# bgconley/cadence-rag

Hardware: AMD Instinct MI355X
Metric: queries/sec @ recall@10=1.0 (exact cosine top-10, 1024-d fp32 corpus) (higher is better)
Workload: dtype f32; 1 GPU; BASELINE configs[1]: brute-force cosine top-10, 100000x1024 fp32 corpus on one GPU, 64 queries/step resident in HBM; rows_per_gpu=100000, rows_total=100000, dim=1024, k=10, parallelism=1 GPU, rounds=1, arithmetic=fp16-MFMA prefilter (proven bound) + exact fp32 rescoring, api=crag_index_search_async (in stream order), hbm_bytes_per_corpus_row=6156

## Files before the change

### cadence_rag_amd/_native.py

```python
from __future__ import annotations

import ctypes
import os
import subprocess
from pathlib import Path
from typing import Optional

_CSRC = Path(__file__).resolve().parent / "csrc"
LIB_PATH = Path(os.environ["CRAG_DENSE_LIB"]) if os.environ.get("CRAG_DENSE_LIB") else _CSRC / "libcrag_dense.so"

CRAG_MAX_K = 128
CRAG_DIM = 1024
CRAG_DEDUPE_MAX_WIDTH = 256
CRAG_SUBSET_MAX_WIDTH = 4096
CRAG_GROUP_MAX_PER = 8
CRAG_FILTER_MAX_QUERIES = 64
CRAG_ATTR_MAX_QUERIES = 64
CRAG_ATTR_MAX_CLAUSES = 8
CRAG_ATTR_MAX_KEYS = 512
CRAG_FACET_MAX_QUERIES = 64
CRAG_FACET_MAX_NAMESPACES = 16
CRAG_FACET_MAX_TOP = 64
CRAG_E2BIG = -5
CRAG_DECODE_MAX_SEQS = 8
CRAG_DECODE_MAX_ROWS = 8
CRAG_DECODE_SPLIT = 128
CRAG_LM_HEAD_MAX_BANNED = 64
CRAG_EXTEND_BLOCK = 32
CRAG_EXTEND_TILE = 32
CRAG_EXTEND_SPLIT = 512
CRAG_EXTEND_SPLIT_ROWS = 512
CRAG_GRAMMAR_MAX_STATES = 4096
CRAG_GRAMMAR_MAX_CLASSES = 64
CRAG_GRAMMAR_DEAD = 0xFFFF
CRAG_SAMPLE_MIN_TEMPERATURE = 0.01
CRAG_SAMPLE_MAX_TEMPERATURE = 100.0

_c = ctypes
_P = _c.c_void_p
SIGNATURES = {
    "crag_last_error": (_c.c_char_p, []),
    "crag_version": (_c.c_char_p, []),
    "crag_device_count": (_c.c_int, []),
    "crag_index_create": (_c.c_int, [_c.c_int, _c.c_int, _c.c_int64, _c.POINTER(_P)]),
    "crag_index_destroy": (_c.c_int, [_P]),
    "crag_index_add": (_c.c_int, [_P, _P, _P, _c.c_int64]),
    "crag_index_update": (_c.c_int, [_P, _c.c_int64, _P, _c.c_int64]),
    "crag_index_remove": (_c.c_int, [_P, _P, _c.c_int64, _c.POINTER(_c.c_int64)]),
    "crag_index_compact": (_c.c_int, [_P, _P, _c.POINTER(_c.c_int64)]),
    "crag_index_insert": (_c.c_int, [_P, _P, _P, _c.c_int64]),
    "crag_index_size": (_c.c_int64, [_P]),
    "crag_index_capacity": (_c.c_int64, [_P]),
    "crag_index_dim": (_c.c_int, [_P]),
    "crag_index_get_rows": (_c.c_int, [_P, _c.c_int64, _c.c_int64, _P, _P]),
    "crag_index_count_eligible": (_c.c_int, [_P, _P, _c.POINTER(_c.c_int64)]),
    "crag_index_search": (_c.c_int, [_P, _P, _c.c_int, _c.c_int, _P, _c.c_int64, _P, _P, _P]),
    "crag_index_search_async": (_c.c_int, [_P, _P, _c.c_int, _c.c_int, _P, _c.c_int64, _P, _P, _P, _P]),
    "crag_merge_topk": (_c.c_int, [_c.c_int, _P, _P, _P, _c.c_int, _c.c_int, _c.c_int, _P, _P, _P, _P]),
    "crag_result_record_bytes": (_c.c_int64, [_c.c_int, _c.c_int]),
    "crag_merge_topk_packed": (_c.c_int, [_c.c_int, _P, _c.c_int, _c.c_int, _c.c_int, _P, _P, _P, _P]),
    "crag_rrf_fuse": (_c.c_int, [_c.c_int, _P, _P, _P, _c.c_int, _c.c_int, _c.c_int, _P, _P, _P, _P, _P]),
    "crag_tech_lane": (_c.c_int, [_P, _P, _P, _P, _c.c_int64, _P, _P, _c.c_int, _c.c_int, _P, _c.c_int64, _P, _P, _P, _P]),
    "crag_upload_slot_create": (_P, []),
    "crag_upload_slot_destroy": (None, [_P]),
    "crag_tech_lane_host": (_c.c_int, [_P, _P, _P, _P, _c.c_int64, _P, _P, _c.c_int, _c.c_int, _P, _c.c_int64, _P, _P, _P,
                                       _P, _P]),
    "crag_bm25_scratch_bytes": (_c.c_int64, [_c.c_int64, _c.c_int, _c.c_int]),
    "crag_bm25_lane_host": (_c.c_int, [_P, _P, _P, _P, _P, _c.c_int64, _c.c_int64, _c.c_float, _P, _P, _P, _c.c_int, _c.c_int,
                                       _P, _c.c_int64, _P, _P, _c.c_int64, _P, _P, _P, _P]),
    "crag_filter_masks_host": (_c.c_int, [_P, _P, _c.c_int64, _c.c_int64, _P, _P, _P, _c.c_int, _P, _P, _c.c_int64, _P]),
    "crag_attr_masks_host": (_c.c_int, [_P, _P, _c.c_int64, _c.c_int64, _P, _P, _c.c_int, _P, _c.c_int, _P, _c.c_int64, _P, _P,
                                        _c.c_int64, _P]),
    "crag_facet_workspace_bytes": (_c.c_int64, [_c.c_int64, _c.c_int, _c.c_int64, _c.c_int]),
    "crag_facet_counts_host": (_c.c_int, [_P, _P, _P, _c.c_int64, _c.c_int64, _c.c_int64, _P, _c.c_int64, _P, _P, _c.c_int,
                                          _c.c_int, _c.c_int, _P, _c.c_int64, _P, _P, _P, _P, _P]),
    "crag_index_profile_enable": (_c.c_int, [_P, _c.c_int]),
    "crag_index_profile_read": (_c.c_int, [_P, _c.POINTER(_c.c_int64), _c.POINTER(_c.c_double),
                                           _c.POINTER(_c.c_double)]),
    "crag_index_profile_read_ex": (_c.c_int, [_P, _c.POINTER(_c.c_int64), _c.POINTER(_c.c_double),
                                              _c.POINTER(_c.c_double), _c.POINTER(_c.c_double)]),
    "crag_index_last_scan_kernel": (_c.c_char_p, [_P]),
    "crag_index_scan_waits": (_c.c_char_p, [_P]),
    "crag_index_prefilter_row_bytes": (_c.c_int64, [_P]),
    "crag_index_search_pipelined": (_c.c_int, [_P, _P, _c.c_int, _c.c_int, _P, _c.c_int64, _P, _P, _P, _P, _c.c_int]),
    "crag_index_join": (_c.c_int, [_P, _P]),
    "crag_index_dedupe_async": (_c.c_int, [_P, _P, _P, _c.c_int, _c.c_int, _c.c_float, _P, _P, _P, _P, _P]),
    "crag_index_search_ids_scratch_bytes": (_c.c_int64, [_c.c_int, _c.c_int]),
    "crag_index_search_ids_async": (_c.c_int, [_P, _P, _c.c_int, _P, _P, _c.c_int, _c.c_int64, _c.c_int, _P, _P, _P, _P, _P,
                                               _c.c_int64, _P]),
    "crag_index_search_grouped_scratch_bytes": (_c.c_int64, [_c.c_int, _c.c_int64, _c.c_int]),
    "crag_index_search_grouped_async": (_c.c_int, [_P, _P, _c.c_int, _c.c_int, _P, _c.c_int64, _c.c_int, _P, _c.c_int64,
                                                   _P, _P, _P, _P, _P, _c.c_int64, _P]),
    "crag_index_phase_trace": (_c.c_int, [_P, _c.POINTER(_c.c_uint64)]),
    "crag_index_prefilter_stats": (_c.c_int, [_P, _c.POINTER(_c.c_int64), _c.POINTER(_c.c_int64),
                                              _c.POINTER(_c.c_int64)]),
    "crag_index_scan_geometry": (_c.c_int, [_P, _c.c_int, _c.POINTER(_c.c_int), _c.POINTER(_c.c_int),
                                            _c.POINTER(_c.c_int), _c.POINTER(_c.c_int64)]),
    "crag_enc_embed_gather": (_c.c_int, [_P, _P, _P, _c.c_int64, _c.c_int, _c.c_int64, _P]),
    "crag_enc_rmsnorm": (_c.c_int, [_P, _P, _P, _P, _P, _c.c_int64, _c.c_int, _c.c_float, _P]),
    "crag_enc_qk_norm_rope": (_c.c_int, [_P, _P, _P, _P, _P, _c.c_int64, _c.c_int, _c.c_int, _c.c_float, _P]),
    "crag_enc_v_transpose": (_c.c_int, [_P, _P, _P, _c.c_int64, _c.c_int, _c.c_int, _P]),
    "crag_enc_attention": (_c.c_int, [_P, _P, _P, _P, _P, _P, _P, _c.c_int, _c.c_int64, _c.c_int, _c.c_int,
                                      _c.c_float, _P]),
    "crag_enc_swiglu": (_c.c_int, [_P, _P, _c.c_int64, _c.c_int, _P]),
    "crag_enc_skinny_gemm": (_c.c_int, [_P, _P, _P, _c.c_int, _c.c_int, _c.c_int, _c.c_int, _c.c_int, _P]),
    "crag_enc_qk_rope_vt": (_c.c_int, [_P, _P, _P, _P, _P, _c.c_int64, _c.c_int, _c.c_int, _c.c_float, _P, _P, _c.c_int64, _P]),
    "crag_enc_pool_normalize": (_c.c_int, [_P, _P, _P, _P, _c.c_int, _c.c_int, _c.c_int, _c.c_int, _c.c_float, _P]),
    "crag_enc_pool_normalize_add": (_c.c_int, [_P, _P, _P, _P, _P, _c.c_int, _c.c_int, _c.c_int, _c.c_int, _c.c_float, _P]),
    "crag_enc_pool_normalize_rows": (_c.c_int, [_P, _P, _P, _P, _P, _c.c_int, _c.c_int, _c.c_int, _c.c_float, _P]),
    "crag_enc_small_gemm": (_c.c_int, [_P, _P, _P, _P, _P, _P, _c.c_int, _c.c_int, _c.c_int, _c.c_int, _c.c_int, _c.c_int,
                                       _c.c_float, _P]),
    "crag_enc_wide_partial_bytes": (_c.c_int64, [_c.c_int, _c.c_int, _c.c_int]),
    "crag_enc_wide_gemm": (_c.c_int, [_P, _P, _P, _c.c_int, _c.c_int, _c.c_int, _c.c_int, _P]),
    "crag_enc_wide_gemm_direct": (_c.c_int, [_P, _P, _P, _c.c_int, _c.c_int, _c.c_int, _c.c_int, _c.c_int, _P]),
    "crag_enc_wide_reduce": (_c.c_int, [_P, _P, _c.c_int, _c.c_int, _c.c_int, _c.c_int, _c.c_int, _P]),
    "crag_enc_wide_gemm_rows": (_c.c_int, [_P, _P, _P, _c.c_int, _c.c_int, _c.c_int, _c.c_int, _P]),
    "crag_enc_rmsnorm_partials": (_c.c_int, [_P, _c.c_int, _c.c_int, _P, _P, _P, _P, _c.c_int, _c.c_int, _c.c_float, _P]),
    "crag_enc_small_attention": (_c.c_int, [_P, _P, _P, _P, _c.c_int, _P, _P, _c.c_int, _c.c_int, _c.c_int, _c.c_float,
                                            _c.c_float, _P]),
    "crag_enc_small_attention_seqs": (_c.c_int, [_P, _P, _P, _P, _c.c_int, _P, _P, _c.c_int, _c.c_int, _P, _c.c_int,
                                                 _c.c_int, _c.c_float, _c.c_float, _P]),
    "crag_enc_small_attention_seqs_parts": (_c.c_int, [_P, _c.c_int, _c.c_int, _P, _P, _P, _c.c_int, _P, _P, _c.c_int,
                                                       _c.c_int, _P, _c.c_int, _c.c_int, _c.c_float, _c.c_float, _P]),
    "crag_enc_attention_prefixed": (_c.c_int, [_P, _P, _P, _P, _P, _P, _P, _P, _c.c_int, _c.c_int64, _c.c_int, _c.c_int,
                                               _c.c_float, _P]),
    "crag_enc_rerank_head": (_c.c_int, [_P, _P, _P, _P, _P, _P, _c.c_int, _c.c_int, _c.c_float, _P]),
    "crag_enc_decode_workspace_bytes": (_c.c_int64, [_c.c_int, _c.c_int, _c.c_int]),
    "crag_enc_decode_attention": (_c.c_int, [_P, _P, _P, _P, _c.c_int, _P, _P, _c.c_int, _c.c_int, _P, _P, _c.c_int, _c.c_int,
                                             _c.c_int, _c.c_float, _c.c_float, _P, _c.c_int64, _P, _P]),
    "crag_enc_decode_attention_shared": (_c.c_int, [_P, _P, _P, _P, _c.c_int, _P, _P, _c.c_int, _c.c_int, _P, _P, _P, _P,
                                                    _c.c_int, _c.c_int, _c.c_int, _c.c_float, _c.c_float, _P, _c.c_int64,
                                                    _P, _P]),
    "crag_enc_decode_attention_rows": (_c.c_int, [_P, _P, _P, _P, _c.c_int, _P, _P, _c.c_int, _c.c_int, _P, _P, _P, _P, _P,
                                                  _c.c_int, _c.c_int, _c.c_int, _c.c_float, _c.c_float, _P, _c.c_int64,
                                                  _P, _P]),
    "crag_enc_lm_head": (_c.c_int, [_P, _P, _P, _P, _P, _P, _P, _c.c_int, _c.c_int, _c.c_int, _c.c_int64, _c.c_float, _P]),
    "crag_enc_extend_workspace_bytes": (_c.c_int64, [_c.c_int, _c.c_int, _c.c_int, _c.c_int]),
    "crag_enc_extend_attention": (_c.c_int, [_P, _P, _P, _P, _c.c_int, _P, _P, _c.c_int, _c.c_int, _P, _P, _P, _c.c_int,
                                             _c.c_int, _c.c_int, _c.c_float, _c.c_float, _P, _c.c_int64, _P, _P]),
    "crag_enc_grammar_argmax": (_c.c_int, [_P, _c.c_int64, _P, _P, _P, _P, _P, _P, _c.c_int, _c.c_int, _P, _P, _P, _c.c_int,
                                           _P]),
    "crag_enc_sample": (_c.c_int, [_P, _c.c_int64, _P, _P, _P, _P, _P, _P, _c.c_uint64, _c.c_uint32, _P, _P, _P, _c.c_int, _P]),
    "crag_enc_grammar_advance": (_c.c_int, [_P, _P, _P, _c.c_int64, _P, _P, _c.c_int, _c.c_int, _P, _P, _c.c_int, _P]),
    "crag_enc_logprobs": (_c.c_int, [_P, _c.c_int64, _P, _P, _P, _P, _P, _P, _P, _P, _c.c_int, _c.c_int, _P]),
}


class NativeLibraryError(RuntimeError):
    """libcrag_dense.so is missing, failed to load, or a call into it failed."""


_lib: Optional[ctypes.CDLL] = None


def build_native(force: bool = False) -> Path:
    cmd = ["make", "-C", str(_CSRC)] + (["-B"] if force else [])
    proc = subprocess.run(cmd, capture_output=True, text=True)
    if proc.returncode != 0:
        raise NativeLibraryError(f"building libcrag_dense.so failed:\n{proc.stdout}\n{proc.stderr}")
    return LIB_PATH


def load() -> ctypes.CDLL:
    global _lib
    if _lib is not None:
        return _lib
    if not LIB_PATH.exists():
        raise NativeLibraryError(
            f"{LIB_PATH} not found: the dense lane has no CPU fallback. Build it with "
            f"`python -c 'import __graft_entry__ as g; g.build()'` or `make -C {_CSRC}`.")
    try:
        lib = ctypes.CDLL(str(LIB_PATH))
    except OSError as exc:
        raise NativeLibraryError(f"failed to load {LIB_PATH}: {exc}") from exc
    for name, (restype, argtypes) in SIGNATURES.items():
        try:
            fn = getattr(lib, name)
        except AttributeError as exc:
            raise NativeLibraryError(f"{LIB_PATH} does not export {name}") from exc
        fn.restype = restype
        fn.argtypes = argtypes
    _lib = lib
    return lib


def last_error() -> str:
    msg = load().crag_last_error()
    return msg.decode("utf-8", "replace") if msg else ""


def check(rc: int, what: str) -> None:
    if rc != 0:
        raise NativeLibraryError(f"{what} failed (code {rc}): {last_error()}")
```

### cadence_rag_amd/csrc/crag_api.hip

```cpp

#include <stdlib.h>

#include <new>

#include "crag_index.h"

namespace {

thread_local char g_err[512] = "";

int init_index(crag_index *ix) {
    const size_t cbytes = (size_t)ix->cap_rows * crag::DIM * sizeof(float);
    hipError_t e;
    if ((e = hipMalloc((void **)&ix->corpus, cbytes)) != hipSuccess ||
        (e = hipMalloc((void **)&ix->inv_norm, (size_t)ix->cap_rows * sizeof(float))) != hipSuccess ||
        (e = hipMalloc((void **)&ix->ids, (size_t)ix->cap_rows * sizeof(int64_t))) != hipSuccess)
        return fail(CRAG_ENOMEM, "hipMalloc for %lld rows failed: %s", (long long)ix->cap_rows, hipGetErrorString(e));
    if ((e = hipMemset(ix->inv_norm, 0, (size_t)ix->cap_rows * sizeof(float))) != hipSuccess ||
        (e = hipMemset(ix->corpus, 0, cbytes)) != hipSuccess)
        return fail(CRAG_EHIP, "hipMemset failed: %s", hipGetErrorString(e));
    for (auto &w : ix->ws)
        if ((e = hipEventCreateWithFlags(&w.done, hipEventDisableTiming)) != hipSuccess)
            return fail(CRAG_EHIP, "hipEventCreate failed: %s", hipGetErrorString(e));
    ix->sw.no_wide = getenv("CRAG_NO_WIDE") != nullptr;
    ix->env_no_reverse = getenv("CRAG_NO_REVERSE") != nullptr;
    ix->env_unpipelined = getenv("CRAG_UNPIPELINED") != nullptr;
    ix->sw.no_prefilter = getenv("CRAG_NO_PREFILTER") != nullptr;
    ix->sw.no_rsplit = getenv("CRAG_NO_RSPLIT") != nullptr;
    if (const char *v = getenv("CRAG_PF_NT")) ix->sw.pf_nt = atoi(v) ? 1 : 0;
    if (const char *v = getenv("CRAG_PF_WAITS")) {
        if (!strcmp(v, "tile")) ix->sw.pf_waits = crag::PF_WAITS_TILE;
        else if (!strcmp(v, "fragment")) ix->sw.pf_waits = crag::PF_WAITS_FRAGMENT;
    }
    if (const char *v = getenv("CRAG_PF_LAGS")) {
        int d = 0, r = 0;
        if (sscanf(v, "%d,%d", &d, &r) == 2 && d >= 1 && r > d && r <= 4) {
            ix->sw.pf_derive_lag = d;
            ix->sw.pf_read_lag = r;
        }
    }
    if (const char *v = getenv("CRAG_TEST_FAIL_AFTER_SCAN")) ix->env_fail_after_scan = atoll(v);
    if (const char *v = getenv("CRAG_PIPE_STREAMS")) {
        const int n = atoi(v);
        if (n >= 1 && n <= crag_index::MAX_PIPE) ix->n_pipe = n;
    }
    if (const char *v = getenv("CRAG_EDIT_CHUNK_ROWS")) {
        const long long c = atoll(v);
        if (c >= 32 && c % 32 == 0 && c <= ((long long)1 << 24)) ix->edit_chunk_rows = c;
    }
    if (const char *v = getenv("CRAG_PF_NT_ABOVE_MB")) ix->sw.nt_above_bytes = (int64_t)atoll(v) << 20;
    if (!ix->sw.no_prefilter && getenv("CRAG_NO_FP16_MIRROR") == nullptr) {
        const size_t mbytes = (size_t)ix->cap_rows * crag::DIM * sizeof(_Float16);
        if ((e = hipMalloc((void **)&ix->corpus16, mbytes)) != hipSuccess ||
            (e = hipMemset(ix->corpus16, 0, mbytes)) != hipSuccess)
            return fail(CRAG_ENOMEM, "hipMalloc for the fp16 mirror of %lld rows failed: %s", (long long)ix->cap_rows,
                        hipGetErrorString(e));
    }
    if ((e = hipMalloc((void **)&ix->irregular_dev, sizeof(uint32_t))) != hipSuccess ||
        (e = hipMalloc((void **)&ix->pf_stats, crag::PF_STAT_SLOTS * 3 * sizeof(unsigned long long))) != hipSuccess ||
        (e = hipMemset(ix->irregular_dev, 0, sizeof(uint32_t))) != hipSuccess ||
        (e = hipMemset(ix->pf_stats, 0, crag::PF_STAT_SLOTS * 3 * sizeof(unsigned long long))) != hipSuccess)
        return fail(CRAG_ENOMEM, "hipMalloc for the index state failed: %s", hipGetErrorString(e));
    if (getenv("CRAG_PHASE_TRACE") != nullptr) {
        if ((e = hipMalloc((void **)&ix->phase_trace, 128 * sizeof(unsigned long long))) != hipSuccess ||
            (e = hipMemset(ix->phase_trace, 0, 128 * sizeof(unsigned long long))) != hipSuccess)
            return fail(CRAG_ENOMEM, "hipMalloc for the phase trace failed: %s", hipGetErrorString(e));
    }
    return CRAG_OK;
}

int check_merge_args(bool any_null, int n_lists, int nq, int k) {
    if (any_null) return fail(CRAG_EINVAL, "NULL pointer argument");
    if (n_lists <= 0 || nq < 0 || k <= 0 || k > CRAG_MAX_K)
        return fail(CRAG_EINVAL, "bad sizes n_lists=%d nq=%d k=%d", n_lists, nq, k);
    if ((int64_t)n_lists * k > 4096) return fail(CRAG_EINVAL, "n_lists*k must be <= 4096");
    return CRAG_OK;
}

int merge_lists(int device, crag::XMergeParams &p, int n_lists, int nq, int k, int64_t *d_out_ids, float *d_out_scores,
                int32_t *d_out_counts, void *stream) {
    DeviceGuard guard(device);
    if (!guard.ok) return fail(CRAG_EHIP, "hipSetDevice(%d) failed", device);
    p.out_ids = d_out_ids;
    p.out_scores = d_out_scores;
    p.out_counts = d_out_counts;
    p.n_lists = n_lists;
    p.nq = nq;
    p.k = k;
    HIP_TRY(crag::launch_merge_results(p, (hipStream_t)stream));
    return CRAG_OK;
}

}

extern "C" {

const char *crag_last_error(void) { return g_err; }

void crag_set_error_(const char *msg) { snprintf(g_err, sizeof(g_err), "%s", msg ? msg : ""); }

const char *crag_version(void) { return "cadence-rag_amd dense lane 0.1 (gfx950)"; }

int crag_device_count(void) {
    int n = 0;
    if (hipGetDeviceCount(&n) != hipSuccess) {
        (void)hipGetLastError();
        return 0;
    }
    return n;
}

int crag_index_create(int device, int dim, int64_t capacity, crag_index **out) {
    if (!out) return fail(CRAG_EINVAL, "out is NULL");
    *out = nullptr;
    if (dim <= 0 || dim > CRAG_DIM) return fail(CRAG_EINVAL, "dim must be in [1, %d] (got %d)", CRAG_DIM, dim);
    if (capacity <= 0) return fail(CRAG_EINVAL, "capacity must be > 0 (got %lld)", (long long)capacity);
    int ndev = crag_device_count();
    if (ndev <= 0) return fail(CRAG_ENODEV, "no HIP device visible");
    if (device < 0 || device >= ndev) return fail(CRAG_EINVAL, "device %d out of range [0, %d)", device, ndev);
    DeviceGuard guard(device);
    if (!guard.ok) return fail(CRAG_EHIP, "hipSetDevice(%d) failed", device);
    hipDeviceProp_t prop;
    HIP_TRY(hipGetDeviceProperties(&prop, device));
    if (strncmp(prop.gcnArchName, "gfx950", 6) != 0)
        return fail(CRAG_ENODEV, "device %d is %s; this library is built for gfx950 only", device,
                    prop.gcnArchName);
    crag_index *ix = new (std::nothrow) crag_index();
    if (!ix) return fail(CRAG_ENOMEM, "out of host memory");
    ix->device = device;
    ix->dim = dim;
    ix->capacity = capacity;
    ix->cap_rows = ((capacity + 31) / 32) * 32;
    ix->n_cu = prop.multiProcessorCount;
    int rc = init_index(ix);
    if (rc) {
        crag_index_destroy(ix);
        return rc;
    }
    *out = ix;
    return CRAG_OK;
}

int crag_index_destroy(crag_index *ix) {
    if (!ix) return CRAG_OK;
    DeviceGuard guard(ix->device);
    (void)hipDeviceSynchronize();
    for (auto &t : ix->ev_pool)
        for (hipEvent_t e : {t.e0, t.e1a, t.e1, t.e2, t.e3}) (void)hipEventDestroy(e);
    for (int i = 0; i < crag_index::MAX_PIPE; ++i) {
        if (ix->pipe_fork[i]) (void)hipEventDestroy(ix->pipe_fork[i]);
        if (ix->pipe_done[i]) (void)hipEventDestroy(ix->pipe_done[i]);
        if (ix->pipe[i]) (void)hipStreamDestroy(ix->pipe[i]);
    }
    for (void *p : {(void *)ix->irregular_dev, (void *)ix->phase_trace, (void *)ix->pf_stats, (void *)ix->corpus,
                    (void *)ix->corpus16, (void *)ix->inv_norm, (void *)ix->ids})
        if (p) (void)hipFree(p);
    for (auto &w : ix->ws) {
        for (auto &b : w.buf) b.release();
        if (w.done) (void)hipEventDestroy(w.done);
    }
    for (DevBuf *b : {&ix->stage_q, &ix->stage_rows, &ix->stage_ids, &ix->stage_mask, &ix->stage_out, &ix->scratch,
                      &ix->edit_bounce, &ix->edit_srcpos, &ix->edit_mask, &ix->edit_prefix, &ix->edit_newpos})
        b->release();
    delete ix;
    return CRAG_OK;
}

int64_t crag_index_size(const crag_index *ix) { return ix ? ix->size : -1; }
int64_t crag_index_capacity(const crag_index *ix) { return ix ? ix->capacity : -1; }
int crag_index_dim(const crag_index *ix) { return ix ? ix->dim : -1; }

int crag_merge_topk(int device, const int64_t *d_ids, const float *d_scores, const int32_t *d_counts,
                    int n_lists, int nq, int k, int64_t *d_out_ids, float *d_out_scores,
                    int32_t *d_out_counts, void *stream) {
    int rc = check_merge_args(!d_ids || !d_scores || !d_counts || !d_out_ids || !d_out_scores || !d_out_counts, n_lists,
                              nq, k);
    if (rc || nq == 0) return rc;
    crag::XMergeParams p;
    p.ids = d_ids;
    p.scores = d_scores;
    p.counts = d_counts;
    p.stride_ids = (int64_t)nq * k;
    p.stride_scores = (int64_t)nq * k;
    p.stride_counts = nq;
    return merge_lists(device, p, n_lists, nq, k, d_out_ids, d_out_scores, d_out_counts, stream);
}

int64_t crag_result_record_bytes(int nq, int k) {
    if (nq < 0 || k <= 0) return -1;
    const int64_t b = (int64_t)nq * k * 8 + (int64_t)nq * k * 4 + (int64_t)nq * 4;
    return (b + 7) & ~(int64_t)7;
}

int crag_merge_topk_packed(int device, const void *d_records, int n_lists, int nq, int k, int64_t *d_out_ids,
                           float *d_out_scores, int32_t *d_out_counts, void *stream) {
    int rc = check_merge_args(!d_records || !d_out_ids || !d_out_scores || !d_out_counts, n_lists, nq, k);
    if (rc || nq == 0) return rc;
    const int64_t rec = crag_result_record_bytes(nq, k);
    const char *base = (const char *)d_records;
    crag::XMergeParams p;
    p.ids = (const int64_t *)base;
    p.scores = (const float *)(base + (int64_t)nq * k * 8);
    p.counts = (const int32_t *)(base + (int64_t)nq * k * 12);
    p.stride_ids = rec / 8;
    p.stride_scores = rec / 4;
    p.stride_counts = rec / 4;
    return merge_lists(device, p, n_lists, nq, k, d_out_ids, d_out_scores, d_out_counts, stream);
}

int crag_index_profile_enable(crag_index *ix, int enabled) {
    if (!ix) return fail(CRAG_EINVAL, "index is NULL");
    std::lock_guard<std::mutex> lk(ix->mu);
    ix->profiling = enabled > 0 ? enabled : 0;
    ix->prof_calls = 0;
    ix->ev_used = 0;
    return CRAG_OK;
}

int crag_index_profile_read_ex(crag_index *ix, int64_t *n_launches, double *scan_ms_total,
                               double *merge_ms_total, double *event_pair_ms_total) {
    if (!ix) return fail(CRAG_EINVAL, "index is NULL");
    std::lock_guard<std::mutex> lk(ix->mu);
    DeviceGuard guard(ix->device);
    double scan = 0.0, merge = 0.0, pair = 0.0;
    for (size_t i = 0; i < ix->ev_used; ++i) {
        float a = 0.f, b = 0.f, c = 0.f, d = 0.f;
        HIP_TRY(hipEventSynchronize(ix->ev_pool[i].e3));
        HIP_TRY(hipEventElapsedTime(&a, ix->ev_pool[i].e0, ix->ev_pool[i].e1a));
        HIP_TRY(hipEventElapsedTime(&d, ix->ev_pool[i].e1a, ix->ev_pool[i].e1));
        HIP_TRY(hipEventElapsedTime(&b, ix->ev_pool[i].e1, ix->ev_pool[i].e2));
        HIP_TRY(hipEventElapsedTime(&c, ix->ev_pool[i].e2, ix->ev_pool[i].e3));
        scan += b;
        merge += a + c;
        pair += d;
    }
    if (n_launches) *n_launches = (int64_t)ix->ev_used;
    if (scan_ms_total) *scan_ms_total = scan;
    if (merge_ms_total) *merge_ms_total = merge;
    if (event_pair_ms_total) *event_pair_ms_total = pair;
    ix->ev_used = 0;
    return CRAG_OK;
}

int crag_index_profile_read(crag_index *ix, int64_t *n_launches, double *scan_ms_total,
                            double *merge_ms_total) {
    return crag_index_profile_read_ex(ix, n_launches, scan_ms_total, merge_ms_total, nullptr);
}

int crag_index_prefilter_stats(crag_index *ix, int64_t *searches, int64_t *candidates, int64_t *rescored_rows) {
    if (!ix) return fail(CRAG_EINVAL, "index is NULL");
    std::lock_guard<std::mutex> lk(ix->mu);
    DeviceGuard guard(ix->device);
    unsigned long long v[3] = {0, 0, 0};
    std::vector<unsigned long long> rec((size_t)crag::PF_STAT_SLOTS * 3);
    HIP_TRY(hipDeviceSynchronize());
    HIP_TRY(hipMemcpy(rec.data(), ix->pf_stats, rec.size() * sizeof(unsigned long long), hipMemcpyDeviceToHost));
    HIP_TRY(hipMemset(ix->pf_stats, 0, rec.size() * sizeof(unsigned long long)));
    for (size_t i = 0; i < rec.size(); ++i) v[i % 3] += rec[i];
    if (candidates) *candidates = (int64_t)v[0];
    if (rescored_rows) *rescored_rows = (int64_t)v[1];
    if (searches) *searches = (int64_t)v[2];
    return CRAG_OK;
}

int crag_index_phase_trace(crag_index *ix, uint64_t *out128) {
    if (!ix || !out128) return fail(CRAG_EINVAL, "index / out is NULL");
    if (!ix->phase_trace) return fail(CRAG_EINVAL, "the index was not created with CRAG_PHASE_TRACE=1");
    std::lock_guard<std::mutex> lk(ix->mu);
    DeviceGuard guard(ix->device);
    HIP_TRY(hipDeviceSynchronize());
    HIP_TRY(hipMemcpy(out128, ix->phase_trace, 128 * sizeof(unsigned long long), hipMemcpyDeviceToHost));
    return CRAG_OK;
}

const char *crag_index_last_scan_kernel(const crag_index *ix) { return ix ? ix->last_scan_kernel : ""; }
const char *crag_index_scan_waits(const crag_index *ix) { return ix ? ix->last_scan_waits : ""; }

int64_t crag_index_prefilter_row_bytes(const crag_index *ix) {
    if (!ix || ix->sw.no_prefilter) return 0;
    return (int64_t)crag::DIM * (ix->corpus16 ? 2 : 4);
}

int crag_index_scan_geometry(const crag_index *ix, int nq, int *workgroups, int *threads,
                             int *query_blocks, int64_t *algorithmic_bytes_per_launch) {
    if (!ix) return fail(CRAG_EINVAL, "index is NULL");
    const int qb = (nq + 31) / 32;
    if (workgroups) *workgroups = plan_search(ix->size, ix->n_cu, nq, 1, false, false, ix->sw).G;
    if (threads) *threads = crag::SCAN_THREADS;
    if (query_blocks) *query_blocks = qb;
    if (algorithmic_bytes_per_launch)
        *algorithmic_bytes_per_launch = ix->size * (int64_t)ix->dim * 4 + (int64_t)nq * ix->dim * 4;
    return CRAG_OK;
}

}
```

### cadence_rag_amd/csrc/crag_api_search.hip

```cpp

#include "crag_index.h"

namespace {

struct SearchArgs {
    const float *queries;
    int nq, k;
    const uint8_t *mask;
    int64_t mask_stride;
    int64_t *out_ids;
    float *out_scores;
    int32_t *out_counts;
};

int acquire_workspace(crag_index *ix, hipStream_t st, Workspace **out) {
    Workspace *ws = nullptr;
    for (auto &w : ix->ws)
        if (w.in_use && w.stream == st) ws = &w;
    if (!ws)
        for (auto &w : ix->ws)
            if (!w.in_use) {
                w.in_use = true;
                w.stream = st;
                ws = &w;
                if (&w == &ix->ws[crag_index::MAX_WS - 1]) ix->record_done = true;
                break;
            }
    if (!ws) {
        for (auto &w : ix->ws)
            if (!ws || w.last_use < ws->last_use) ws = &w;
        if (ws->done_recorded && !ws->dirty) {
            HIP_TRY(hipStreamWaitEvent(st, ws->done, 0));
        } else {
            HIP_TRY(hipDeviceSynchronize());
        }
        ix->record_done = true;
        ws->stream = st;
    }
    ws->last_use = ++ix->use_clock;
    *out = ws;
    return CRAG_OK;
}

int reserve_workspace(const crag_index *ix, Workspace *ws, const SearchPlan &pl, int k, hipStream_t st) {
    DevBuf *b = ws->buf;
    const size_t nq_pad = (size_t)pl.nq_pad;
    int rc;
    if ((rc = b[Workspace::PARTIAL].ensure((size_t)pl.q_blocks * pl.G * 32 * (size_t)k * sizeof(uint2)))) return rc;
    if ((rc = b[Workspace::GBOUND].ensure_zeroed((size_t)pl.q_blocks * 32 * crag::GB_CELLS * sizeof(uint32_t), st))) return rc;
    if ((rc = b[Workspace::A32].ensure(nq_pad * crag::DIM * sizeof(float)))) return rc;
    if ((rc = b[Workspace::QINV].ensure(nq_pad * sizeof(float)))) return rc;
    if (!pl.prefilter) return CRAG_OK;
    if ((rc = b[Workspace::A16].ensure(nq_pad * crag::DIM * 2))) return rc;
    if ((rc = b[Workspace::PF_GBOUND].ensure_zeroed((ix->n_cu + nq_pad) * crag::PF_BOUND_CELLS * sizeof(uint32_t), st))) return rc;
    if ((rc = b[Workspace::PF_CAND].ensure(nq_pad * pl.cap * sizeof(uint2)))) return rc;
    if (pl.rsplit > 1) {
        const size_t slots = nq_pad * 8;
        if ((rc = b[Workspace::PF_XKEYS].ensure(slots * CRAG_MAX_K * sizeof(uint64_t)))) return rc;
        if ((rc = b[Workspace::PF_XIDS].ensure(slots * CRAG_MAX_K * sizeof(int64_t)))) return rc;
        if ((rc = b[Workspace::PF_XCOUNT].ensure(slots * sizeof(uint2)))) return rc;
        if ((rc = b[Workspace::PF_XTICKET].ensure_zeroed(nq_pad * sizeof(uint32_t), st))) return rc;
    }
    if ((rc = b[Workspace::PF_COUNT].ensure_zeroed(nq_pad * sizeof(uint32_t), st))) return rc;
    if ((rc = b[Workspace::PF_FLAGS].ensure_zeroed(4 * sizeof(uint32_t), st))) return rc;
    if (ws->dirty) {
        for (int i = Workspace::KEPT_ZERO_FIRST; i < Workspace::KEPT_ZERO_END; ++i)
            if (b[i].p) HIP_TRY(hipMemsetAsync(b[i].p, 0, b[i].bytes, st));
        ws->dirty = false;
    }
    return CRAG_OK;
}

int profile_begin(crag_index *ix, hipStream_t st, EvSet **out) {
    *out = nullptr;
    if (!(ix->profiling > 0 && (ix->prof_calls++ % ix->profiling) == ix->profiling / 2)) return CRAG_OK;
    if (ix->ev_used == ix->ev_pool.size()) {
        EvSet t;
        for (hipEvent_t *e : {&t.e0, &t.e1a, &t.e1, &t.e2, &t.e3}) HIP_TRY(hipEventCreate(e));
        ix->ev_pool.push_back(t);
    }
    *out = &ix->ev_pool[ix->ev_used++];
    HIP_TRY(hipEventRecord((*out)->e0, st));
    return CRAG_OK;
}

crag::PrepParams prep_params(const crag_index *ix, const Workspace *ws, const SearchPlan &pl, const SearchArgs &a) {
    return crag::PrepParams{a.queries, a.nq, ix->dim, ws->at<float>(Workspace::QINV), ws->at<float>(Workspace::A32),
                            pl.prefilter ? ws->at<_Float16>(Workspace::A16) : nullptr};
}

crag::ScanParams scan_params(const crag_index *ix, const Workspace *ws, const SearchPlan &pl, const SearchArgs &a,
                             int reverse) {
    crag::ScanParams sp;
    sp.wide = pl.wide;
    sp.corpus = ix->corpus;
    sp.inv_norm = ix->inv_norm;
    sp.queries = a.queries;
    sp.a32 = ws->at<const float>(Workspace::A32);
    sp.qinv = ws->at<const float>(Workspace::QINV);
    sp.gate = nullptr;
    sp.dim = ix->dim;
    sp.mask = (const uint32_t *)a.mask;
    sp.mask_stride_w = a.mask_stride / 4;
    sp.partial = ws->at<uint2>(Workspace::PARTIAL);
    sp.gbound = ws->at<uint32_t>(Workspace::GBOUND);
    sp.n_rows = ix->size;
    sp.cap_rows = ix->cap_rows;
    sp.nq = a.nq;
    sp.k = a.k;
    sp.G = pl.G;
    sp.nb = pl.nb;
    sp.pub_rank = pl.pub_rank;
    sp.reverse = reverse;
    sp.unpipelined = (ix->env_unpipelined && !pl.prefilter) ? 1 : 0;
    sp.piece_shift = crag::crag_piece_shift(ix->corpus16 != nullptr);
    return sp;
}

crag::MergeParams merge_params(const crag_index *ix, const Workspace *ws, const SearchPlan &pl, const SearchArgs &a) {
    crag::MergeParams mp;
    mp.partial = ws->at<const uint2>(Workspace::PARTIAL);
    mp.ids = ix->ids;
    mp.gbound = ws->at<uint32_t>(Workspace::GBOUND);
    mp.id_base = 0;
    mp.out_ids = a.out_ids;
    mp.out_scores = a.out_scores;
    mp.out_counts = a.out_counts;
    mp.k = a.k;
    mp.G = pl.G;
    return mp;
}

crag::PfParams pf_params(const crag_index *ix, const Workspace *ws, const SearchPlan &pl, const SearchArgs &a,
                         int reverse) {
    crag::PfParams fp;
    fp.corpus = ix->corpus;
    fp.corpus16 = ix->corpus16;
    fp.inv_norm = ix->inv_norm;
    fp.a16 = ws->at<const _Float16>(Workspace::A16);
    fp.qinv = ws->at<const float>(Workspace::QINV);
    fp.mask = (const uint32_t *)a.mask;
    fp.mask_stride_w = a.mask_stride / 4;
    fp.gbound_idle = ws->at<const uint32_t>(Workspace::PF_GBOUND);
    fp.gbound = ws->at<uint32_t>(Workspace::PF_GBOUND) + (size_t)ix->n_cu * crag::PF_BOUND_CELLS;
    fp.cand = ws->at<uint2>(Workspace::PF_CAND);
    fp.count = ws->at<uint32_t>(Workspace::PF_COUNT);
    fp.flags = ws->at<uint32_t>(Workspace::PF_FLAGS);
    fp.seq = ws->seq;
    fp.n_rows = ix->size;
    fp.nq = a.nq;
    fp.k = a.k;
    fp.G = pl.G;
    fp.reverse = reverse;
    fp.sets = pl.sets;
    fp.pub0 = pl.pub0;
    fp.cap = pl.cap;
    fp.derive_lag = pl.derive_lag;
    fp.read_lag = pl.read_lag;
    fp.nt = pl.nt;
    return fp;
}

crag::FinParams fin_params(const crag_index *ix, const Workspace *ws, const SearchPlan &pl, const SearchArgs &a,
                           const crag::PfParams &fp, crag::ScanParams sp, const crag::MergeParams &mp) {
    crag::FinParams fin;
    fin.corpus = ix->corpus;
    fin.inv_norm = ix->inv_norm;
    fin.a32 = ws->at<const float>(Workspace::A32);
    fin.qinv = ws->at<const float>(Workspace::QINV);
    fin.cand = ws->at<const uint2>(Workspace::PF_CAND);
    fin.count = ws->at<uint32_t>(Workspace::PF_COUNT);
    fin.gbound = fp.gbound;
    fin.flags = ws->at<const uint32_t>(Workspace::PF_FLAGS);
    fin.seq = fp.seq;
    fin.ids = ix->ids;
    fin.out_ids = a.out_ids;
    fin.out_scores = a.out_scores;
    fin.out_counts = a.out_counts;
    fin.stats = ix->pf_stats + (size_t)(ws - ix->ws) * (crag::PF_STAT_SLOTS / crag_index::MAX_WS) * 3;
    fin.k = a.k;
    fin.cap = pl.cap;
    fin.merge = mp;
    fin.nq = a.nq;
    fin.rsplit = pl.rsplit;
    const bool shared = pl.rsplit > 1;
    fin.xkeys = shared ? ws->at<uint64_t>(Workspace::PF_XKEYS) : nullptr;
    fin.xids = shared ? ws->at<int64_t>(Workspace::PF_XIDS) : nullptr;
    fin.xcount = shared ? ws->at<uint2>(Workspace::PF_XCOUNT) : nullptr;
    fin.xticket = shared ? ws->at<uint32_t>(Workspace::PF_XTICKET) : nullptr;
    sp.wide = 0;
    sp.gate = nullptr;
    sp.unpipelined = 1;
    fin.scan = sp;
    fin.fb_blocks = pl.fb_blocks;
    fin.fb_done = ws->at<uint32_t>(Workspace::PF_FLAGS) + 1;
    fin.trace = ix->phase_trace;
    return fin;
}

int search_device(crag_index *ix, const SearchArgs &a, hipStream_t st) {
    if (a.nq <= 0) return CRAG_OK;
    const SearchPlan pl = plan_search(ix->size, ix->n_cu, a.nq, a.k, ix->corpus16 != nullptr, ix->irregular, ix->sw);
    int rc;
    Workspace *ws = nullptr;
    if ((rc = acquire_workspace(ix, st, &ws))) return rc;
    if ((rc = reserve_workspace(ix, ws, pl, a.k, st))) return rc;
    if (pl.window_too_large)
        return fail(CRAG_EINVAL, "index too large for one device scan window (%lld rows)", (long long)ix->size);
    EvSet *ev = nullptr;
    if ((rc = profile_begin(ix, st, &ev))) return rc;

    HIP_TRY(crag::launch_prep_queries(prep_params(ix, ws, pl, a), pl.nq_pad, st));
    const int reverse = ix->env_no_reverse ? 0 : ix->pass_parity;
    ix->pass_parity ^= 1;
    const crag::ScanParams sp = scan_params(ix, ws, pl, a, reverse);
    const crag::MergeParams mp = merge_params(ix, ws, pl, a);
    if (ev) {
        HIP_TRY(hipEventRecord(ev->e1a, st));
        HIP_TRY(hipEventRecord(ev->e1, st));
    }
    if (pl.prefilter) {
        if (++ws->seq == 0u) ws->seq = 1u;
        const crag::PfParams fp = pf_params(ix, ws, pl, a, reverse);
        const int nqb = pl.wide ? 2 : 1;
        ws->dirty = true;
        const int waits = pf_waits_for(ix->size * (int64_t)crag::DIM * 2, ix->corpus16 != nullptr, pl.nt, ix->sw.pf_waits);
        HIP_TRY(crag::launch_prefilter(fp, nqb, pl.nq_pad / (32 * nqb), waits == crag::PF_WAITS_FRAGMENT, st,
                                       &ix->last_scan_kernel));
        ix->last_scan_waits = waits == crag::PF_WAITS_FRAGMENT ? "fragment" : "tile";
        if (ix->env_fail_after_scan > 0 && ++ix->pf_searches == ix->env_fail_after_scan)
            return fail(CRAG_EHIP, "injected failure behind the scan launch (CRAG_TEST_FAIL_AFTER_SCAN)");
        if (ev) HIP_TRY(hipEventRecord(ev->e2, st));
        HIP_TRY(crag::launch_finalize(fin_params(ix, ws, pl, a, fp, sp, mp), st));
        ws->dirty = false;
    } else {
        HIP_TRY(crag::launch_scan(sp, pl.q_blocks, st, &ix->last_scan_kernel));
        ix->last_scan_waits = "tile";
        if (ev) HIP_TRY(hipEventRecord(ev->e2, st));
        HIP_TRY(crag::launch_merge_partials(mp, a.nq, st));
    }
    if (ev) HIP_TRY(hipEventRecord(ev->e3, st));
    ws->done_recorded = ix->record_done;
    if (ix->record_done) HIP_TRY(hipEventRecord(ws->done, st));
    return CRAG_OK;
}

int check_search_args(const crag_index *ix, const SearchArgs &a) {
    if (!ix) return fail(CRAG_EINVAL, "index is NULL");
    if (a.nq < 0) return fail(CRAG_EINVAL, "nq must be >= 0 (got %d)", a.nq);
    if (a.k <= 0 || a.k > CRAG_MAX_K) return fail(CRAG_EINVAL, "k must be in [1, %d] (got %d)", CRAG_MAX_K, a.k);
    if (a.nq > 0 && (!a.queries || !a.out_ids || !a.out_scores || !a.out_counts))
        return fail(CRAG_EINVAL, "queries / out_ids / out_scores / out_counts must not be NULL");
    if (a.mask) {
        const int64_t need = ((ix->size + 31) / 32) * 4;
        if (a.mask_stride != 0 && (a.mask_stride % 4 != 0 || a.mask_stride < need))
            return fail(CRAG_EINVAL, "mask_stride must be 0 or a multiple of 4 >= %lld (got %lld)",
                        (long long)need, (long long)a.mask_stride);
        if (((uintptr_t)a.mask) & 3) return fail(CRAG_EINVAL, "row_mask must be 4-byte aligned");
    }
    return CRAG_OK;
}

}

extern "C" {

int crag_search_plan_(int64_t size, int n_cu, int nq, int k, int has_mirror, int irregular, int no_wide,
                      int no_prefilter, int no_rsplit, int pf_derive_lag, int pf_read_lag, int pf_nt,
                      int64_t nt_above_bytes, SearchPlan *out) {
    const SearchSwitches sw = {no_wide, no_prefilter, no_rsplit, pf_derive_lag, pf_read_lag, pf_nt, nt_above_bytes};
    if (out) *out = plan_search(size, n_cu, nq, k, has_mirror != 0, irregular != 0, sw);
    return (int)sizeof(SearchPlan);
}

int crag_pf_waits_(int64_t mirror_bytes, int has_mirror, int nt, int pf_waits_switch) {
    return pf_waits_for(mirror_bytes, has_mirror != 0, nt, pf_waits_switch);
}

int64_t crag_pf_frag_waits_max_bytes_(void) { return crag::PF_FRAG_WAITS_MAX_BYTES; }

int crag_index_search_async(crag_index *ix, const float *d_queries, int nq, int k,
                            const uint8_t *d_row_mask, int64_t mask_stride, int64_t *d_out_ids,
                            float *d_out_scores, int32_t *d_out_counts, void *stream) {
    const SearchArgs a = {d_queries, nq, k, d_row_mask, mask_stride, d_out_ids, d_out_scores, d_out_counts};
    int rc = check_search_args(ix, a);
    if (rc) return rc;
    std::lock_guard<std::mutex> lk(ix->mu);
    DeviceGuard guard(ix->device);
    return search_device(ix, a, (hipStream_t)stream);
}

int crag_index_search_pipelined(crag_index *ix, const float *d_queries, int nq, int k,
                                const uint8_t *d_row_mask, int64_t mask_stride, int64_t *d_out_ids,
                                float *d_out_scores, int32_t *d_out_counts, void *stream, int flags) {
    const SearchArgs a = {d_queries, nq, k, d_row_mask, mask_stride, d_out_ids, d_out_scores, d_out_counts};
    int rc = check_search_args(ix, a);
    if (rc) return rc;
    std::lock_guard<std::mutex> lk(ix->mu);
    DeviceGuard guard(ix->device);
    for (int i = 0; i < ix->n_pipe; ++i) {
        if (!ix->pipe[i]) HIP_TRY(hipStreamCreateWithFlags(&ix->pipe[i], hipStreamNonBlocking));
        if (!ix->pipe_fork[i]) HIP_TRY(hipEventCreateWithFlags(&ix->pipe_fork[i], hipEventDisableTiming));
        if (!ix->pipe_done[i]) HIP_TRY(hipEventCreateWithFlags(&ix->pipe_done[i], hipEventDisableTiming));
    }
    if (k > 24 || ix->n_pipe <= 1) return search_device(ix, a, (hipStream_t)stream);
    const int i = (int)(ix->pipe_next++ % (unsigned)ix->n_pipe);
    if (!(flags & CRAG_PIPE_INPUTS_READY)) {
        HIP_TRY(hipEventRecord(ix->pipe_fork[i], (hipStream_t)stream));
        HIP_TRY(hipStreamWaitEvent(ix->pipe[i], ix->pipe_fork[i], 0));
    }
    rc = search_device(ix, a, ix->pipe[i]);
    if (rc) return rc;
    ix->pipe_pending[i] = true;
    return CRAG_OK;
}

int crag_index_join(crag_index *ix, void *stream) {
    if (!ix) return fail(CRAG_EINVAL, "index is NULL");
    std::lock_guard<std::mutex> lk(ix->mu);
    DeviceGuard guard(ix->device);
    for (int i = 0; i < ix->n_pipe; ++i)
        if (ix->pipe_pending[i]) {
            HIP_TRY(hipEventRecord(ix->pipe_done[i], ix->pipe[i]));
            HIP_TRY(hipStreamWaitEvent((hipStream_t)stream, ix->pipe_done[i], 0));
            ix->pipe_pending[i] = false;
        }
    return CRAG_OK;
}

int crag_index_search(crag_index *ix, const float *queries, int nq, int k, const uint8_t *row_mask,
                      int64_t mask_stride, int64_t *out_ids, float *out_scores, int32_t *out_counts) {
    int rc = check_search_args(ix, {queries, nq, k, row_mask, mask_stride, out_ids, out_scores, out_counts});
    if (rc) return rc;
    if (nq == 0) return CRAG_OK;
    std::lock_guard<std::mutex> lk(ix->mu);
    DeviceGuard guard(ix->device);

    const float *dq = nullptr;
    if ((rc = stage_in(ix->stage_q, queries, (size_t)nq * ix->dim * sizeof(float), &dq))) return rc;
    const uint8_t *dm = nullptr;
    int64_t dstride = 0;
    if ((rc = stage_row_masks(ix, row_mask, mask_stride, nq, &dm, &dstride))) return rc;
    const bool ids_dev = is_device_ptr(out_ids), sc_dev = is_device_ptr(out_scores),
               ct_dev = is_device_ptr(out_counts);
    const size_t b_ids = (size_t)nq * k * sizeof(int64_t), b_sc = (size_t)nq * k * sizeof(float),
                 b_ct = (size_t)nq * sizeof(int32_t);
    if ((rc = ix->stage_out.ensure(b_ids + b_sc + b_ct + 64))) return rc;
    char *so = (char *)ix->stage_out.p;
    int64_t *d_ids = ids_dev ? out_ids : (int64_t *)so;
    float *d_sc = sc_dev ? out_scores : (float *)(so + b_ids);
    int32_t *d_ct = ct_dev ? out_counts : (int32_t *)(so + b_ids + b_sc);

    rc = search_device(ix, {dq, nq, k, dm, dstride, d_ids, d_sc, d_ct}, 0);
    if (rc) return rc;
    HIP_TRY(hipStreamSynchronize(0));
    if (!ids_dev) HIP_TRY(hipMemcpy(out_ids, d_ids, b_ids, hipMemcpyDeviceToHost));
    if (!sc_dev) HIP_TRY(hipMemcpy(out_scores, d_sc, b_sc, hipMemcpyDeviceToHost));
    if (!ct_dev) HIP_TRY(hipMemcpy(out_counts, d_ct, b_ct, hipMemcpyDeviceToHost));
    return CRAG_OK;
}

int crag_index_dedupe_async(crag_index *ix, const int64_t *d_ids, const int32_t *d_counts, int nq, int width,
                            float threshold, int64_t *d_out_ids, int32_t *d_out_counts, int32_t *d_out_dup_of,
                            float *d_out_sim, void *stream) {
    if (!ix) return fail(CRAG_EINVAL, "index is NULL");
    if (nq < 0) return fail(CRAG_EINVAL, "nq must be >= 0 (got %d)", nq);
    if (width < 1 || width > CRAG_DEDUPE_MAX_WIDTH)
        return fail(CRAG_EINVAL, "width must be in [1, %d] (got %d)", CRAG_DEDUPE_MAX_WIDTH, width);
    if (!(threshold > -1.f && threshold <= 1.f))
        return fail(CRAG_EINVAL, "threshold must be finite, in (-1, 1] (got %g)", (double)threshold);
    if (!d_ids || !d_counts || !d_out_ids || !d_out_counts)
        return fail(CRAG_EINVAL, "ids / counts / out_ids / out_counts must not be NULL");
    if (nq == 0) return CRAG_OK;
    std::lock_guard<std::mutex> lk(ix->mu);
    DeviceGuard guard(ix->device);
    crag::DedupeParams p;
    p.corpus = ix->corpus;
    p.inv_norm = ix->inv_norm;
    p.stored = ix->ids;
    p.size = ix->size;
    p.piece_shift = crag::crag_piece_shift(ix->corpus16 != nullptr);
    p.ids = d_ids;
    p.counts = d_counts;
    p.width = width;
    p.threshold = threshold;
    p.out_ids = d_out_ids;
    p.out_counts = d_out_counts;
    p.out_dup_of = d_out_dup_of;
    p.out_sim = d_out_sim;
    HIP_TRY(crag::launch_dedupe(p, nq, (hipStream_t)stream));
    return CRAG_OK;
}

int64_t crag_index_search_ids_scratch_bytes(int nq, int width) { return crag::subset_scratch_bytes(nq, width); }

int crag_index_search_ids_async(crag_index *ix, const float *d_queries, int nq, const int64_t *d_ids,
                                const int32_t *d_counts, int width, int64_t list_stride, int k, int64_t *d_out_ids,
                                float *d_out_scores, int32_t *d_out_counts, float *d_out_slot_scores, void *d_scratch,
                                int64_t scratch_bytes, void *stream) {
    if (!ix) return fail(CRAG_EINVAL, "search_ids: index is NULL");
    if (nq < 0 || nq > 65535) return fail(CRAG_EINVAL, "search_ids: nq must be in [0, 65535] (got %d)", nq);
    if (width < 1) return fail(CRAG_EINVAL, "search_ids: width must be >= 1 (got %d)", width);
    if (k < 1 || k > CRAG_MAX_K) return fail(CRAG_EINVAL, "search_ids: k must be in [1, %d] (got %d)", CRAG_MAX_K, k);
    if (list_stride != 0 && list_stride != width)
        return fail(CRAG_EINVAL, "search_ids: list_stride must be 0 (one shared list) or width (got %lld)",
                    (long long)list_stride);
    if (!d_queries || !d_ids || !d_counts || !d_out_ids || !d_out_scores || !d_out_counts || !d_scratch)
        return fail(CRAG_EINVAL, "search_ids: queries / ids / counts / outputs / scratch must not be NULL");
    if (width > CRAG_SUBSET_MAX_WIDTH)
        return fail(CRAG_E2BIG, "search_ids: width %d exceeds CRAG_SUBSET_MAX_WIDTH (%d): use the row_mask route", width,
                    CRAG_SUBSET_MAX_WIDTH);
    if (scratch_bytes < crag::subset_scratch_bytes(nq, width) || ((uintptr_t)d_scratch & 7))
        return fail(CRAG_EINVAL, "search_ids: scratch too small or not 8-byte aligned (crag_index_search_ids_scratch_bytes)");
    if (nq == 0) return CRAG_OK;
    std::lock_guard<std::mutex> lk(ix->mu);
    DeviceGuard guard(ix->device);
    crag::SubsetParams p;
    p.corpus = ix->corpus;
    p.inv_norm = ix->inv_norm;
    p.stored = ix->ids;
    p.size = ix->size;
    p.piece_shift = crag::crag_piece_shift(ix->corpus16 != nullptr);
    p.queries = d_queries;
    p.nq = nq;
    p.dim = ix->dim;
    p.k = k;
    p.ids = d_ids;
    p.counts = d_counts;
    p.width = width;
    p.list_stride = list_stride;
    p.keys = (uint64_t *)d_scratch;
    p.out_ids = d_out_ids;
    p.out_scores = d_out_scores;
    p.out_counts = d_out_counts;
    p.out_slot_scores = d_out_slot_scores;
    HIP_TRY(crag::launch_subset(p, (hipStream_t)stream));
    return CRAG_OK;
}

int64_t crag_index_search_grouped_scratch_bytes(int nq, int64_t n_groups, int per_group) {
    return crag::group_scratch_bytes(nq, n_groups, per_group);
}

int crag_index_search_grouped_async(crag_index *ix, const float *d_queries, int nq, int k, const int32_t *d_row_group,
                                    int64_t n_groups, int per_group, const uint8_t *d_row_mask, int64_t mask_stride,
                                    int64_t *d_out_ids, float *d_out_scores, int32_t *d_out_groups, int32_t *d_out_counts,
                                    void *d_scratch, int64_t scratch_bytes, void *stream) {
    if (!ix) return fail(CRAG_EINVAL, "search_grouped: index is NULL");
    if (nq < 0 || nq > 65535) return fail(CRAG_EINVAL, "search_grouped: nq must be in [0, 65535] (got %d)", nq);
    if (k < 1 || k > CRAG_MAX_K) return fail(CRAG_EINVAL, "search_grouped: k must be in [1, %d] (got %d)", CRAG_MAX_K, k);
    if (per_group < 1 || per_group > CRAG_GROUP_MAX_PER)
        return fail(CRAG_EINVAL, "search_grouped: per_group must be in [1, %d] (got %d)", CRAG_GROUP_MAX_PER, per_group);
    if (n_groups < 1 || n_groups >= ((int64_t)1 << 31))
        return fail(CRAG_EINVAL, "search_grouped: n_groups must be in [1, 2^31) (got %lld)", (long long)n_groups);
    if (!d_queries || !d_row_group || !d_out_ids || !d_out_scores || !d_out_counts || !d_scratch)
        return fail(CRAG_EINVAL, "search_grouped: queries / row_group / out_ids / out_scores / out_counts / scratch must not be NULL");
    if (d_row_mask) {
        const int64_t need = ((ix->size + 31) / 32) * 4;
        if (mask_stride != 0 && (mask_stride % 4 != 0 || mask_stride < need))
            return fail(CRAG_EINVAL, "search_grouped: mask_stride must be 0 or a multiple of 4 >= %lld (got %lld)",
                        (long long)need, (long long)mask_stride);
        if (((uintptr_t)d_row_mask) & 3) return fail(CRAG_EINVAL, "search_grouped: row_mask must be 4-byte aligned");
    }
    if (scratch_bytes < crag::group_scratch_bytes(nq, n_groups, per_group) || ((uintptr_t)d_scratch & 7))
        return fail(CRAG_EINVAL,
                    "search_grouped: scratch too small or not 8-byte aligned (crag_index_search_grouped_scratch_bytes)");
    if (nq == 0) return CRAG_OK;
    std::lock_guard<std::mutex> lk(ix->mu);
    DeviceGuard guard(ix->device);
    crag::GroupParams p;
    p.corpus = ix->corpus;
    p.inv_norm = ix->inv_norm;
    p.stored = ix->ids;
    p.size = ix->size;
    p.piece_shift = crag::crag_piece_shift(ix->corpus16 != nullptr);
    p.queries = d_queries;
    p.nq = nq;
    p.dim = ix->dim;
    p.k = k;
    p.row_group = d_row_group;
    p.n_groups = n_groups;
    p.per_group = per_group;
    p.mask = (const uint32_t *)d_row_mask;
    p.mask_stride_w = mask_stride / 4;
    p.table = (uint64_t *)d_scratch;
    p.qinv = (float *)(p.table + (size_t)nq * (size_t)n_groups * (size_t)per_group);
    p.out_ids = d_out_ids;
    p.out_scores = d_out_scores;
    p.out_groups = d_out_groups;
    p.out_counts = d_out_counts;
    HIP_TRY(crag::launch_grouped(p, (hipStream_t)stream));
    return CRAG_OK;
}

}
```

### cadence_rag_amd/csrc/crag_exact.h

```cpp
#pragma once
#include <hip/hip_runtime.h>
#include <stdint.h>

#include "crag_kernels.h"
#include "crag_layout.h"

namespace crag {

__device__ __forceinline__ uint32_t f2ord(float f) {
    uint32_t u = __float_as_uint(f);
    return (u & 0x80000000u) ? ~u : (u | 0x80000000u);
}
__device__ __forceinline__ float ord2f(uint32_t u) {
    u = (u & 0x80000000u) ? (u & 0x7fffffffu) : ~u;
    return __uint_as_float(u);
}
__device__ __forceinline__ uint64_t mk64(uint32_t hi, uint32_t lo) {
    return ((uint64_t)hi << 32) | lo;
}

__device__ __forceinline__ void sort_keys_desc(uint64_t *keys, int P) {
    const int tid = threadIdx.x;
    for (int k2 = 2; k2 <= P; k2 <<= 1)
        for (int j = k2 >> 1; j > 0; j >>= 1) {
            for (int t = tid; t < (P >> 1); t += SCAN_THREADS) {
                const int i = ((t & ~(j - 1)) << 1) | (t & (j - 1)), l = i | j;
                const uint64_t a = keys[i], b = keys[l];
                const bool desc = (i & k2) == 0;
                if (desc ? a < b : a > b) {
                    keys[i] = b;
                    keys[l] = a;
                }
            }
            __syncthreads();
        }
}

__device__ __forceinline__ f32x4 load_query_quad(const float *queries, int dim, int q, int nq, int t) {
    f32x4 v = {0.f, 0.f, 0.f, 0.f};
    if (q < nq && t < 256) {
        const float *src = queries + (size_t)q * dim;
        if ((dim & 3) == 0) {
            if (4 * t < dim) v = *reinterpret_cast<const f32x4 *>(src + 4 * t);
        } else {
#pragma unroll
            for (int c = 0; c < 4; ++c)
                if (4 * t + c < dim) v[c] = src[4 * t + c];
        }
    }
    return v;
}

__device__ __forceinline__ float canonical_qinv(const f32x4 v, bool real_query, double *sh) {
    double ss = ((double)v[0] * v[0] + (double)v[1] * v[1]) + ((double)v[2] * v[2] + (double)v[3] * v[3]);
    for (int o = 32; o > 0; o >>= 1) ss += __shfl_xor(ss, o);
    const int wv = threadIdx.x >> 6;
    if ((threadIdx.x & 63) == 0 && wv < 4) sh[wv] = ss;
    __syncthreads();
    const double tot = sh[0] + sh[1] + sh[2] + sh[3];
    __syncthreads();
    const bool ok = real_query && (tot > 0.0) && (tot < 1.0e300) && (tot == tot);
    float qinv = ok ? (float)(1.0 / sqrt(tot)) : 0.f;
    if (!(qinv < 3.0e38f)) qinv = 0.f;
    return qinv;
}

__device__ __forceinline__ void make_key(float dot, float scale, int64_t row, uint32_t &khi, uint32_t &klo) {
    float sc = dot * scale;
    sc = __builtin_amdgcn_fmed3f(sc, -1.f, 1.f);
    const bool ok = (scale > 0.f) && (sc == sc);
    khi = ok ? f2ord(sc) : 0u;
    klo = ok ? ~(uint32_t)row : 0u;
}

template <int PS>
__device__ __forceinline__ float exact_slice_dot(const f32x4 *qslice ,
                                                 const f32x4 *ctile , int jrow) {
    f32x4 c0[16], c1[16];
#pragma unroll
    for (int s = 0; s < 16; ++s) {
        c0[s] = ctile[(((2 * s) >> PS) * 32 + jrow) * (1 << PS) + ((2 * s) & ((1 << PS) - 1))];
        c1[s] = ctile[(((2 * s) >> PS) * 32 + jrow) * (1 << PS) + ((2 * s) & ((1 << PS) - 1)) + 1];
    }
    float acc = 0.f;
#pragma unroll
    for (int s = 0; s < 16; ++s) {
        const f32x4 q0 = qslice[2 * s], q1 = qslice[2 * s + 1];
#pragma unroll
        for (int cc = 0; cc < 4; ++cc) {
            acc = __builtin_fmaf(q0[cc], c0[s][cc], acc);
            acc = __builtin_fmaf(q1[cc], c1[s][cc], acc);
        }
    }
    return acc;
}

template <int PS>
__device__ __forceinline__ void exact_slice_fetch(const f32x4 *ctile , int jrow, f32x4 (&c0)[16],
                                                  f32x4 (&c1)[16]) {
#pragma unroll
    for (int s = 0; s < 16; ++s) {
        c0[s] = ctile[(((2 * s) >> PS) * 32 + jrow) * (1 << PS) + ((2 * s) & ((1 << PS) - 1))];
        c1[s] = ctile[(((2 * s) >> PS) * 32 + jrow) * (1 << PS) + ((2 * s) & ((1 << PS) - 1)) + 1];
    }
}

__device__ __forceinline__ void slice_query_read(const f32x4 *qslice, int h, f32x4 (&q)[8]) {
#pragma unroll
    for (int i = 0; i < 8; ++i) q[i] = qslice[8 * h + i];
}
__device__ __forceinline__ float slice_query_fma(float acc, int h, const f32x4 (&q)[8], const f32x4 (&c0)[16],
                                                 const f32x4 (&c1)[16]) {
#pragma unroll
    for (int s4 = 0; s4 < 4; ++s4) {
        const f32x4 q0 = q[2 * s4], q1 = q[2 * s4 + 1];
#pragma unroll
        for (int cc = 0; cc < 4; ++cc) {
            acc = __builtin_fmaf(q0[cc], c0[4 * h + s4][cc], acc);
            acc = __builtin_fmaf(q1[cc], c1[4 * h + s4][cc], acc);
        }
    }
    return acc;
}
__device__ __forceinline__ float exact_slice_fma(const f32x4 *qslice , const f32x4 (&c0)[16],
                                                 const f32x4 (&c1)[16]) {
    f32x4 qa[8], qb[8];
    slice_query_read(qslice, 0, qa);
    slice_query_read(qslice, 1, qb);
    __builtin_amdgcn_sched_barrier(0);
    float acc = slice_query_fma(0.f, 0, qa, c0, c1);
    __builtin_amdgcn_sched_barrier(0);
    slice_query_read(qslice, 2, qa);
    __builtin_amdgcn_sched_barrier(0);
    acc = slice_query_fma(acc, 1, qb, c0, c1);
    __builtin_amdgcn_sched_barrier(0);
    slice_query_read(qslice, 3, qb);
    __builtin_amdgcn_sched_barrier(0);
    acc = slice_query_fma(acc, 2, qa, c0, c1);
    acc = slice_query_fma(acc, 3, qb, c0, c1);
    return acc;
}

}
```

### cadence_rag_amd/csrc/crag_index.h

```cpp
#pragma once
#include <mutex>
#include <vector>

#include "crag_host.h"
#include "crag_kernels.h"
#include "crag_search_plan.h"

#pragma GCC visibility push(hidden)

int stage_row_masks(struct crag_index *ix, const uint8_t *row_mask, int64_t mask_stride, int nq, const uint8_t **d_mask,
                    int64_t *d_stride);

struct EvSet {
    hipEvent_t e0, e1a, e1, e2, e3;
};

struct Workspace {
    enum Buf {
        PARTIAL, GBOUND,
        A32, A16, QINV, PF_CAND, PF_XKEYS, PF_XIDS, PF_XCOUNT,
        PF_GBOUND, PF_COUNT, PF_FLAGS, PF_XTICKET,
        N_BUF,
        KEPT_ZERO_FIRST = PF_GBOUND, KEPT_ZERO_END = N_BUF
    };
    DevBuf buf[N_BUF];
    template <class T> T *at(Buf b) const { return (T *)buf[b].p; }
    hipStream_t stream = nullptr;
    bool in_use = false;
    hipEvent_t done = nullptr;
    uint32_t seq = 0;
    bool done_recorded = false;
    bool dirty = false;
    uint64_t last_use = 0;
};

#pragma GCC visibility pop

struct crag_index {
    int device = 0;
    int dim = 0;
    int64_t capacity = 0;
    int64_t cap_rows = 0;
    int64_t size = 0;
    int n_cu = 0;
    float *corpus = nullptr;
    _Float16 *corpus16 = nullptr;
    float *inv_norm = nullptr;
    int64_t *ids = nullptr;
    static constexpr int MAX_WS = 8;
    Workspace ws[MAX_WS];
    static constexpr int MAX_PIPE = 4;
    int n_pipe = 3;
    hipStream_t pipe[MAX_PIPE] = {nullptr, nullptr, nullptr, nullptr};
    hipEvent_t pipe_fork[MAX_PIPE] = {nullptr, nullptr, nullptr, nullptr}, pipe_done[MAX_PIPE] = {nullptr, nullptr, nullptr, nullptr};
    bool pipe_pending[MAX_PIPE] = {false, false, false, false};
    unsigned pipe_next = 0;
    uint64_t use_clock = 0;
    bool record_done = false;
    int64_t last_id = INT64_MIN;
    SearchSwitches sw;
    bool env_no_reverse = false, env_unpipelined = false;
    bool irregular = false;
    uint32_t *irregular_dev = nullptr;
    unsigned long long *pf_stats = nullptr;
    unsigned long long *phase_trace = nullptr;
    const char *last_scan_kernel = "";
    const char *last_scan_waits = "";
    DevBuf stage_q, stage_rows, stage_ids, stage_mask, stage_out, scratch;
    int64_t edit_chunk_rows = 16384;
    DevBuf edit_bounce, edit_srcpos, edit_mask, edit_prefix, edit_newpos;
    std::mutex mu;
    int pass_parity = 0;
    int64_t env_fail_after_scan = 0;
    int64_t pf_searches = 0;
    int profiling = 0;
    int64_t prof_calls = 0;
    std::vector<EvSet> ev_pool;
    size_t ev_used = 0;
};

static_assert(crag_index::MAX_WS == crag::PF_STAT_WS, "one block of statistics records per workspace");
```

### cadence_rag_amd/csrc/crag_kernels.h

```cpp
#pragma once
#include <hip/hip_runtime.h>
#include <stdint.h>

#include "crag_arch.h"

namespace crag {

constexpr int TILE_ROWS = 32;
constexpr int DIM = 1024;
constexpr int TILE_FLOATS = TILE_ROWS * DIM;
constexpr int SCAN_WAVES = 8;
constexpr int SCAN_THREADS = SCAN_WAVES * 64;
constexpr int KSLICE = DIM / SCAN_WAVES;
constexpr int GB_CELLS = 32;

struct ScanParams {
    const float *corpus;
    const float *inv_norm;
    const float *queries;
    const float *a32;
    const float *qinv;
    const uint32_t *gate;
    int wide;
    const uint32_t *mask;
    int64_t mask_stride_w;
    uint2 *partial;
    uint32_t *gbound;
    int64_t n_rows;
    int64_t cap_rows;
    int nq;
    int dim;
    int k;
    int G;
    int nb;
    int pub_rank;
    int reverse;
    int unpipelined;
    int piece_shift;
};

struct MergeParams {
    const uint2 *partial;
    const int64_t *ids;
    uint32_t *gbound;
    int64_t id_base;
    int64_t *out_ids;
    float *out_scores;
    int32_t *out_counts;
    int k;
    int G;
};

constexpr int PF_BOUND_CELLS = 160;
constexpr int PF_STAT_WS = 8;
constexpr int PF_STAT_SLOTS = 2048;
constexpr int PF_MIN_ROWS_PER_GROUP = 128;
enum PfWaits { PF_WAITS_TILE = 0, PF_WAITS_FRAGMENT = 1 };
constexpr int64_t PF_FRAG_WAITS_MAX_BYTES = 256ll << 20;

struct PrepParams {
    const float *queries;
    int nq, dim;
    float *qinv;
    float *a32;
    _Float16 *a16;
};

struct PfParams {
    const float *corpus;
    const _Float16 *corpus16;
    const float *inv_norm;
    const _Float16 *a16;
    const float *qinv;
    const uint32_t *mask;
    int64_t mask_stride_w;
    uint32_t *gbound;
    const uint32_t *gbound_idle;
    uint2 *cand;
    uint32_t *count;
    uint32_t *flags;
    uint32_t seq;
    int64_t n_rows;
    int nq, k, G, reverse;
    int sets;
    int pub0;
    int nt;
    int derive_lag, read_lag;
    int cap;
};

struct FinParams {
    const float *corpus;
    const float *inv_norm;
    const float *a32;
    const float *qinv;
    const uint2 *cand;
    uint32_t *count;
    uint32_t *gbound;
    const uint32_t *flags;
    uint32_t seq;
    const int64_t *ids;
    int64_t *out_ids;
    float *out_scores;
    int32_t *out_counts;
    unsigned long long *stats;
    int k, cap;
    int nq;
    int rsplit;
    uint64_t *xkeys;
    int64_t *xids;
    uint2 *xcount;
    uint32_t *xticket;
    int fb_blocks;
    uint32_t *fb_done;
    unsigned long long *trace;

    ScanParams scan;
    MergeParams merge;
};

struct XMergeParams {
    const int64_t *ids;
    const float *scores;
    const int32_t *counts;
    int64_t *out_ids;
    float *out_scores;
    int32_t *out_counts;
    int64_t stride_ids, stride_scores, stride_counts;
    int n_lists;
    int nq;
    int k;
};

hipError_t launch_scan(const ScanParams &p, int q_blocks, hipStream_t st, const char **kernel_name);
hipError_t launch_prep_queries(const PrepParams &p, int nq_pad, hipStream_t st);
hipError_t launch_prefilter(const PfParams &p, int nqb, int passes, int frag_waits, hipStream_t st,
                            const char **kernel_name);
hipError_t launch_finalize(const FinParams &p, hipStream_t st);
hipError_t launch_merge_partials(const MergeParams &p, int nq, hipStream_t st);
hipError_t launch_merge_results(const XMergeParams &p, hipStream_t st);
hipError_t launch_store_rows(const float *rows, int dim, int64_t pos, int64_t n, float *corpus,
                             float *inv_norm, uint32_t *irregular, _Float16 *mirror, hipStream_t st);
hipError_t launch_load_rows(const float *corpus, int dim, int64_t pos, int64_t n, float *rows, int piece_shift,
                            hipStream_t st);
inline int crag_piece_shift(bool has_mirror) { return has_mirror ? 5 : 2; }
hipError_t launch_count_eligible(const float *inv_norm, int64_t n, const uint32_t *mask,
                                 unsigned long long *out, hipStream_t st);
hipError_t launch_check_ids(const int64_t *ids, int64_t n, int64_t prev, unsigned long long *out_bad,
                            hipStream_t st);
hipError_t launch_fill_ids(int64_t *ids, int64_t pos, int64_t n, int64_t first, hipStream_t st);

struct RowStore {
    float *corpus;
    _Float16 *mirror;
    float *inv_norm;
    int64_t *ids;
};
hipError_t launch_lookup_ids(const int64_t *stored, int64_t size, const int64_t *ids, int64_t n, int64_t *pos,
                             int add_index, uint32_t *drop, unsigned long long *found, hipStream_t st);
hipError_t launch_remove_srcpos(const uint32_t *keep, const uint32_t *prefix, int64_t n_words, int64_t d0, int64_t m,
                                int64_t *srcpos, hipStream_t st);
hipError_t launch_insert_srcpos(const int64_t *newpos, int64_t n_new, int64_t d0, int64_t m, int64_t *srcpos,
                                hipStream_t st);
hipError_t launch_move_rows(const RowStore &index, const RowStore &bounce, const int64_t *srcpos, int64_t d0, int64_t m,
                            hipStream_t st);
hipError_t launch_store_rows_at(const float *rows, int dim, const int64_t *dstpos, const int64_t *new_ids, int64_t n,
                                const RowStore &index, uint32_t *irregular, hipStream_t st);
hipError_t launch_clear_rows(const RowStore &index, int64_t pos, int64_t n, hipStream_t st);
hipError_t launch_irregular_flag(const float *inv_norm, int64_t n, uint32_t *flag, hipStream_t st);

constexpr int BM25_RANGE = 16384;
constexpr int BM25_MAX_Q = 64;

struct Bm25Params {
    const int64_t *post_ptr;
    const int32_t *post_pos;
    const uint16_t *post_tf;
    const int32_t *doc_len;
    const int64_t *ids;
    const int32_t *q_ptr;
    const int32_t *q_term;
    const float *q_w;
    const uint32_t *mask;
    int64_t mask_stride_w;
    uint64_t *part_keys;
    int32_t *part_cnt;
    int64_t n;
    int n_ranges, nq, k;
    float avgdl;
    int64_t *out_ids;
    float *out_scores;
    int32_t *out_counts;
};
int64_t bm25_scratch_bytes(int64_t n_rows, int nq, int k);
hipError_t launch_bm25(const Bm25Params &p, hipStream_t st);


struct DedupeParams {
    const float *corpus;
    const float *inv_norm;
    const int64_t *stored;
    int64_t size;
    int piece_shift;
    const int64_t *ids;
    const int32_t *counts;
    int width;
    float threshold;
    int64_t *out_ids;
    int32_t *out_counts;
    int32_t *out_dup_of;
    float *out_sim;
};
hipError_t launch_dedupe(const DedupeParams &p, int nq, hipStream_t st);

struct SubsetParams {
    const float *corpus;
    const float *inv_norm;
    const int64_t *stored;
    int64_t size;
    int piece_shift;
    const float *queries;
    int nq, dim, k;
    const int64_t *ids;
    const int32_t *counts;
    int width;
    int64_t list_stride;
    uint64_t *keys;
    int64_t *out_ids;
    float *out_scores;
    int32_t *out_counts;
    float *out_slot_scores;
};
int64_t subset_scratch_bytes(int nq, int width);
hipError_t launch_subset(const SubsetParams &p, hipStream_t st);

struct GroupParams {
    const float *corpus;
    const float *inv_norm;
    const int64_t *stored;
    int64_t size;
    int piece_shift;
    const float *queries;
    int nq, dim, k;
    const int32_t *row_group;
    int64_t n_groups;
    int per_group;
    const uint32_t *mask;
    int64_t mask_stride_w;
    uint64_t *table;
    float *qinv;
    int64_t *out_ids;
    float *out_scores;
    int32_t *out_groups;
    int32_t *out_counts;
};
int64_t group_scratch_bytes(int nq, int64_t n_groups, int per_group);
hipError_t launch_grouped(const GroupParams &p, hipStream_t st);

}
```

### cadence_rag_amd/csrc/crag_search.hip

```cpp

#include <hip/hip_runtime.h>
#include <stdint.h>

#include <type_traits>

#include "crag_exact.h"
#include "crag_kernels.h"
#include "crag_layout.h"

namespace crag {

typedef float f32x16 __attribute__((ext_vector_type(16)));


template <int X>
__device__ __forceinline__ uint32_t swz_xor(uint32_t v) {
    return (uint32_t)__builtin_amdgcn_ds_swizzle((int)v, (X << 10) | 0x1f);
}

template <int X>
__device__ __forceinline__ void cmpx(uint32_t &hi, uint32_t &lo, bool want_max) {
    const uint32_t phi = swz_xor<X>(hi), plo = swz_xor<X>(lo);
    const bool keep = (mk64(hi, lo) > mk64(phi, plo)) == want_max;
    hi = keep ? hi : phi;
// ... 1059 lines not shown
        for (int o = 32; o > 0; o >>= 1) {
            const unsigned long long other = __shfl_xor(m, o);
            m = other > m ? other : m;
        }
        if ((tid & 63) == 0) wave_max[tid >> 6] = m;
    }
    __syncthreads();
    if (tid == 0) {
        unsigned long long m = wave_max[0];
        for (int i = 1; i < MERGE_THREADS / 64; ++i) m = wave_max[i] > m ? wave_max[i] : m;
        s_tau = m;
    }
    __syncthreads();
    if (use_heads) {
        const int n_pad = (n_lists + 7) & ~7;
        const ulonglong2 *h2 = reinterpret_cast<const ulonglong2 *>(heads);
        for (int l = tid; l < n_lists; l += MERGE_THREADS) {
            const uint64_t mine = heads[l];
            if (mine == 0ull) continue;
            int rank = 0;
            for (int i = 0; i < n_pad / 2; i += 4) {
                const ulonglong2 a0 = h2[i], a1 = h2[i + 1], a2 = h2[i + 2], a3 = h2[i + 3];
                rank += (a0.x > mine) + (a0.y > mine) + (a1.x > mine) + (a1.y > mine) + (a2.x > mine) +
                        (a2.y > mine) + (a3.x > mine) + (a3.y > mine);
            }
            if (rank == k - 1) atomicMax(&s_tau, (unsigned long long)mine);
        }
        __syncthreads();
    }
    const uint64_t tau = s_tau;

    for (int l = tid; l < n_lists; l += MERGE_THREADS) {
        const uint2 *lp = base + (size_t)l * lstride;
        for (int pos = 0; pos < k; ++pos) {
            uint64_t kk;
            if (l == tid && pos < LEAD) {
                kk = lead[0];
#pragma unroll
                for (int i = 1; i < LEAD; ++i)
                    if (pos == i) kk = lead[i];
            } else {
                kk = key_of(lp[pos]);
            }
            if (kk == 0ull || kk < tau) break;
            const int idx = atomicAdd(&s_cnt, 1);
            if (idx < MERGE_CAP) cand[idx] = kk;
        }
    }
    __syncthreads();
    int C = s_cnt;
    const bool in_lds = C <= MERGE_CAP;
    const uint64_t *src = cand;

    if (C > MERGE_RANK_MAX) {
        uint64_t prefix = 0ull, pmask = 0ull;
        int need = k;
        for (int pass = 0; pass < 8; ++pass) {
            const int shift = 56 - 8 * pass;
            hist[tid] = 0;
            __syncthreads();
            if (in_lds) {
                for (int e = tid; e < C; e += MERGE_THREADS) {
                    const uint64_t kk = cand[e];
                    if ((kk & pmask) == prefix) atomicAdd(&hist[(int)((kk >> shift) & 255ull)], 1);
                }
            } else {
                for (int e = tid; e < total; e += MERGE_THREADS) {
                    const int l = e / k, pos = e - l * k;
                    const uint64_t kk = key_of(base[(size_t)l * lstride + pos]);
                    if (kk >= tau && kk != 0ull && (kk & pmask) == prefix)
                        atomicAdd(&hist[(int)((kk >> shift) & 255ull)], 1);
                }
            }
            __syncthreads();
            {
                const int above = suffix_above(hist, wave_tot, tid);
                const int here = hist[tid];
                if (above < need && above + here >= need) {
                    s_digit = tid;
                    s_need = need - above;
                }
            }
            __syncthreads();
            prefix |= (uint64_t)s_digit << shift;
            pmask |= 255ull << shift;
            need = s_need;
            __syncthreads();
        }
        const uint64_t kth = prefix;
        if (tid == 0) s_cnt = 0;
        __syncthreads();
        if (in_lds) {
            for (int e = tid; e < C; e += MERGE_THREADS) {
                const uint64_t kk = cand[e];
                if (kk >= kth) {
                    const int idx = atomicAdd(&s_cnt, 1);
                    if (idx < CRAG_MAX_K_) win[idx] = kk;
                }
            }
        } else {
            for (int e = tid; e < total; e += MERGE_THREADS) {
                const int l = e / k, pos = e - l * k;
                const uint64_t kk = key_of(base[(size_t)l * lstride + pos]);
                if (kk != 0ull && kk >= kth) {
                    const int idx = atomicAdd(&s_cnt, 1);
                    if (idx < CRAG_MAX_K_) win[idx] = kk;
                }
            }
        }
        __syncthreads();
        C = s_cnt < CRAG_MAX_K_ ? s_cnt : CRAG_MAX_K_;
        src = win;
    }

    const int count = C < k ? C : k;
    for (int e = tid; e < C; e += MERGE_THREADS) {
        const uint64_t mine = src[e];
        int rank = 0;
        for (int i = 0; i < C; ++i) rank += (src[i] > mine) ? 1 : 0;
        if (rank < k) {
            const uint32_t row = ~(uint32_t)(mine & 0xffffffffull);
            p.out_scores[(size_t)q * k + rank] = ord2f((uint32_t)(mine >> 32));
            p.out_ids[(size_t)q * k + rank] = p.ids ? p.ids[row] : (int64_t)row + p.id_base;
        }
    }
    for (int r = count + tid; r < k; r += MERGE_THREADS) {
        p.out_scores[(size_t)q * k + r] = __uint_as_float(0x7fc00000u);
        p.out_ids[(size_t)q * k + r] = -1;
    }
    if (tid == 0) p.out_counts[q] = count;
    if (p.gbound && tid < GB_CELLS) p.gbound[(size_t)q * GB_CELLS + tid] = 0u;
}

__global__ __launch_bounds__(MERGE_THREADS) void merge_partials_kernel(MergeParams p) { merge_partials_body(p, blockIdx.x); }

constexpr int XMERGE_CAP = 4096;

__global__ __launch_bounds__(MERGE_THREADS) void merge_results_kernel(XMergeParams p) {
    __shared__ uint32_t s_sc[XMERGE_CAP];
    __shared__ int64_t s_id[XMERGE_CAP];
    __shared__ int s_cnt;
    const int q = blockIdx.x, tid = threadIdx.x, k = p.k;
    if (tid == 0) s_cnt = 0;
    __syncthreads();
    for (int e = tid; e < p.n_lists * k; e += MERGE_THREADS) {
        const int l = e / k, pos = e - l * k;
        const size_t src = (size_t)q * k + pos;
        const int cnt = p.counts[(size_t)l * p.stride_counts + q];
        const float sc = p.scores[(size_t)l * p.stride_scores + src];
        const int64_t id = p.ids[(size_t)l * p.stride_ids + src];
        if (pos < cnt) {
            const int idx = atomicAdd(&s_cnt, 1);
            s_sc[idx] = f2ord(sc);
            s_id[idx] = id;
        }
    }
    __syncthreads();
    const int C = s_cnt;
    const int count = C < k ? C : k;
    for (int e = tid; e < C; e += MERGE_THREADS) {
        const uint32_t ms = s_sc[e];
        const int64_t mi = s_id[e];
        int rank = 0;
        for (int i = 0; i < C; ++i) {
            const uint32_t os = s_sc[i];
            rank += (os > ms || (os == ms && s_id[i] < mi)) ? 1 : 0;
        }
        if (rank < k) {
            p.out_scores[(size_t)q * k + rank] = ord2f(ms);
            p.out_ids[(size_t)q * k + rank] = mi;
        }
    }
    for (int r = count + tid; r < k; r += MERGE_THREADS) {
        p.out_scores[(size_t)q * k + r] = __uint_as_float(0x7fc00000u);
        p.out_ids[(size_t)q * k + r] = -1;
    }
    if (tid == 0) p.out_counts[q] = count;
}

template <int PS>
__global__ __launch_bounds__(256) void store_rows_kernel(const float *rows, int dim, int64_t pos,
                                                         float *corpus, float *inv_norm, uint32_t *irregular,
                                                         _Float16 *mirror) {
    const int64_t i = blockIdx.x;
    store_row<PS>(rows + (size_t)i * dim, dim, pos + i, corpus, inv_norm, irregular, mirror);
}

template <int PS>
__global__ __launch_bounds__(256) void load_rows_kernel(const float *corpus, int dim, int64_t pos,
                                                        float *rows) {
    const int64_t i = blockIdx.x;
    const int kq = threadIdx.x;
    const int64_t row = pos + i;
    const float *src = corpus + (size_t)(row >> 5) * TILE_FLOATS + ((size_t)(kq >> PS) * 32 + (row & 31)) * (4 << PS) + (kq & ((1 << PS) - 1)) * 4;
    const f32x4 v = *reinterpret_cast<const f32x4 *>(src);
    float *dst = rows + (size_t)i * dim;
#pragma unroll
    for (int c = 0; c < 4; ++c)
        if (4 * kq + c < dim) dst[4 * kq + c] = v[c];
}

__global__ __launch_bounds__(256) void count_eligible_kernel(const float *inv_norm, int64_t n,
                                                             const uint32_t *mask,
                                                             unsigned long long *out) {
    unsigned long long c = 0;
    for (int64_t i = (int64_t)blockIdx.x * blockDim.x + threadIdx.x; i < n;
         i += (int64_t)gridDim.x * blockDim.x) {
        bool ok = inv_norm[i] > 0.f;
        if (ok && mask) ok = (mask[i >> 5] >> (i & 31)) & 1u;
        c += ok ? 1 : 0;
    }
    for (int o = 32; o > 0; o >>= 1) c += __shfl_xor(c, o);
    if ((threadIdx.x & 63) == 0 && c) atomicAdd(out, c);
}

__global__ void fill_ids_kernel(int64_t *ids, int64_t pos, int64_t n, int64_t first) {
    const int64_t i = (int64_t)blockIdx.x * blockDim.x + threadIdx.x;
    if (i < n) ids[pos + i] = first + i;
}

constexpr float PF_DELTA = 1.25e-3f;
constexpr int PF_FLUSH_ABOVE = 768;
constexpr int PF_STAGE = PF_FLUSH_ABOVE + 2048;
constexpr int PF_PER = (PF_STAGE + SCAN_THREADS - 1) / SCAN_THREADS;
constexpr int PF_TAU_CELL = 128;
constexpr int PF_STASH_MIRROR = 4;
constexpr int PF_STASH_ROWS = 2;

typedef _Float16 f16x8 __attribute__((ext_vector_type(8)));
typedef _Float16 f16x2 __attribute__((ext_vector_type(2)));
typedef float f32x2 __attribute__((ext_vector_type(2)));

__global__ __launch_bounds__(256) void prep_queries_kernel(PrepParams p) {
    __shared__ double sh[4];
    const int q = blockIdx.x, t = threadIdx.x;
    const f32x4 v = load_query_quad(p.queries, p.dim, q, p.nq, t);
    const float qinv = canonical_qinv(v, q < p.nq, sh);
    if (t == 0) p.qinv[q] = qinv;
    const int qb = q >> 5, i = q & 31, w = t >> 5, d = (4 * t) & 127;
    {
        const int sidx = d >> 3, h = (d >> 2) & 1;
        reinterpret_cast<f32x4 *>(p.a32)[((size_t)(qb * SCAN_WAVES + w) * 16 + sidx) * 64 + h * 32 + i] = v;
    }
    if (p.a16) {
        const int t8 = d >> 4, g = (d >> 3) & 1, h = (d >> 2) & 1;
        f32x2 lo = {v[0] * qinv, v[1] * qinv}, hi = {v[2] * qinv, v[3] * qinv};
        const f16x2 l2 = __builtin_convertvector(lo, f16x2), h2 = __builtin_convertvector(hi, f16x2);
        _Float16 *dst = p.a16 + ((((size_t)(qb * SCAN_WAVES + w) * 8 + t8) * 64 + h * 32 + i) * 8 + 4 * g);
        typedef _Float16 f16x4 __attribute__((ext_vector_type(4)));
        *reinterpret_cast<f16x4 *>(dst) = f16x4{l2[0], l2[1], h2[0], h2[1]};
    }
}

template <int X>
__device__ __forceinline__ uint32_t dpp_xor(uint32_t v, int lane) {
    if constexpr (X == 1) return (uint32_t)__builtin_amdgcn_mov_dpp((int)v, 0xB1, 0xF, 0xF, true);
    else if constexpr (X == 2) return (uint32_t)__builtin_amdgcn_mov_dpp((int)v, 0x4E, 0xF, 0xF, true);
    else if constexpr (X == 3) return (uint32_t)__builtin_amdgcn_mov_dpp((int)v, 0x1B, 0xF, 0xF, true);
    else if constexpr (X == 7) return (uint32_t)__builtin_amdgcn_mov_dpp((int)v, 0x141, 0xF, 0xF, true);
    else if constexpr (X == 15) return (uint32_t)__builtin_amdgcn_mov_dpp((int)v, 0x140, 0xF, 0xF, true);
    else if constexpr (X == 8) return (uint32_t)__builtin_amdgcn_mov_dpp((int)v, 0x128, 0xF, 0xF, true);
    else if constexpr (X == 4) {
        const uint32_t up = (uint32_t)__builtin_amdgcn_mov_dpp((int)v, 0x12C, 0xF, 0xF, true);
        const uint32_t dn = (uint32_t)__builtin_amdgcn_mov_dpp((int)v, 0x124, 0xF, 0xF, true);
        return (lane & 4) ? dn : up;
    } else return swz_xor<X>(v);
}

__device__ __forceinline__ uint32_t sort32_desc_u32(uint32_t v, int lane) {
#define CRAG_CX(X_, BIT_)                                              \
    {                                                                  \
        const uint32_t o_ = dpp_xor<X_>(v, lane);                      \
        const bool mx_ = !(lane & BIT_);                               \
        v = mx_ ? (o_ > v ? o_ : v) : (o_ < v ? o_ : v);               \
    }
    CRAG_CX(1, 1) CRAG_CX(3, 2) CRAG_CX(1, 1) CRAG_CX(7, 4) CRAG_CX(2, 2) CRAG_CX(1, 1) CRAG_CX(15, 8) CRAG_CX(4, 4)
    CRAG_CX(2, 2) CRAG_CX(1, 1) CRAG_CX(31, 16) CRAG_CX(8, 8) CRAG_CX(4, 4) CRAG_CX(2, 2) CRAG_CX(1, 1)
#undef CRAG_CX
    return v;
}

template <class F>
__device__ __forceinline__ uint32_t wave_reduce_u32(uint32_t v, int lane, F f) {
    v = f(v, dpp_xor<1>(v, lane));
    v = f(v, dpp_xor<2>(v, lane));
    v = f(v, dpp_xor<4>(v, lane));
    v = f(v, dpp_xor<8>(v, lane));
    const auto r16 = __builtin_amdgcn_permlane16_swap(v, v, false, false);
    v = f(r16[0], r16[1]);
    const auto r32 = __builtin_amdgcn_permlane32_swap(v, v, false, false);
    return f(r32[0], r32[1]);
}

template <int NQB>
struct PfLds {
    typedef float slab_t __attribute__((ext_vector_type(2 * NQB)));
    slab_t slab[2][SCAN_WAVES][SCAN_WAVES][64];
    uint2 stage[PF_STAGE];
    float qthr[32 * NQB];
    uint32_t qcount[32 * NQB], qbase[32 * NQB], qfill[32 * NQB];
    uint32_t n_stage;
    uint32_t need[NQB];
    uint32_t want_flush[2][SCAN_WAVES];
};

template <int NQB>
struct PfOwner {
    int ql0;
    int qg0;
    uint32_t okmask;
};

template <int NQB>
__device__ __forceinline__ void pf_stage(PfLds<NQB> &L, const PfOwner<NQB> &o, const float (&sc)[2 * NQB],
                                         const bool (&pass)[2 * NQB], uint32_t row_in_window, uint32_t *flags, uint32_t seq) {
#pragma unroll
    for (int e = 0; e < 2 * NQB; ++e) {
        if (pass[e]) {
            const uint32_t slot = atomicAdd(&L.n_stage, 1u);
            if (slot < (uint32_t)PF_STAGE) {
                L.stage[slot] = make_uint2(f2ord(sc[e]), (row_in_window << 6) | (uint32_t)(o.ql0 + e));
            } else {
                *flags = seq;
            }
        }
    }
}

template <int NQB, bool LAST>
__device__ __forceinline__ void pf_sift(const PfParams &p, PfLds<NQB> &L, int64_t window_row0) {
    __syncthreads();
    const uint32_t n = L.n_stage < (uint32_t)PF_STAGE ? L.n_stage : (uint32_t)PF_STAGE;
    const int tid = threadIdx.x;
    if (LAST && n == 0u) return;
    uint2 ent[PF_PER];
    bool keep[PF_PER];
#pragma unroll
    for (int i = 0; i < PF_PER; ++i) {
        const uint32_t idx = (uint32_t)tid + (uint32_t)i * SCAN_THREADS;
        keep[i] = false;
        if (idx < n) {
            ent[i] = L.stage[idx];
            keep[i] = ord2f(ent[i].x) >= L.qthr[ent[i].y & 63u];
        }
    }
    if (tid < 32 * NQB) {
        L.qcount[tid] = 0u;
        L.qfill[tid] = 0u;
    }
    __syncthreads();
    if (tid == 0) L.n_stage = 0u;
    __syncthreads();
#pragma unroll
    for (int i = 0; i < PF_PER; ++i)
        if (keep[i]) {
            atomicAdd(&L.qcount[ent[i].y & 63u], 1u);
            if (!LAST) L.stage[atomicAdd(&L.n_stage, 1u)] = ent[i];
        }
    __syncthreads();
    if constexpr (!LAST) {
        const uint32_t kept = L.n_stage;
        __syncthreads();
        if (kept <= (uint32_t)(PF_FLUSH_ABOVE / 2)) return;
    }
    if (tid < 32 * NQB) {
        const uint32_t cnt = L.qcount[tid];
        const int qg = (int)blockIdx.y * (32 * NQB) + tid;
        L.qbase[tid] = cnt ? atomicAdd(&p.count[qg], cnt) : 0u;
    }
    __syncthreads();
#pragma unroll
    for (int i = 0; i < PF_PER; ++i)
        if (keep[i]) {
            const uint32_t ql = ent[i].y & 63u;
            const uint32_t pos = L.qbase[ql] + atomicAdd(&L.qfill[ql], 1u);
            const int qg = (int)blockIdx.y * (32 * NQB) + (int)ql;
            if (pos < (uint32_t)p.cap) {
                p.cand[(size_t)qg * p.cap + pos] = make_uint2(ent[i].x, (uint32_t)(window_row0 + (int64_t)(ent[i].y >> 6)));
            } else {
                p.flags[0] = p.seq;
            }
        }
    if (LAST) return;
    __syncthreads();
    if (tid == 0) L.n_stage = 0u;
    __syncthreads();
}


__device__ __forceinline__ int pf_next_pub(int after, int n_tiles, int read_lag) {
    const int last = n_tiles >= 12 ? n_tiles - 4 : -1;
    const int np = after < 0 ? 0 : (after == 0 ? read_lag + 1 : after * 4 + 3);
    if (after < last && np + (np >> 2) >= last) return last;
    return (np < n_tiles) ? np : (1 << 30);
}

template <int NQB, int SETS, bool MIRROR, bool NT, bool FRAG>
__global__ __launch_bounds__(SCAN_THREADS) void prefilter_kernel(PfParams p) {
    static_assert(!FRAG || (MIRROR && !NT), "the per-fragment wait schedule exists for the cached mirror only");
    constexpr int RPO = 2 * NQB;
    constexpr int AUX = NT ? 2 : 0;
    __shared__ PfLds<NQB> L;
    ScanCtx c;
    c.lane = threadIdx.x & 63;
    c.w = __builtin_amdgcn_readfirstlane((int)(threadIdx.x >> 6));
    c.g = blockIdx.x;
    c.qb = blockIdx.y;
    c.j = c.lane & 31;
    c.h = c.lane >> 5;
    c.reverse = p.reverse != 0;
    constexpr int PS = PS_SMALL;
    c.lane_off = (uint32_t)(c.w * (KSLICE * 32 * 4) + c.j * (16 << PS) + c.h * 16);
    {
        const uint32_t nt = (uint32_t)((p.n_rows + 31) >> 5), G = (uint32_t)p.G, g = (uint32_t)c.g;
        const uint32_t qt = nt / G, rt = nt - qt * G;
        const uint32_t t0 = qt * g + (rt * g) / G, t1 = qt * (g + 1) + (rt * (g + 1)) / G;
        c.t_begin = t0;
        c.n_tiles = (int)(t1 - t0);
        c.r_begin = (int64_t)t0 * 32;
        c.r_end = (int64_t)t1 * 32 < p.n_rows ? (int64_t)t1 * 32 : p.n_rows;
    }
    const int lane = c.lane, w = c.w, j = c.j, h = c.h;

    constexpr int NB = MIRROR ? 8 : 16;
    constexpr uint32_t TILE_BYTES = MIRROR ? TILE_FLOATS * 2 : TILE_FLOATS * 4;
    const char *wg_base = MIRROR ? reinterpret_cast<const char *>(p.corpus16) + (size_t)c.t_begin * TILE_BYTES
                                 : reinterpret_cast<const char *>(p.corpus) + (size_t)c.t_begin * TILE_BYTES;
    const __amdgpu_buffer_rsrc_t rsrc = __builtin_amdgcn_make_buffer_rsrc(
        const_cast<char *>(wg_base), 0, (int)((uint32_t)c.n_tiles * TILE_BYTES), 0x00020000);
    const uint32_t lane_off = MIRROR ? (uint32_t)(w * (8 * 1024) + lane * 16) : c.lane_off;
    auto voff = [&](int step) -> uint32_t {
        const int t = tile_of(c, step);
        const int64_t r = (c.t_begin + t) * 32 + j;
        const bool valid = (step < c.n_tiles) && (r >= c.r_begin) && (r < c.r_end);
        return valid ? (uint32_t)t * TILE_BYTES + lane_off : 0x80000000u;
    };
    u32x4 b[NB];
    if constexpr (!FRAG) {
        const uint32_t v0 = voff(0);
#pragma unroll
        for (int s = 0; s < NB; ++s) b[s] = __builtin_amdgcn_raw_buffer_load_b128(rsrc, v0 + (MIRROR ? (uint32_t)s * 1024u : b_soff<PS>(s)), 0, AUX);
    }
    f16x8 a[NQB][8];
    PfOwner<NQB> o;
    {
        const int R = w * RPO, qb = R >> 4, r = R & 15;
        o.ql0 = qb * 32 + (r & 3) + 8 * (r >> 2) + 4 * h;
        o.qg0 = (int)blockIdx.y * (32 * NQB) + o.ql0;
        o.okmask = 0u;
    }
    {
        typedef float qv_t __attribute__((ext_vector_type(RPO)));
        qv_t qi;
        if constexpr (FRAG) qi = *reinterpret_cast<const qv_t *>(p.qinv + o.qg0);
#pragma unroll
        for (int qb = 0; qb < NQB; ++qb) {
            const f16x8 *af = reinterpret_cast<const f16x8 *>(p.a16) +
                              ((size_t)(((int)blockIdx.y * NQB + qb) * SCAN_WAVES + w) * 8) * 64 + lane;
#pragma unroll
            for (int t8 = 0; t8 < 8; ++t8) a[qb][t8] = af[t8 * 64];
        }
        if constexpr (FRAG) {
            __builtin_amdgcn_sched_barrier(0);
            const uint32_t v0 = voff(0);
#pragma unroll
            for (int s = 0; s < NB; ++s) b[s] = __builtin_amdgcn_raw_buffer_load_b128(rsrc, v0 + (uint32_t)s * 1024u, 0, AUX);
            __builtin_amdgcn_sched_barrier(0);
        } else {
            qi = *reinterpret_cast<const qv_t *>(p.qinv + o.qg0);
        }
#pragma unroll
        for (int e = 0; e < RPO; ++e)
            if (o.qg0 + e < p.nq && qi[e] > 0.f) o.okmask |= 1u << e;
    }
    if (threadIdx.x < 32 * NQB) L.qthr[threadIdx.x] = -__builtin_inff();
    if (threadIdx.x < NQB) L.need[threadIdx.x] = 0u;
    if (threadIdx.x == 0) L.n_stage = 0u;
    constexpr int PF_STASH = MIRROR ? PF_STASH_MIRROR : PF_STASH_ROWS;
    float stash[PF_STASH][RPO];
#pragma unroll
    for (int t = 0; t < PF_STASH; ++t)
#pragma unroll
        for (int e = 0; e < RPO; ++e) stash[t][e] = __uint_as_float(0x7fc00000u);
    float thr[RPO];
    uint32_t tau[RPO];
    uint32_t lmax[RPO][SETS];
    uint32_t dirty = 0u;
#pragma unroll
    for (int e = 0; e < RPO; ++e) {
        thr[e] = -__builtin_inff();
        tau[e] = 0u;
#pragma unroll
        for (int s = 0; s < SETS; ++s) lmax[e][s] = 0u;
    }
    float inv_cur = 1.f;
    if (!MIRROR && c.n_tiles > 0) inv_cur = p.inv_norm[(c.t_begin + tile_of(c, 0)) * 32 + j];
    if constexpr (!FRAG) __builtin_amdgcn_s_waitcnt(0x0F70);
    __syncthreads();

    const int k_base = p.k / SETS, k_rem = p.k % SETS;
    const f32x16 zero16 = f32x16{0, 0, 0, 0, 0, 0, 0, 0, 0, 0, 0, 0, 0, 0, 0, 0};
    uint32_t *const gb_row = p.gbound + (size_t)o.qg0 * PF_BOUND_CELLS + j;
    const uint32_t *const idle_row = p.gbound_idle + (size_t)c.g * PF_BOUND_CELLS + j;

    auto load_taus = [&](uint32_t (&tq)[RPO]) {
#pragma unroll
        for (int e = 0; e < RPO; ++e) {
            const bool live = (o.okmask >> e) & 1u;
            tq[e] = __hip_atomic_load(live ? gb_row - j + e * PF_BOUND_CELLS + PF_TAU_CELL : idle_row - j + PF_TAU_CELL,
                                      __ATOMIC_RELAXED, __HIP_MEMORY_SCOPE_AGENT);
        }
    };
    auto take_taus = [&](const uint32_t (&tq)[RPO]) {
#pragma unroll
        for (int e = 0; e < RPO; ++e)
            if (tq[e] > tau[e]) {
                tau[e] = tq[e];
                thr[e] = ord2f(tq[e]) - 2.f * PF_DELTA;
                if (j == 0) L.qthr[o.ql0 + e] = thr[e];
            }
    };
    auto any_without_bound = [&]() -> bool {
        bool none = false;
#pragma unroll
        for (int e = 0; e < RPO; ++e) none = none || (((o.okmask >> e) & 1u) && tau[e] == 0u);
        return __builtin_amdgcn_ballot_w64(none) != 0ull;
    };
    constexpr int DS = SETS >= 2 ? SETS / 2 : 1;
    auto load_cells = [&](int dq, uint32_t (&cell)[DS]) {
        const uint32_t *rec = p.gbound + (size_t)((int)blockIdx.y * (32 * NQB) + dq) * PF_BOUND_CELLS;
#pragma unroll
        for (int i = 0; i < DS; ++i)
            cell[i] = __hip_atomic_load(rec + (SETS >= 2 ? 2 * i + h : 0) * 32 + j, __ATOMIC_RELAXED, __HIP_MEMORY_SCOPE_AGENT);
    };
    auto derive_cells = [&](int dq, const uint32_t (&cell)[DS]) {
        uint32_t t = 0xffffffffu;
#pragma unroll
        for (int i = 0; i < DS; ++i) {
            const uint32_t sorted = sort32_desc_u32(cell[i], lane);
            const int sset = SETS >= 2 ? 2 * i + h : 0;
            const int ks = k_base + (sset < k_rem ? 1 : 0);
            const uint32_t kth = (uint32_t)__shfl((int)sorted, (lane & 32) | (ks - 1));
            t = kth < t ? kth : t;
        }
        if constexpr (SETS >= 2) {
            const uint32_t other = (uint32_t)__shfl((int)t, lane ^ 32);
            t = other < t ? other : t;
        }
        if (lane == 0 && t != 0u)
            (void)__hip_atomic_fetch_max(p.gbound + (size_t)((int)blockIdx.y * (32 * NQB) + dq) * PF_BOUND_CELLS + PF_TAU_CELL, t,
                                         __ATOMIC_RELAXED, __HIP_MEMORY_SCOPE_AGENT);
    };
    auto derive_own = [&]() {
#pragma unroll
        for (int e = 0; e < RPO; ++e) {
            const bool live = (o.okmask >> e) & 1u;
            uint32_t t = 0xffffffffu;
#pragma unroll
            for (int s = 0; s < SETS; ++s) {
                const uint32_t v = __hip_atomic_load(live ? gb_row + e * PF_BOUND_CELLS + s * 32 : idle_row + s * 32,
                                                     __ATOMIC_RELAXED, __HIP_MEMORY_SCOPE_AGENT);
                const uint32_t sorted = sort32_desc_u32(v, lane);
                const int ks = k_base + (s < k_rem ? 1 : 0);
                const uint32_t kth = (uint32_t)__shfl((int)sorted, (lane & 32) | (ks - 1));
                t = kth < t ? kth : t;
            }
            if (t > tau[e]) {
                tau[e] = t;
                thr[e] = ord2f(t) - 2.f * PF_DELTA;
                if (j == 0) L.qthr[o.ql0 + e] = thr[e];
            }
        }
    };

    const int PF_DERIVE_LAG = p.derive_lag, PF_READ_LAG = p.read_lag;
    int pub_at = pf_next_pub(-1, c.n_tiles, PF_READ_LAG);
    int der_base = pub_at, rd_base = pub_at;
    int next_read = rd_base + PF_READ_LAG;
    const int dq0 = c.g % (32 * NQB);
    int buf = 0;
    uint32_t tq_end[RPO];
    for (int ti = 0; ti < c.n_tiles; ++ti) {
        const uint32_t vnext = voff(ti + 1);
        const int64_t tile = c.t_begin + tile_of(c, ti);
        const int64_t row = tile * 32 + j;
        const bool rd = ti == next_read;
        const bool dv = (w == 0) && (ti == der_base + PF_DERIVE_LAG);
        float inv_nxt = 1.f;
        if constexpr (!MIRROR) inv_nxt = p.inv_norm[(c.t_begin + tile_of(c, ti + 1 < c.n_tiles ? ti + 1 : ti)) * 32 + j];
        uint32_t mword[RPO], tq[RPO], cell[DS];
#pragma unroll
        for (int e = 0; e < RPO; ++e)
            mword[e] = p.mask ? p.mask[(size_t)(((o.okmask >> e) & 1u) ? o.qg0 + e : 0) * (size_t)p.mask_stride_w + tile]
                              : 0xffffffffu;
        if (rd) load_taus(tq);
        if (dv) load_cells(dq0, cell);
        if constexpr (!FRAG) __builtin_amdgcn_s_waitcnt(0x0F70);

        f32x16 acc[NQB];
        static_for<0, 8>([&](auto T) {
            constexpr int t8 = decltype(T)::value;
            f16x8 bf;
            if constexpr (MIRROR) {
                bf = __builtin_bit_cast(f16x8, b[t8]);
            } else {
                const f32x4 lo = __builtin_bit_cast(f32x4, b[2 * t8]) * inv_cur;
                const f32x4 hi = __builtin_bit_cast(f32x4, b[2 * t8 + 1]) * inv_cur;
                const f16x2 p0 = __builtin_convertvector((f32x2{lo[0], lo[1]}), f16x2);
                const f16x2 p1 = __builtin_convertvector((f32x2{lo[2], lo[3]}), f16x2);
                const f16x2 p2 = __builtin_convertvector((f32x2{hi[0], hi[1]}), f16x2);
                const f16x2 p3 = __builtin_convertvector((f32x2{hi[2], hi[3]}), f16x2);
                bf = f16x8{p0[0], p0[1], p1[0], p1[1], p2[0], p2[1], p3[0], p3[1]};
            }
#pragma unroll
            for (int qb = 0; qb < NQB; ++qb)
                acc[qb] = __builtin_amdgcn_mfma_f32_32x32x16_f16(a[qb][t8], bf, t8 == 0 ? zero16 : acc[qb], 0, 0, AUX);
            if constexpr (MIRROR) {
                b[t8] = __builtin_amdgcn_raw_buffer_load_b128(rsrc, vnext + t8 * 1024, 0, AUX);
            } else {
                b[2 * t8] = __builtin_amdgcn_raw_buffer_load_b128(rsrc, vnext + b_soff<PS>(2 * t8), 0, AUX);
                b[2 * t8 + 1] = __builtin_amdgcn_raw_buffer_load_b128(rsrc, vnext + b_soff<PS>(2 * t8 + 1), 0, AUX);
            }
            __builtin_amdgcn_sched_barrier(0);
        });
#pragma unroll
        for (int ow = 0; ow < SCAN_WAVES; ++ow) {
            typename PfLds<NQB>::slab_t v;
#pragma unroll
            for (int e = 0; e < RPO; ++e) v[e] = acc[(ow * RPO + e) >> 4][(ow * RPO + e) & 15];
            L.slab[buf][ow][w][lane] = v;
        }
        if (lane == 0) L.want_flush[buf][w] = L.n_stage > (uint32_t)PF_FLUSH_ABOVE ? 1u : 0u;
        __syncthreads();
        if constexpr (FRAG) {
            if (ti == c.n_tiles - 1) load_taus(tq_end);
        }
        {
            const u32x4 f0 = *reinterpret_cast<const u32x4 *>(&L.want_flush[buf][0]);
            const u32x4 f1 = *reinterpret_cast<const u32x4 *>(&L.want_flush[buf][4]);
            if ((f0[0] | f0[1] | f0[2] | f0[3] | f1[0] | f1[1] | f1[2] | f1[3]) != 0u) pf_sift<NQB, false>(p, L, c.t_begin * 32);
        }
        float sc[RPO];
#pragma unroll
        for (int e = 0; e < RPO; ++e) sc[e] = 0.f;
#pragma unroll
        for (int ww = 0; ww < SCAN_WAVES; ++ww) {
            const typename PfLds<NQB>::slab_t v = L.slab[buf][w][ww][lane];
#pragma unroll
            for (int e = 0; e < RPO; ++e) sc[e] += v[e];
        }
        buf ^= 1;
        if (dv) {
            derive_cells(dq0, cell);
            for (int dq = dq0 + p.G; dq < 32 * NQB; dq += p.G) {
                uint32_t more[DS];
                load_cells(dq, more);
                derive_cells(dq, more);
            }
        }
        if (ti == der_base + PF_DERIVE_LAG) der_base = pf_next_pub(der_base, c.n_tiles, PF_READ_LAG);
        if constexpr (MIRROR) {
            uint32_t need[NQB];
#pragma unroll
            for (int i = 0; i < NQB; ++i) need[i] = __builtin_amdgcn_readfirstlane((int)L.need[i]);
            bool any = false;
#pragma unroll
            for (int i = 0; i < NQB; ++i) any = any || need[i] != 0u;
            if (any) {
#pragma unroll
                for (int i = 0; i < NQB; ++i) {
                    uint32_t mine = need[i] & (0x01010101u << w);
                    while (mine) {
                        const int b = __builtin_ctz(mine);
                        mine &= mine - 1u;
                        uint32_t more[DS];
                        load_cells(32 * i + b, more);
                        derive_cells(32 * i + b, more);
                    }
                    if (lane == 0 && (need[i] & (0x01010101u << w))) atomicAnd(&L.need[i], ~(need[i] & (0x01010101u << w)));
                }
            }
        }
        if (rd) {
            take_taus(tq);
            if (any_without_bound()) {
                if constexpr (MIRROR) {
                    if (j == 0) {
#pragma unroll
                        for (int e = 0; e < RPO; ++e)
                            if (((o.okmask >> e) & 1u) && tau[e] == 0u) atomicOr(&L.need[(o.ql0 + e) >> 5], 1u << ((o.ql0 + e) & 31));
                    }
                }
                next_read = ti + 1;
            } else {
                rd_base = pf_next_pub(rd_base, c.n_tiles, PF_READ_LAG);
                while (rd_base + PF_READ_LAG <= ti) rd_base = pf_next_pub(rd_base, c.n_tiles, PF_READ_LAG);
                next_read = rd_base + PF_READ_LAG;
            }
        }
        const bool row_ok = (row >= c.r_begin) && (row < c.r_end) && (inv_cur > 0.f);
        const int set = __builtin_amdgcn_readfirstlane((int)(tile & (int64_t)(SETS - 1)));
        bool pass[RPO];
        uint32_t ord[RPO];
#pragma unroll
        for (int e = 0; e < RPO; ++e) {
            const bool ok = row_ok && ((o.okmask >> e) & 1u) && ((mword[e] >> j) & 1u) && (sc[e] == sc[e]);
            sc[e] = ok ? sc[e] : __uint_as_float(0x7fc00000u);
            ord[e] = ok ? f2ord(sc[e]) : 0u;
            pass[e] = sc[e] >= thr[e];
        }
#pragma unroll
        for (int s = 0; s < SETS; ++s)
            if (s == set) {
#pragma unroll
                for (int e = 0; e < RPO; ++e)
                    if (ord[e] > lmax[e][s]) {
                        lmax[e][s] = ord[e];
                        dirty |= 1u << (e * SETS + s);
                    }
            }
        if (ti < PF_STASH) {
#pragma unroll
            for (int t = 0; t < PF_STASH; ++t)
                if (ti == t) {
#pragma unroll
                    for (int e = 0; e < RPO; ++e) stash[t][e] = sc[e];
                }
        } else {
            pf_stage<NQB>(L, o, sc, pass, (uint32_t)(row - c.t_begin * 32), p.flags, p.seq);
        }
        if (ti == pub_at) {
#pragma unroll
            for (int e = 0; e < RPO; ++e) {
                uint32_t first_cut = 0u;
                if (ti == 0) {
                    uint32_t v0 = lmax[e][0];
#pragma unroll
                    for (int s = 1; s < SETS; ++s) v0 = (s == set) ? lmax[e][s] : v0;
                    if constexpr (SETS == 1) first_cut = half_max_u32(v0);
                    else first_cut = (uint32_t)__shfl((int)sort32_desc_u32(v0, lane), (lane & 32) | (p.pub0 - 1));
                }
#pragma unroll
                for (int s = 0; s < SETS; ++s) {
                    const uint32_t v = lmax[e][s];
                    const bool lift = ((dirty >> (e * SETS + s)) & 1u) && v > tau[e] && v >= first_cut;
                    if (lift)
                        (void)__hip_atomic_fetch_max(gb_row + e * PF_BOUND_CELLS + s * 32, v, __ATOMIC_RELAXED,
                                                     __HIP_MEMORY_SCOPE_AGENT);
                }
            }
            dirty = 0u;
            pub_at = pf_next_pub(pub_at, c.n_tiles, PF_READ_LAG);
        }
        inv_cur = inv_nxt;
    }
    if (c.n_tiles > 0) {
        {
            if constexpr (FRAG) {
                take_taus(tq_end);
            } else {
                uint32_t tq[RPO];
                load_taus(tq);
                take_taus(tq);
            }
            if (any_without_bound()) derive_own();
        }
        const bool unbounded = any_without_bound();
        auto sift_if_full = [&](bool post_unbounded) -> bool {
            if (lane == 0) L.want_flush[buf][w] = (L.n_stage > (uint32_t)PF_FLUSH_ABOVE ? 1u : 0u) | (post_unbounded ? 2u : 0u);
            __syncthreads();
            const u32x4 f0 = *reinterpret_cast<const u32x4 *>(&L.want_flush[buf][0]);
            const u32x4 f1 = *reinterpret_cast<const u32x4 *>(&L.want_flush[buf][4]);
            buf ^= 1;
            const uint32_t f = f0[0] | f0[1] | f0[2] | f0[3] | f1[0] | f1[1] | f1[2] | f1[3];
            if ((f & 1u) != 0u) pf_sift<NQB, false>(p, L, c.t_begin * 32);
            return (f & 2u) != 0u;
        };
        const bool careful = sift_if_full(unbounded);
#pragma unroll
        for (int t = 0; t < PF_STASH; ++t) {
            if (careful && t > 0) (void)sift_if_full(false);
            bool pass[RPO];
#pragma unroll
            for (int e = 0; e < RPO; ++e) pass[e] = stash[t][e] >= thr[e];
            pf_stage<NQB>(L, o, stash[t], pass, (uint32_t)(tile_of(c, t) * 32 + j), p.flags, p.seq);
        }
    }
    pf_sift<NQB, true>(p, L, c.t_begin * 32);
}

constexpr int FIN_SKIP_BITS = 12;
constexpr int FIN_THREADS = SCAN_THREADS;
constexpr int FIN_ROUND = 4096;
constexpr int FIN_BEST = FIN_ROUND + 128;


struct FinLds {
    uint64_t best[FIN_BEST];
    uint2 lcand[FIN_ROUND];
    uint32_t surv[FIN_ROUND];
    f32x4 qs[SCAN_WAVES][16][2];
    int64_t best_id[FIN_BEST];
    unsigned long long hist[64];
    int s_nbest, s_nsurv, s_rescored;
    uint32_t s_kth;
};
union FinFbLds {
    FinLds f;
    float2 slab[2][SCAN_WAVES][8][64];
};

template <int S, int PS>
__global__ __launch_bounds__(SCAN_THREADS) void finalize_fb_kernel(FinParams p) {
    __shared__ FinFbLds U;
    __shared__ int s_last;
    const int wave = __builtin_amdgcn_readfirstlane((int)(threadIdx.x >> 6));
    const int R = p.rsplit;
    if ((int)blockIdx.x >= p.nq * R) {
        if (__hip_atomic_load(p.flags, __ATOMIC_RELAXED, __HIP_MEMORY_SCOPE_AGENT) != p.seq) return;
        const int b = (int)blockIdx.x - p.nq * R;
        scan_body<S, PS>(p.scan, b % p.scan.G, b / p.scan.G, U.slab);
        asm volatile("s_waitcnt vmcnt(0)" ::: "memory");
        __syncthreads();
        if (threadIdx.x == 0) {
            __builtin_amdgcn_fence(__ATOMIC_RELEASE, "agent");
            asm volatile("s_waitcnt vmcnt(0)" ::: "memory");
            const uint32_t t = __hip_atomic_fetch_add(p.fb_done, 1u, __ATOMIC_RELAXED, __HIP_MEMORY_SCOPE_AGENT);
            s_last = (t == (uint32_t)(p.fb_blocks - 1)) ? 1 : 0;
            if (s_last) {
                __builtin_amdgcn_fence(__ATOMIC_ACQUIRE, "agent");
                asm volatile("s_waitcnt vmcnt(0)" ::: "memory");
            }
        }
        __syncthreads();
        if (!s_last || wave >= MERGE_THREADS / 64) return;
        for (int q = 0; q < p.nq; ++q) {
            merge_partials_body(p.merge, q);
            __syncthreads();
        }
        if (threadIdx.x == 0) __hip_atomic_store(p.fb_done, 0u, __ATOMIC_RELAXED, __HIP_MEMORY_SCOPE_AGENT);
        return;
    }
#define FIN_T(PH_)                                                                                               \
    do {                                                                                                         \
        if (p.trace && (int)blockIdx.x < R && threadIdx.x == 0) p.trace[((int)blockIdx.x % R) * 16 + (PH_)] = wall_clock64(); \
    } while (0)
    FIN_T(0);
    constexpr int NT = FIN_THREADS;
    auto &best = U.f.best;
    auto &lcand = U.f.lcand;
    auto &surv = U.f.surv;
    auto &qs = U.f.qs;
    auto &best_id = U.f.best_id;
    auto &hist = U.f.hist;
    int &s_nbest = U.f.s_nbest, &s_nsurv = U.f.s_nsurv, &s_rescored = U.f.s_rescored;
    uint32_t &s_kth = U.f.s_kth;
    const int q = (int)blockIdx.x / R, rpart = (int)blockIdx.x % R, tid = threadIdx.x;
    const uint2 *gcand = p.cand + (size_t)q * p.cap;
    const bool overflow = p.flags[0] == p.seq;
    const uint32_t total = p.count[q];
    const uint2 first = gcand[tid];
    const float qinv = p.qinv[q];
    f32x4 qfrag = f32x4{0.f, 0.f, 0.f, 0.f};
    if (tid < 256)
        qfrag = reinterpret_cast<const f32x4 *>(p.a32)[((size_t)((q >> 5) * SCAN_WAVES + (tid >> 5)) * 16 + ((tid >> 1) & 15)) * 64 + (tid & 1) * 32 + (q & 31)];
    unsigned long long *const stat = p.stats ? p.stats + (size_t)(q % (PF_STAT_SLOTS / PF_STAT_WS)) * 3 : nullptr;
    unsigned long long stat_old[3] = {0ull, 0ull, 0ull};
    if (stat && tid == 0 && R == 1) {
        stat_old[0] = stat[0];
        stat_old[1] = stat[1];
        stat_old[2] = stat[2];
    }
    if (tid < PF_BOUND_CELLS && rpart == 0) p.gbound[(size_t)q * PF_BOUND_CELLS + tid] = 0u;
    if (overflow) {
        if (tid == 0 && rpart == 0) p.count[q] = 0u;
        return;
    }
    const int k = p.k;
    const int C = (int)(total < (uint32_t)p.cap ? total : (uint32_t)p.cap);
    const bool in_lds = C <= FIN_ROUND;
    if (tid < C) lcand[tid] = first;
    if (in_lds)
        for (int e = tid + NT; e < C; e += NT) lcand[e] = gcand[e];
    if (tid < 256) qs[tid >> 5][(tid >> 1) & 15][tid & 1] = qfrag;
    if (tid == 0) {
        s_nbest = 0;
        s_rescored = 0;
        s_kth = 0u;
    }
    __syncthreads();
    if (tid == 0 && R == 1) p.count[q] = 0u;
    FIN_T(1);

    uint32_t thr_ord = 0u;
    if (C > k) {
        if (C <= 64) {
            if (tid < C) {
                const uint32_t mine = lcand[tid].x;
                int rank = 0;
                for (int i = 0; i < C; ++i) {
                    const uint32_t o = lcand[i].x;
                    rank += (o > mine || (o == mine && i < tid)) ? 1 : 0;
                }
                if (rank == k - 1) s_kth = mine & ~((1u << FIN_SKIP_BITS) - 1u);
            }
            __syncthreads();
        } else {
            const int ln = tid & 63;
            uint32_t vmax = 0u, vmin = 0xffffffffu;
            if (in_lds) {
                for (int e = tid; e < C; e += NT) {
                    const uint32_t o = lcand[e].x;
                    vmax = o > vmax ? o : vmax;
                    vmin = o < vmin ? o : vmin;
                }
            } else {
                for (int e = tid; e < C; e += NT) {
                    const uint32_t o = gcand[e].x;
                    vmax = o > vmax ? o : vmax;
                    vmin = o < vmin ? o : vmin;
                }
            }
            vmax = wave_reduce_u32(vmax, ln, [](uint32_t x, uint32_t y) { return x > y ? x : y; });
            vmin = wave_reduce_u32(vmin, ln, [](uint32_t x, uint32_t y) { return x < y ? x : y; });
            uint32_t *const cnts = reinterpret_cast<uint32_t *>(hist);
            uint32_t *const xch = surv;
            (void)cnts;
            if (ln == 0) {
                xch[wave] = vmax;
                xch[8 + wave] = vmin;
            }
            __syncthreads();
#pragma unroll
            for (int i = 0; i < NT / 64; ++i) {
                const uint32_t a = xch[i], b = xch[8 + i];
                vmax = a > vmax ? a : vmax;
                vmin = b < vmin ? b : vmin;
            }
            const uint32_t diff = vmax ^ vmin;
            const int top0 = diff ? 32 - __builtin_clz(diff) : 0;
            const int top = top0 > FIN_SKIP_BITS ? top0 : FIN_SKIP_BITS;
            uint32_t ans = top >= 32 ? 0u : (vmax >> top) << top;
            int round = 0;
            const int digit_of = ln & 15, subset = (ln >> 4) + 4 * wave;
            for (int bit = top; bit > FIN_SKIP_BITS; ++round) {
                const int nb = bit - FIN_SKIP_BITS >= 4 ? 4 : bit - FIN_SKIP_BITS, lo = bit - nb;
                const uint32_t t = ans | ((uint32_t)digit_of << lo);
                uint32_t c = 0u;
                if (in_lds) {
                    int e = subset;
                    for (; e + 3 * 32 < C; e += 4 * 32) {
                        const uint32_t x0 = lcand[e].x, x1 = lcand[e + 32].x, x2 = lcand[e + 64].x, x3 = lcand[e + 96].x;
                        c += (x0 >= t ? 1u : 0u) + (x1 >= t ? 1u : 0u) + (x2 >= t ? 1u : 0u) + (x3 >= t ? 1u : 0u);
                    }
                    for (; e < C; e += 32) c += lcand[e].x >= t ? 1u : 0u;
                } else {
                    for (int e = subset; e < C; e += 32) c += gcand[e].x >= t ? 1u : 0u;
                }
                {
                    const auto r16 = __builtin_amdgcn_permlane16_swap(c, c, false, false);
                    c = r16[0] + r16[1];
                    const auto r32 = __builtin_amdgcn_permlane32_swap(c, c, false, false);
                    c = r32[0] + r32[1];
                }
                uint32_t *const slot = xch + 16 + (round & 1) * 128;
                if (ln < 16) slot[wave * 16 + ln] = c;
                __syncthreads();
                uint32_t total = 0u;
#pragma unroll
                for (int wv = 0; wv < NT / 64; ++wv) total += slot[wv * 16 + digit_of];
                const unsigned long long reach =
                    __builtin_amdgcn_ballot_w64((int)total >= k && ln >= 1 && ln < (1 << nb) && ln < 16);
                const uint32_t digit = reach ? 63u - (uint32_t)__builtin_clzll(reach) : 0u;
                ans |= digit << lo;
                bit = lo;
            }
            if (tid == 0) s_kth = ans;
            __syncthreads();
        }
        thr_ord = f2ord(ord2f(s_kth) - 2.f * PF_DELTA);
    }
    FIN_T(2);

    const int grp = tid >> 3, sub = tid & 7;
    for (int r0 = 0; r0 < C; r0 += FIN_ROUND) {
        const int rn = (C - r0) < FIN_ROUND ? (C - r0) : FIN_ROUND;
        if (tid == 0) s_nsurv = 0;
        __syncthreads();
        for (int e = tid; e < rn; e += NT) {
            const uint2 ce = in_lds ? lcand[e] : gcand[r0 + e];
            if (ce.x >= thr_ord && (((r0 + e) & (R - 1)) == rpart)) surv[atomicAdd(&s_nsurv, 1)] = ce.y;
        }
        __syncthreads();
        const int ns = s_nsurv;
        for (int e0 = 0; e0 < ns; e0 += NT / 8) {
            const int e = e0 + grp;
            const bool live = e < ns;
            const uint32_t row = live ? surv[e] : 0u;
            float part = 0.f, inv_row = 0.f;
            int64_t rid = -1;
            if (live) {
                if (sub == 0) {
                    inv_row = p.inv_norm[row];
                    rid = p.ids ? p.ids[row] : (int64_t)row;
                }
                const f32x4 *ctile = reinterpret_cast<const f32x4 *>(p.corpus + (size_t)(row >> 5) * TILE_FLOATS) + (size_t)sub * 32 * 32;
                part = exact_slice_dot<PS>(&qs[sub][0][0], ctile, (int)(row & 31u));
            }
            float d = __shfl(part, (tid & 63 & ~7) | 0);
#pragma unroll
            for (int ww = 1; ww < 8; ++ww) d += __shfl(part, (tid & 63 & ~7) | ww);
            if (live && sub == 0) {
                const float scale = inv_row * qinv;
                float sc = d * scale;
                sc = __builtin_amdgcn_fmed3f(sc, -1.f, 1.f);
                if (scale > 0.f && sc == sc) {
                    const uint32_t u = __float_as_uint(sc);
                    const uint32_t ord = u ^ ((uint32_t)((int32_t)u >> 31) | 0x80000000u);
                    const int slot = atomicAdd(&s_nbest, 1);
                    best[slot] = mk64(ord, ~row);
                    best_id[slot] = rid;
                }
            }
        }
        __syncthreads();
        if (tid == 0) s_rescored += ns;
        if (r0 + FIN_ROUND < C && s_nbest > k) {
            const int B = s_nbest;
            uint64_t mine[(FIN_BEST + NT - 1) / NT];
            int64_t mine_id[(FIN_BEST + NT - 1) / NT];
            int rank[(FIN_BEST + NT - 1) / NT];
            int n_mine = 0;
            for (int e = tid; e < B; e += NT) {
                const uint64_t m = best[e];
                int rk = 0;
                for (int i = 0; i < B; ++i) rk += (best[i] > m) ? 1 : 0;
                mine[n_mine] = m;
                mine_id[n_mine] = best_id[e];
                rank[n_mine++] = rk;
            }
            __syncthreads();
            for (int e = 0; e < n_mine; ++e)
                if (rank[e] < k) {
                    best[rank[e]] = mine[e];
                    best_id[rank[e]] = mine_id[e];
                }
            if (tid == 0) s_nbest = k;
            __syncthreads();
        }
    }

    FIN_T(3);
    int B = s_nbest;
    unsigned long long rescored_all = (unsigned long long)s_rescored;
    if (R > 1) {
        uint64_t *const xk = p.xkeys + ((size_t)q * R + rpart) * k;
        int64_t *const xi = p.xids + ((size_t)q * R + rpart) * k;
        if (B <= k) {
            for (int e = tid; e < B; e += NT) {
                xk[e] = best[e];
                xi[e] = best_id[e];
            }
        } else {
            for (int e = tid; e < B; e += NT) {
                const uint64_t mine = best[e];
                int rank = 0;
                for (int i = 0; i < B; ++i) rank += (best[i] > mine) ? 1 : 0;
                if (rank < k) {
                    xk[rank] = mine;
                    xi[rank] = best_id[e];
                }
            }
        }
        if (tid == 0) p.xcount[(size_t)q * R + rpart] = make_uint2((uint32_t)(B < k ? B : k), (uint32_t)s_rescored);
        asm volatile("s_waitcnt vmcnt(0)" ::: "memory");
        __syncthreads();
        if (tid == 0) {
            __builtin_amdgcn_fence(__ATOMIC_RELEASE, "agent");
            asm volatile("s_waitcnt vmcnt(0)" ::: "memory");
            const uint32_t t = __hip_atomic_fetch_add(p.xticket + q, 1u, __ATOMIC_RELAXED, __HIP_MEMORY_SCOPE_AGENT);
            s_last = (t == (uint32_t)(R - 1)) ? 1 : 0;
            if (s_last) {
                __builtin_amdgcn_fence(__ATOMIC_ACQUIRE, "agent");
                asm volatile("s_waitcnt vmcnt(0)" ::: "memory");
            }
        }
        __syncthreads();
        FIN_T(4);
        if (!s_last) return;
        const int per = NT / R, rr_mine = tid / per, e_mine = tid % per;
        const uint2 cr_mine = p.xcount[(size_t)q * R + rr_mine];
        uint64_t k_mine = 0ull;
        int64_t i_mine = -1;
        if (e_mine < k) {
            k_mine = p.xkeys[((size_t)q * R + rr_mine) * k + e_mine];
            i_mine = p.xids[((size_t)q * R + rr_mine) * k + e_mine];
        }
        if (e_mine == 0) hist[48 + rr_mine] = ((unsigned long long)cr_mine.y << 32) | cr_mine.x;
        __syncthreads();
        int base = 0, base_mine = 0;
        rescored_all = 0ull;
        for (int rr = 0; rr < R; ++rr) {
            const unsigned long long c2 = hist[48 + rr];
            if (rr == rr_mine) base_mine = base;
            base += (int)(uint32_t)c2;
            rescored_all += c2 >> 32;
        }
        if (e_mine < (int)cr_mine.x) {
            best[base_mine + e_mine] = k_mine;
            best_id[base_mine + e_mine] = i_mine;
        }
        for (int e = e_mine + per; e < (int)cr_mine.x; e += per) {
            best[base_mine + e] = p.xkeys[((size_t)q * R + rr_mine) * k + e];
            best_id[base_mine + e] = p.xids[((size_t)q * R + rr_mine) * k + e];
        }
        B = base;
        if (tid == 0) {
            __hip_atomic_store(p.xticket + q, 0u, __ATOMIC_RELAXED, __HIP_MEMORY_SCOPE_AGENT);
            p.count[q] = 0u;
            if (stat) {
                stat_old[0] = stat[0];
                stat_old[1] = stat[1];
                stat_old[2] = stat[2];
            }
        }
        __syncthreads();
        FIN_T(5);
    }
    const int count = B < k ? B : k;
    for (int e = tid; e < B; e += NT) {
        const uint64_t mine = best[e];
        int rank = 0;
        for (int i = 0; i < B; ++i) rank += (best[i] > mine) ? 1 : 0;
        if (rank < k) {
            p.out_scores[(size_t)q * k + rank] = ord2f((uint32_t)(mine >> 32));
            p.out_ids[(size_t)q * k + rank] = best_id[e];
        }
    }
    for (int r = count + tid; r < k; r += NT) {
        p.out_scores[(size_t)q * k + r] = __uint_as_float(0x7fc00000u);
        p.out_ids[(size_t)q * k + r] = -1;
    }
    if (tid == 0) {
        p.out_counts[q] = count;
        if (stat) {
            stat[0] = stat_old[0] + (unsigned long long)total;
            stat[1] = stat_old[1] + rescored_all;
            if (q == 0) stat[2] = stat_old[2] + 1ull;
        }
    }
    FIN_T(6);
    if (p.trace && (int)blockIdx.x < R && threadIdx.x == 0) {
        p.trace[rpart * 16 + 8] = (unsigned long long)C;
        p.trace[rpart * 16 + 9] = (unsigned long long)s_rescored;
    }
#undef FIN_T
}

__global__ __launch_bounds__(256) void check_ids_kernel(const int64_t *ids, int64_t n, int64_t prev,
                                                        unsigned long long *out_bad) {
    unsigned long long c = 0;
    for (int64_t i = (int64_t)blockIdx.x * blockDim.x + threadIdx.x; i < n; i += (int64_t)gridDim.x * blockDim.x) {
        const int64_t before = i ? ids[i - 1] : prev;
        c += ids[i] <= before ? 1 : 0;
    }
    for (int o = 32; o > 0; o >>= 1) c += __shfl_xor(c, o);
    if ((threadIdx.x & 63) == 0 && c) atomicAdd(out_bad, c);
}

hipError_t launch_scan(const ScanParams &p, int q_blocks, hipStream_t st, const char **kernel_name) {
    dim3 grid(p.G, q_blocks), block(SCAN_THREADS);
    const int ks = p.k <= 32 ? 1 : (p.k <= 64 ? 2 : 4);
    const char *name;
#define CRAG_LAUNCH(GRID_, ...)                                       \
    do {                                                              \
        name = "crag::" #__VA_ARGS__;                                 \
        hipLaunchKernelGGL((__VA_ARGS__), GRID_, block, 0, st, p);    \
    } while (0)
    const bool big = p.piece_shift == PS_BIG;
#define CRAG_LAUNCH_PS(GRID_, K_, ...)                                          \
    do {                                                                        \
        if (big) CRAG_LAUNCH(GRID_, K_<__VA_ARGS__, PS_BIG>);                    \
        else CRAG_LAUNCH(GRID_, K_<__VA_ARGS__, PS_SMALL>);                      \
    } while (0)
    if (p.unpipelined) {
        if (ks == 1) CRAG_LAUNCH_PS(grid, scan_kernel, 1);
        else if (ks == 2) CRAG_LAUNCH_PS(grid, scan_kernel, 2);
        else CRAG_LAUNCH_PS(grid, scan_kernel, 4);
    } else if (p.wide) {
        const dim3 g2(p.G, q_blocks / 2);
        if (ks == 1) CRAG_LAUNCH_PS(g2, scan_pipe2_kernel, 1, 2);
        else if (ks == 2) CRAG_LAUNCH_PS(g2, scan_pipe2_kernel, 2, 2);
        else CRAG_LAUNCH_PS(g2, scan_pipe2_kernel, 4, 2);
    } else if (ks == 1) {
        if (big) CRAG_LAUNCH(grid, scan_pipe_kernel<PS_BIG>);
        else CRAG_LAUNCH(grid, scan_pipe_kernel<PS_SMALL>);
    } else if (ks == 2) {
        CRAG_LAUNCH_PS(grid, scan_pipe2_kernel, 2, 1);
    } else {
        CRAG_LAUNCH_PS(grid, scan_pipe2_kernel, 4, 1);
    }
#undef CRAG_LAUNCH_PS
#undef CRAG_LAUNCH
    if (kernel_name) *kernel_name = name;
    return hipGetLastError();
}

hipError_t launch_prep_queries(const PrepParams &p, int nq_pad, hipStream_t st) {
    hipLaunchKernelGGL(prep_queries_kernel, dim3(nq_pad), dim3(256), 0, st, p);
    return hipGetLastError();
}

hipError_t launch_prefilter(const PfParams &p, int nqb, int passes, int frag_waits, hipStream_t st,
                            const char **kernel_name) {
    const dim3 grid(p.G, passes), block(SCAN_THREADS);
    const char *name = "";
#define CRAG_LAUNCH(...) hipLaunchKernelGGL((__VA_ARGS__), grid, block, 0, st, p)
    const bool mirror = p.corpus16 != nullptr;
#define CRAG_PICK(NQB_, SETS_)                                                                     \
    do {                                                                                            \
        if (mirror && p.nt) {                                                                       \
            name = "crag::prefilter_kernel<" #NQB_ ", " #SETS_ ", true, true>";                      \
            CRAG_LAUNCH(prefilter_kernel<NQB_, SETS_, true, true, false>);                           \
        } else if (mirror) {                                                                        \
            name = "crag::prefilter_kernel<" #NQB_ ", " #SETS_ ", true, false>";                     \
            if (frag_waits) CRAG_LAUNCH(prefilter_kernel<NQB_, SETS_, true, false, true>);           \
            else CRAG_LAUNCH(prefilter_kernel<NQB_, SETS_, true, false, false>);                     \
        } else {                                                                                    \
            name = "crag::prefilter_kernel<" #NQB_ ", " #SETS_ ", false, false>";                    \
            CRAG_LAUNCH(prefilter_kernel<NQB_, SETS_, false, false, false>);                         \
        }                                                                                           \
    } while (0)
    if (nqb == 2) {
        if (p.sets == 1) CRAG_PICK(2, 1);
        else if (p.sets == 2) CRAG_PICK(2, 2);
        else CRAG_PICK(2, 4);
    } else {
        if (p.sets == 1) CRAG_PICK(1, 1);
        else if (p.sets == 2) CRAG_PICK(1, 2);
        else CRAG_PICK(1, 4);
    }
#undef CRAG_PICK
#undef CRAG_LAUNCH
    if (kernel_name) *kernel_name = name;
    return hipGetLastError();
}

hipError_t launch_finalize(const FinParams &p, hipStream_t st) {
    const dim3 grid(p.nq * p.rsplit + p.fb_blocks), block(SCAN_THREADS);
    const int ks = (p.k + 31) / 32;
    if (p.scan.piece_shift == PS_BIG) {
        if (ks == 1) hipLaunchKernelGGL((finalize_fb_kernel<1, PS_BIG>), grid, block, 0, st, p);
        else if (ks == 2) hipLaunchKernelGGL((finalize_fb_kernel<2, PS_BIG>), grid, block, 0, st, p);
        else hipLaunchKernelGGL((finalize_fb_kernel<4, PS_BIG>), grid, block, 0, st, p);
    } else {
        if (ks == 1) hipLaunchKernelGGL((finalize_fb_kernel<1, PS_SMALL>), grid, block, 0, st, p);
        else if (ks == 2) hipLaunchKernelGGL((finalize_fb_kernel<2, PS_SMALL>), grid, block, 0, st, p);
        else hipLaunchKernelGGL((finalize_fb_kernel<4, PS_SMALL>), grid, block, 0, st, p);
    }
    return hipGetLastError();
}

hipError_t launch_merge_partials(const MergeParams &p, int nq, hipStream_t st) {
    hipLaunchKernelGGL(merge_partials_kernel, dim3(nq), dim3(MERGE_THREADS), 0, st, p);
    return hipGetLastError();
}

hipError_t launch_merge_results(const XMergeParams &p, hipStream_t st) {
    hipLaunchKernelGGL(merge_results_kernel, dim3(p.nq), dim3(MERGE_THREADS), 0, st, p);
    return hipGetLastError();
}

hipError_t launch_store_rows(const float *rows, int dim, int64_t pos, int64_t n, float *corpus,
                             float *inv_norm, uint32_t *irregular, _Float16 *mirror, hipStream_t st) {
    if (n <= 0) return hipSuccess;
    if (mirror) hipLaunchKernelGGL(store_rows_kernel<PS_BIG>, dim3((unsigned)n), dim3(256), 0, st, rows, dim, pos, corpus,
                                   inv_norm, irregular, mirror);
    else hipLaunchKernelGGL(store_rows_kernel<PS_SMALL>, dim3((unsigned)n), dim3(256), 0, st, rows, dim, pos, corpus,
                       inv_norm, irregular, mirror);
    return hipGetLastError();
}

hipError_t launch_load_rows(const float *corpus, int dim, int64_t pos, int64_t n, float *rows, int piece_shift,
                            hipStream_t st) {
    if (n <= 0) return hipSuccess;
    if (piece_shift == PS_BIG) hipLaunchKernelGGL(load_rows_kernel<PS_BIG>, dim3((unsigned)n), dim3(256), 0, st, corpus, dim, pos, rows);
    else hipLaunchKernelGGL(load_rows_kernel<PS_SMALL>, dim3((unsigned)n), dim3(256), 0, st, corpus, dim, pos, rows);
    return hipGetLastError();
}

hipError_t launch_count_eligible(const float *inv_norm, int64_t n, const uint32_t *mask,
                                 unsigned long long *out, hipStream_t st) {
    hipLaunchKernelGGL(count_eligible_kernel, dim3(1024), dim3(256), 0, st, inv_norm, n, mask, out);
    return hipGetLastError();
}

hipError_t launch_check_ids(const int64_t *ids, int64_t n, int64_t prev, unsigned long long *out_bad,
                            hipStream_t st) {
    if (n <= 0) return hipSuccess;
    const int64_t blocks = (n + 255) / 256;
    hipLaunchKernelGGL(check_ids_kernel, dim3((unsigned)(blocks < 1024 ? blocks : 1024)), dim3(256), 0, st, ids, n,
                       prev, out_bad);
    return hipGetLastError();
}

hipError_t launch_fill_ids(int64_t *ids, int64_t pos, int64_t n, int64_t first, hipStream_t st) {
    if (n <= 0) return hipSuccess;
    hipLaunchKernelGGL(fill_ids_kernel, dim3((unsigned)((n + 255) / 256)), dim3(256), 0, st, ids, pos, n,
                       first);
    return hipGetLastError();
}

}
```

### cadence_rag_amd/csrc/crag_search_plan.h

```cpp
#pragma once
#include <stdint.h>

#include <algorithm>

#include "crag_kernels.h"

struct SearchSwitches {
    int no_wide = 0;
    int no_prefilter = 0;
    int no_rsplit = 0;
    int pf_derive_lag = 2, pf_read_lag = 4;
    int pf_nt = -1;
    int64_t nt_above_bytes = 1536ll << 20;
    int pf_waits = -1;
};

struct SearchPlan {
    int wide;
    int q_blocks;
    int nq_pad;
    int G;
    int prefilter;
    int cap;
    int rsplit;
    int nb;
    int pub_rank;
    int sets;
    int pub0;
    int derive_lag, read_lag;
    int nt;
    int fb_blocks;
    int window_too_large;
};

inline SearchPlan plan_search(int64_t size, int n_cu, int nq, int k, bool has_mirror, bool irregular,
                              const SearchSwitches &sw) {
    SearchPlan pl;
    pl.wide = (nq > 32 && !sw.no_wide) ? 1 : 0;
    pl.q_blocks = pl.wide ? ((nq + 63) / 64) * 2 : (nq + 31) / 32;
    pl.nq_pad = pl.q_blocks * 32;
    pl.G = (int)std::max<int64_t>(1, std::min<int64_t>(n_cu, (size + 7) / 8));
    pl.prefilter = (!sw.no_prefilter && !irregular && size >= (int64_t)pl.G * crag::PF_MIN_ROWS_PER_GROUP &&
                    (pl.wide || nq <= 32)) ? 1 : 0;
    pl.cap = (k > 104 && pl.nq_pad <= 128) ? 32768 : 8192;
    pl.rsplit = (k <= 32 || sw.no_rsplit) ? 1 : (nq <= 16 ? 8 : (nq <= 128 ? 4 : 1));
    pl.nb = k < crag::GB_CELLS ? k : crag::GB_CELLS;
    pl.pub_rank = (k + pl.nb - 1) / pl.nb - 1;
    pl.sets = k <= 24 ? 1 : (k <= 56 ? 2 : 4);
    pl.pub0 = (k + pl.sets - 1) / pl.sets >= 27 ? 8 : pl.sets;
    pl.derive_lag = has_mirror ? sw.pf_derive_lag : 1;
    pl.read_lag = has_mirror ? sw.pf_read_lag : 2;
    pl.nt = !has_mirror ? 0 : (sw.pf_nt >= 0 ? sw.pf_nt : (size * (int64_t)crag::DIM * 2 > sw.nt_above_bytes ? 1 : 0));
    pl.fb_blocks = pl.G * ((nq + 31) / 32);
    const int64_t rows_per_g = (size + pl.G - 1) / pl.G + 64;
    pl.window_too_large = rows_per_g * (int64_t)(crag::DIM * 4) >= (int64_t)0x7ff00000 ? 1 : 0;
    return pl;
}

inline int pf_waits_for(int64_t mirror_bytes, bool has_mirror, int nt, int pf_waits_switch) {
    if (!has_mirror || nt) return crag::PF_WAITS_TILE;
    if (pf_waits_switch >= 0) return pf_waits_switch ? crag::PF_WAITS_FRAGMENT : crag::PF_WAITS_TILE;
    return mirror_bytes <= crag::PF_FRAG_WAITS_MAX_BYTES ? crag::PF_WAITS_FRAGMENT : crag::PF_WAITS_TILE;
}
```

### cadence_rag_amd/dense_index.py

```python
from __future__ import annotations

import ctypes
from typing import Optional, Tuple

import numpy as np

from . import _native

try:
    import torch
except Exception:
    torch = None


def _is_torch(x) -> bool:
    return torch is not None and isinstance(x, torch.Tensor)


def _as_f32_2d(x, dim: int, what: str):
    if _is_torch(x):
        t = x
        if t.dtype != torch.float32:
            t = t.to(torch.float32)
        if t.dim() == 1:
# ... 96 lines not shown
        return int(size.value)

    def insert(self, vectors, ids) -> None:
        ptr, n, keep = _as_f32_2d(vectors, self.dim, "vectors")
        ids_ptr, _, keep_ids = self._ids_arg(ids, n)
        _native.check(self._lib.crag_index_insert(self._h, ptr, ids_ptr, n), "crag_index_insert")
        del keep, keep_ids

    def get_rows(self, pos: int, n: int) -> Tuple[np.ndarray, np.ndarray]:
        rows = np.empty((n, self.dim), dtype=np.float32)
        ids = np.empty((n,), dtype=np.int64)
        _native.check(self._lib.crag_index_get_rows(self._h, int(pos), int(n), rows.ctypes.data,
                                                    ids.ctypes.data), "crag_index_get_rows")
        return rows, ids

    def get_rows_into(self, pos: int, n: int, d_rows) -> np.ndarray:
        if tuple(d_rows.shape) != (n, self.dim) or not d_rows.is_contiguous() or d_rows.dtype != torch.float32:
            raise ValueError(f"d_rows must be a contiguous float32 [{n}, {self.dim}] tensor")
        ids = np.empty((n,), dtype=np.int64)
        if n:
            _native.check(self._lib.crag_index_get_rows(self._h, int(pos), int(n), d_rows.data_ptr(),
                                                        ids.ctypes.data), "crag_index_get_rows")
        return ids

    @staticmethod
    def pack_mask(eligible) -> np.ndarray:
        e = np.asarray(eligible, dtype=bool)
        packed = np.packbits(e, axis=-1, bitorder="little")
        pad = (-packed.shape[-1]) % 4
        if pad:
            width = [(0, 0)] * (packed.ndim - 1) + [(0, pad)]
            packed = np.pad(packed, width)
        return np.ascontiguousarray(packed)

    @staticmethod
    def _mask_arg(row_mask):
        if _is_torch(row_mask):
            if row_mask.dtype != torch.uint8 or not row_mask.is_cuda or not row_mask.is_contiguous():
                raise ValueError("a tensor row_mask must be a contiguous uint8 CUDA tensor")
            return (row_mask.data_ptr() or None), row_mask
        row_mask = np.ascontiguousarray(np.asarray(row_mask, dtype=np.uint8))
        return row_mask.ctypes.data, row_mask

    def count_eligible(self, row_mask=None) -> int:
        out = ctypes.c_int64(0)
        ptr = None
        if row_mask is not None:
            ptr, row_mask = self._mask_arg(row_mask)
            if row_mask.shape[-1] < ((len(self) + 31) // 32) * 4 and _is_torch(row_mask):
                raise ValueError("a device row_mask needs ceil(size/32)*4 bytes")
        _native.check(self._lib.crag_index_count_eligible(self._h, ptr, ctypes.byref(out)),
                      "crag_index_count_eligible")
        return int(out.value)

    def search(self, queries, k: int, row_mask=None) -> Tuple[np.ndarray, np.ndarray, np.ndarray]:
        ptr, nq, keep = _as_f32_2d(queries, self.dim, "queries")
        if not 1 <= int(k) <= _native.CRAG_MAX_K:
            raise ValueError(f"k must be in [1, {_native.CRAG_MAX_K}] (got {k})")
        out_ids = np.empty((nq, k), dtype=np.int64)
        out_scores = np.empty((nq, k), dtype=np.float32)
        out_counts = np.empty((nq,), dtype=np.int32)
        mptr, stride = None, 0
        if row_mask is not None:
            mptr, row_mask = self._mask_arg(row_mask)
            need = ((len(self) + 31) // 32) * 4
            if row_mask.shape[-1] < need:
                raise ValueError(f"row_mask needs {need} bytes per row (use pack_mask)")
            if row_mask.ndim == 2:
                if row_mask.shape[0] != nq:
                    raise ValueError("per-query row_mask must have one row per query")
                stride = int(row_mask.shape[1])
                if stride % 4:
                    raise ValueError("row_mask row stride must be a multiple of 4 bytes")
        _native.check(self._lib.crag_index_search(self._h, ptr, nq, int(k), mptr, stride,
                                                  out_ids.ctypes.data, out_scores.ctypes.data,
                                                  out_counts.ctypes.data), "crag_index_search")
        del keep
        return out_ids, out_scores, out_counts

    def search_async(self, d_queries, k: int, d_out_ids, d_out_scores, d_out_counts,
                     d_row_mask=None, mask_stride: int = 0, stream: int = 0) -> None:
        nq = int(d_queries.shape[0])
        _native.check(self._lib.crag_index_search_async(
            self._h, d_queries.data_ptr(), nq, int(k),
            None if d_row_mask is None else d_row_mask.data_ptr(), int(mask_stride),
            d_out_ids.data_ptr(), d_out_scores.data_ptr(), d_out_counts.data_ptr(),
            ctypes.c_void_p(stream)), "crag_index_search_async")

    def search_pipelined(self, d_queries, k: int, d_out_ids, d_out_scores, d_out_counts,
                         d_row_mask=None, mask_stride: int = 0, stream: int = 0, inputs_ready: bool = False) -> None:
        nq = int(d_queries.shape[0])
        _native.check(self._lib.crag_index_search_pipelined(
            self._h, d_queries.data_ptr(), nq, int(k),
            None if d_row_mask is None else d_row_mask.data_ptr(), int(mask_stride),
            d_out_ids.data_ptr(), d_out_scores.data_ptr(), d_out_counts.data_ptr(),
            ctypes.c_void_p(stream), 1 if inputs_ready else 0), "crag_index_search_pipelined")

    def join(self, stream: int = 0) -> None:
        _native.check(self._lib.crag_index_join(self._h, ctypes.c_void_p(stream)), "crag_index_join")

    def dedupe_async(self, d_ids, d_counts, threshold: float, d_out_ids, d_out_counts, d_out_dup_of=None,
                     d_out_sim=None, stream: int = 0) -> None:
        if d_ids.dim() != 2:
            raise ValueError("d_ids must have shape [nq, width]")
        nq, width = int(d_ids.shape[0]), int(d_ids.shape[1])
        _native.check(self._lib.crag_index_dedupe_async(
            self._h, d_ids.data_ptr(), d_counts.data_ptr(), nq, width, float(threshold), d_out_ids.data_ptr(),
            d_out_counts.data_ptr(), None if d_out_dup_of is None else d_out_dup_of.data_ptr(),
            None if d_out_sim is None else d_out_sim.data_ptr(), ctypes.c_void_p(stream)), "crag_index_dedupe_async")

    def dedupe(self, ids, threshold: float):
        if torch is None:
            raise _native.NativeLibraryError("DenseIndex.dedupe stages its buffers with torch")
        single = len(ids) == 0 or np.ndim(ids[0]) == 0
        lists = [np.asarray(ids, dtype=np.int64).reshape(-1)] if single else \
            [np.asarray(l, dtype=np.int64).reshape(-1) for l in ids]
        width = max([int(l.size) for l in lists] + [1])
        if width > _native.CRAG_DEDUPE_MAX_WIDTH:
            raise ValueError(f"a list holds at most {_native.CRAG_DEDUPE_MAX_WIDTH} ids (got {width})")
        h_ids = np.full((len(lists), width), -1, dtype=np.int64)
        for q, l in enumerate(lists):
            h_ids[q, :l.size] = l
        dev = torch.device("cuda", self.device)
        d_ids = torch.from_numpy(h_ids).to(dev)
        d_ct = torch.tensor([int(l.size) for l in lists], dtype=torch.int32, device=dev)
        d_out = torch.empty_like(d_ids)
        d_oct = torch.empty_like(d_ct)
        d_dup = torch.empty(len(lists), width, dtype=torch.int32, device=dev)
        d_sim = torch.empty(len(lists), width, dtype=torch.float32, device=dev)
        self.dedupe_async(d_ids, d_ct, threshold, d_out, d_oct, d_dup, d_sim,
                          stream=torch.cuda.current_stream(dev).cuda_stream)
        dup, sim = d_dup.cpu().numpy(), d_sim.cpu().numpy()
        res = [(np.flatnonzero(dup[q, :l.size] < 0).astype(np.int64), dup[q, :l.size].copy(), sim[q, :l.size].copy())
               for q, l in enumerate(lists)]
        if single:
            return res[0]
        return [r[0] for r in res], [r[1] for r in res], [r[2] for r in res]

    @staticmethod
    def search_ids_scratch_bytes(nq: int, width: int) -> int:
        return int(_native.load().crag_index_search_ids_scratch_bytes(int(nq), int(width)))

    def search_ids_async(self, d_queries, d_ids, d_counts, k: int, d_out_ids, d_out_scores, d_out_counts,
                         d_out_slot_scores=None, shared: bool = False, scratch=None, stream: int = 0) -> None:
        nq = int(d_queries.shape[0])
        if d_ids.dim() != (1 if shared else 2) or (not shared and int(d_ids.shape[0]) != nq):
            raise ValueError("d_ids must have shape [nq, width], or [width] with shared=True")
        width = int(d_ids.shape[-1])
        if scratch is None:
            scratch = torch.empty(self.search_ids_scratch_bytes(nq, width), dtype=torch.uint8, device=d_ids.device)
        _native.check(self._lib.crag_index_search_ids_async(
            self._h, d_queries.data_ptr(), nq, d_ids.data_ptr(), d_counts.data_ptr(), width, 0 if shared else width,
            int(k), d_out_ids.data_ptr(), d_out_scores.data_ptr(), d_out_counts.data_ptr(),
            None if d_out_slot_scores is None else d_out_slot_scores.data_ptr(), scratch.data_ptr(),
            int(scratch.numel()) * scratch.element_size(), ctypes.c_void_p(stream)), "crag_index_search_ids_async")

    def search_ids(self, queries, ids, k: int, slot_scores: bool = False):
        if torch is None:
            raise _native.NativeLibraryError("DenseIndex.search_ids stages its buffers with torch")
        ptr, nq, keep = _as_f32_2d(queries, self.dim, "queries")
        if not 1 <= int(k) <= _native.CRAG_MAX_K:
            raise ValueError(f"k must be in [1, {_native.CRAG_MAX_K}] (got {k})")
        shared = len(ids) == 0 or np.ndim(ids[0]) == 0
        lists = [np.asarray(ids, dtype=np.int64).reshape(-1)] if shared else \
            [np.asarray(l, dtype=np.int64).reshape(-1) for l in ids]
        if not shared and len(lists) != nq:
            raise ValueError("per-query id lists must have one list per query")
        width = max([int(l.size) for l in lists] + [1])
        if width > _native.CRAG_SUBSET_MAX_WIDTH:
            raise ValueError(f"a list holds at most {_native.CRAG_SUBSET_MAX_WIDTH} ids (got {width}): use a row_mask")
        h_ids = np.full((len(lists), width), -1, dtype=np.int64)
        for q, l in enumerate(lists):
            h_ids[q, :l.size] = l
        dev = torch.device("cuda", self.device)
        d_q = keep.to(dev) if _is_torch(keep) else torch.from_numpy(keep).to(dev)
        d_ids = torch.from_numpy(h_ids[0] if shared else h_ids).to(dev)
        d_ct = torch.tensor([int(l.size) for l in lists], dtype=torch.int32, device=dev)
        out_ids = torch.empty(nq, int(k), dtype=torch.int64, device=dev)
        out_sc = torch.empty(nq, int(k), dtype=torch.float32, device=dev)
        out_ct = torch.empty(nq, dtype=torch.int32, device=dev)
        slot = torch.empty(nq, width, dtype=torch.float32, device=dev) if slot_scores else None
        if nq:
            self.search_ids_async(d_q, d_ids, d_ct, k, out_ids, out_sc, out_ct, slot, shared=shared,
                                  stream=torch.cuda.current_stream(dev).cuda_stream)
        res = (out_ids.cpu().numpy(), out_sc.cpu().numpy(), out_ct.cpu().numpy())
        return res + (slot.cpu().numpy(),) if slot_scores else res

    GROUPED_SCRATCH_LIMIT = 256 << 20

    @staticmethod
    def search_grouped_scratch_bytes(nq: int, n_groups: int, per_group: int) -> int:
        return int(_native.load().crag_index_search_grouped_scratch_bytes(int(nq), int(n_groups), int(per_group)))

    def search_grouped_async(self, d_queries, k: int, d_row_group, n_groups: int, per_group: int, d_out_ids,
                             d_out_scores, d_out_counts, d_out_groups=None, d_row_mask=None, mask_stride: int = 0,
                             scratch=None, stream: int = 0) -> None:
        nq = int(d_queries.shape[0])
        if scratch is None:
            scratch = torch.empty(self.search_grouped_scratch_bytes(nq, n_groups, per_group), dtype=torch.uint8,
                                  device=d_queries.device)
        _native.check(self._lib.crag_index_search_grouped_async(
            self._h, d_queries.data_ptr(), nq, int(k), d_row_group.data_ptr(), int(n_groups), int(per_group),
            None if d_row_mask is None else d_row_mask.data_ptr(), int(mask_stride), d_out_ids.data_ptr(),
            d_out_scores.data_ptr(), None if d_out_groups is None else d_out_groups.data_ptr(), d_out_counts.data_ptr(),
            scratch.data_ptr(), int(scratch.numel()) * scratch.element_size(), ctypes.c_void_p(stream)),
            "crag_index_search_grouped_async")

    def search_grouped(self, queries, k: int, row_group, n_groups: int, per_group: int, row_mask=None):
        if torch is None:
            raise _native.NativeLibraryError("DenseIndex.search_grouped stages its buffers with torch")
        _, nq, keep = _as_f32_2d(queries, self.dim, "queries")
        k, n_groups, per_group = int(k), int(n_groups), int(per_group)
        if not 1 <= k <= _native.CRAG_MAX_K:
            raise ValueError(f"k must be in [1, {_native.CRAG_MAX_K}] (got {k})")
        if not 1 <= per_group <= _native.CRAG_GROUP_MAX_PER:
            raise ValueError(f"per_group must be in [1, {_native.CRAG_GROUP_MAX_PER}] (got {per_group})")
        if not 1 <= n_groups < 1 << 31:
            raise ValueError(f"n_groups must be in [1, 2^31) (got {n_groups})")
        if nq == 0 or len(self) == 0:
            return (np.full((nq, k), -1, dtype=np.int64), np.full((nq, k), np.nan, dtype=np.float32),
                    np.full((nq, k), -1, dtype=np.int32), np.zeros((nq,), dtype=np.int32))
        dev = torch.device("cuda", self.device)

        def on_device(x, dtype):
            t = x if _is_torch(x) else torch.from_numpy(np.ascontiguousarray(x))
            return t.to(device=dev, dtype=dtype).contiguous()

        d_q = on_device(keep, torch.float32)
        d_grp = on_device(row_group, torch.int32).reshape(-1)
        if int(d_grp.numel()) != len(self):
            raise ValueError(f"row_group needs one entry per stored row ({len(self)}, got {int(d_grp.numel())})")
        d_mask, stride = None, 0
        if row_mask is not None:
            d_mask = on_device(row_mask, torch.uint8)
            need = ((len(self) + 31) // 32) * 4
            if d_mask.shape[-1] < need:
                raise ValueError(f"row_mask needs {need} bytes per row (use pack_mask)")
            if d_mask.dim() == 2:
                if d_mask.shape[0] != nq:
                    raise ValueError("per-query row_mask must have one row per query")
                stride = int(d_mask.shape[1])
                if stride % 4:
                    raise ValueError("row_mask row stride must be a multiple of 4 bytes")
        out_ids = torch.empty(nq, k, dtype=torch.int64, device=dev)
        out_sc = torch.empty(nq, k, dtype=torch.float32, device=dev)
        out_grp = torch.empty(nq, k, dtype=torch.int32, device=dev)
        out_ct = torch.empty(nq, dtype=torch.int32, device=dev)
        per_query = self.search_grouped_scratch_bytes(2, n_groups, per_group) - \
            self.search_grouped_scratch_bytes(1, n_groups, per_group)
        step = max(1, min(65535, self.GROUPED_SCRATCH_LIMIT // max(per_query + 8, 1)))
        stream = torch.cuda.current_stream(dev).cuda_stream
        scratch = None
        for q0 in range(0, nq, step):
            q1 = min(nq, q0 + step)
            if scratch is None:
                scratch = torch.empty(self.search_grouped_scratch_bytes(q1 - q0, n_groups, per_group), dtype=torch.uint8,
                                      device=dev)
            self.search_grouped_async(d_q[q0:q1], k, d_grp, n_groups, per_group, out_ids[q0:q1], out_sc[q0:q1],
                                      out_ct[q0:q1], out_grp[q0:q1],
                                      d_row_mask=None if d_mask is None else (d_mask[q0:q1] if stride else d_mask),
                                      mask_stride=stride, scratch=scratch, stream=stream)
        return out_ids.cpu().numpy(), out_sc.cpu().numpy(), out_grp.cpu().numpy(), out_ct.cpu().numpy()

    def profile_enable(self, every: int = 1) -> None:
        _native.check(self._lib.crag_index_profile_enable(self._h, int(every)), "profile_enable")

    def profile_read(self) -> Tuple[int, float, float]:
        n = ctypes.c_int64(0)
        scan = ctypes.c_double(0.0)
        merge = ctypes.c_double(0.0)
        _native.check(self._lib.crag_index_profile_read(self._h, ctypes.byref(n), ctypes.byref(scan),
                                                        ctypes.byref(merge)), "profile_read")
        return int(n.value), float(scan.value), float(merge.value)

    def profile_read_ex(self) -> Tuple[int, float, float, float]:
        n = ctypes.c_int64(0)
        scan, merge, pair = ctypes.c_double(0.0), ctypes.c_double(0.0), ctypes.c_double(0.0)
        _native.check(self._lib.crag_index_profile_read_ex(self._h, ctypes.byref(n), ctypes.byref(scan),
                                                           ctypes.byref(merge), ctypes.byref(pair)), "profile_read_ex")
        return int(n.value), float(scan.value), float(merge.value), float(pair.value)

    def prefilter_stats(self) -> dict:
        a, b, c = ctypes.c_int64(0), ctypes.c_int64(0), ctypes.c_int64(0)
        _native.check(self._lib.crag_index_prefilter_stats(self._h, ctypes.byref(a), ctypes.byref(b),
                                                           ctypes.byref(c)), "prefilter_stats")
        return {"searches": a.value, "candidates": b.value, "rescored_rows": c.value}

    def phase_trace(self):
        buf = (ctypes.c_uint64 * 128)()
        _native.check(self._lib.crag_index_phase_trace(self._h, buf), "phase_trace")
        return [int(v) for v in buf]

    def prefilter_row_bytes(self) -> int:
        return int(self._lib.crag_index_prefilter_row_bytes(self._h))

    def last_scan_kernel(self) -> str:
        name = self._lib.crag_index_last_scan_kernel(self._h)
        return name.decode() if name else ""

    def scan_waits(self) -> str:
        name = self._lib.crag_index_scan_waits(self._h)
        return name.decode() if name else ""

    def scan_geometry(self, nq: int) -> dict:
        wg, th, qb = ctypes.c_int(0), ctypes.c_int(0), ctypes.c_int(0)
        ab = ctypes.c_int64(0)
        _native.check(self._lib.crag_index_scan_geometry(self._h, int(nq), ctypes.byref(wg),
                                                         ctypes.byref(th), ctypes.byref(qb),
                                                         ctypes.byref(ab)), "scan_geometry")
        return {"workgroups": wg.value, "threads": th.value, "query_blocks": qb.value,
                "algorithmic_bytes": int(ab.value)}


def merge_topk(d_ids, d_scores, d_counts, d_out_ids, d_out_scores, d_out_counts, stream: int = 0,
               device: Optional[int] = None) -> None:
    lib = _native.load()
    n_lists, nq, k = (int(v) for v in d_ids.shape)
    dev = d_ids.device.index if device is None else device
    _native.check(lib.crag_merge_topk(int(dev or 0), d_ids.data_ptr(), d_scores.data_ptr(),
                                      d_counts.data_ptr(), n_lists, nq, k, d_out_ids.data_ptr(),
                                      d_out_scores.data_ptr(), d_out_counts.data_ptr(),
                                      ctypes.c_void_p(stream)), "crag_merge_topk")


class ResultRecord:

    @staticmethod
    def record_bytes(nq: int, k: int) -> int:
        return int(_native.load().crag_result_record_bytes(int(nq), int(k)))

    def __init__(self, nq: int, k: int, device, buf=None) -> None:
        self.nq, self.k = int(nq), int(k)
        self.nbytes = self.record_bytes(self.nq, self.k)
        if buf is None:
            buf = torch.zeros(self.nbytes, dtype=torch.uint8, device=device)
        if buf.dtype != torch.uint8 or buf.numel() != self.nbytes or not buf.is_contiguous() or buf.data_ptr() % 8:
            raise ValueError("a ResultRecord needs a contiguous, 8-byte aligned uint8 buffer of record_bytes(nq, k) bytes")
        self.buf = buf
        a, b = self.nq * self.k * 8, self.nq * self.k * 12
        self.ids = self.buf[:a].view(torch.int64).view(self.nq, self.k)
        self.scores = self.buf[a:b].view(torch.float32).view(self.nq, self.k)
        self.counts = self.buf[b:b + self.nq * 4].view(torch.int32)


def merge_topk_packed(d_records, n_lists: int, nq: int, k: int, d_out_ids, d_out_scores, d_out_counts,
                      stream: int = 0) -> None:
    lib = _native.load()
    _native.check(lib.crag_merge_topk_packed(int(d_records.device.index or 0), d_records.data_ptr(), int(n_lists),
                                             int(nq), int(k), d_out_ids.data_ptr(), d_out_scores.data_ptr(),
                                             d_out_counts.data_ptr(), ctypes.c_void_p(stream)),
                  "crag_merge_topk_packed")
```

### include/crag_dense.h

```cpp
#ifndef CRAG_DENSE_H
#define CRAG_DENSE_H

#include <stdint.h>

#ifdef __cplusplus
extern "C" {
#endif

#define CRAG_OK 0
#define CRAG_EINVAL (-1)
#define CRAG_EHIP (-2)
#define CRAG_ENOMEM (-3)
#define CRAG_E2BIG (-5)
#define CRAG_ENODEV (-4)

#define CRAG_MAX_K 128
#define CRAG_DIM 1024

typedef struct crag_index crag_index;

const char *crag_last_error(void);
const char *crag_version(void);
int crag_device_count(void);


int crag_index_create(int device, int dim, int64_t capacity, crag_index **out);
int crag_index_destroy(crag_index *ix);

int crag_index_add(crag_index *ix, const float *rows, const int64_t *ids, int64_t n);

int crag_index_update(crag_index *ix, int64_t pos, const float *rows, int64_t n);


int crag_index_remove(crag_index *ix, const int64_t *ids, int64_t n, int64_t *out_removed);

int crag_index_compact(crag_index *ix, const uint8_t *keep_mask, int64_t *out_size);

int crag_index_insert(crag_index *ix, const float *rows, const int64_t *ids, int64_t n);

int64_t crag_index_size(const crag_index *ix);
int64_t crag_index_capacity(const crag_index *ix);
int crag_index_dim(const crag_index *ix);

int crag_index_get_rows(crag_index *ix, int64_t pos, int64_t n, float *rows, int64_t *ids);

int crag_index_count_eligible(crag_index *ix, const uint8_t *row_mask, int64_t *out_count);

int crag_index_search(crag_index *ix, const float *queries, int nq, int k,
                      const uint8_t *row_mask, int64_t mask_stride, int64_t *out_ids,
                      float *out_scores, int32_t *out_counts);

int crag_index_search_async(crag_index *ix, const float *d_queries, int nq, int k,
                            const uint8_t *d_row_mask, int64_t mask_stride, int64_t *d_out_ids,
                            float *d_out_scores, int32_t *d_out_counts, void *stream);

#define CRAG_PIPE_INPUTS_READY 1
int crag_index_search_pipelined(crag_index *ix, const float *d_queries, int nq, int k,
                                const uint8_t *d_row_mask, int64_t mask_stride, int64_t *d_out_ids,
                                float *d_out_scores, int32_t *d_out_counts, void *stream, int flags);
int crag_index_join(crag_index *ix, void *stream);

#define CRAG_DEDUPE_MAX_WIDTH 256
int crag_index_dedupe_async(crag_index *ix, const int64_t *d_ids, const int32_t *d_counts, int nq, int width,
                            float threshold, int64_t *d_out_ids, int32_t *d_out_counts,
                            int32_t *d_out_dup_of, float *d_out_sim, void *stream);

#define CRAG_SUBSET_MAX_WIDTH 4096
int64_t crag_index_search_ids_scratch_bytes(int nq, int width);
int crag_index_search_ids_async(crag_index *ix, const float *d_queries, int nq, const int64_t *d_ids,
                                const int32_t *d_counts, int width, int64_t list_stride, int k, int64_t *d_out_ids,
                                float *d_out_scores, int32_t *d_out_counts, float *d_out_slot_scores, void *d_scratch,
                                int64_t scratch_bytes, void *stream);

#define CRAG_GROUP_MAX_PER 8
int64_t crag_index_search_grouped_scratch_bytes(int nq, int64_t n_groups, int per_group);
int crag_index_search_grouped_async(crag_index *ix, const float *d_queries, int nq, int k, const int32_t *d_row_group,
                                    int64_t n_groups, int per_group, const uint8_t *d_row_mask, int64_t mask_stride,
                                    int64_t *d_out_ids, float *d_out_scores, int32_t *d_out_groups, int32_t *d_out_counts,
                                    void *d_scratch, int64_t scratch_bytes, void *stream);

int crag_merge_topk(int device, const int64_t *d_ids, const float *d_scores,
                    const int32_t *d_counts, int n_lists, int nq, int k, int64_t *d_out_ids,
                    float *d_out_scores, int32_t *d_out_counts, void *stream);

int64_t crag_result_record_bytes(int nq, int k);
int crag_merge_topk_packed(int device, const void *d_records, int n_lists, int nq, int k,
                           int64_t *d_out_ids, float *d_out_scores, int32_t *d_out_counts, void *stream);

int crag_rrf_fuse(int n_lanes, const int64_t *const *d_lane_ids, const int32_t *const *d_lane_counts,
                  const int *lane_width, int nq, int rrf_k, int out_k, int64_t *d_out_ids,
                  double *d_out_scores, uint32_t *d_out_lanes, int32_t *d_out_counts, void *stream);

int crag_tech_lane(const int32_t *d_order, const int64_t *d_row_ptr, const uint64_t *d_tokens,
                   const int64_t *d_ids, int64_t n_rows, const uint64_t *d_query_tokens,
                   const int32_t *d_query_token_counts, int nq, int k, const uint8_t *d_row_mask,
                   int64_t mask_stride, uint64_t *d_bitmap_scratch, int64_t *d_out_ids,
                   int32_t *d_out_counts, void *stream);

typedef struct crag_upload_slot crag_upload_slot;
crag_upload_slot *crag_upload_slot_create(void);
void crag_upload_slot_destroy(crag_upload_slot *slot);
int crag_tech_lane_host(const int32_t *d_order, const int64_t *d_row_ptr, const uint64_t *d_tokens,
                        const int64_t *d_ids, int64_t n_rows, const uint64_t *h_token_hashes,
                        const int32_t *h_token_counts, int nq, int k, const uint8_t *d_row_mask, int64_t mask_stride,
                        crag_upload_slot *slot, uint64_t *d_bitmap_scratch, int64_t *d_out_ids, int32_t *d_out_counts,
                        void *stream);

int64_t crag_bm25_scratch_bytes(int64_t n_rows, int nq, int k);
int crag_bm25_lane_host(const int64_t *d_post_ptr, const int32_t *d_post_pos, const uint16_t *d_post_tf,
                        const int32_t *d_doc_len, const int64_t *d_ids, int64_t n_rows, int64_t n_terms, float avgdl,
                        const int32_t *h_q_ptr, const int32_t *h_term_ids, const float *h_weights, int nq, int k,
                        const uint8_t *d_row_mask, int64_t mask_stride, crag_upload_slot *slot, void *d_scratch,
                        int64_t scratch_bytes, int64_t *d_out_ids, float *d_out_scores, int32_t *d_out_counts,
                        void *stream);

#define CRAG_FILTER_MAX_QUERIES 64
int crag_filter_masks_host(const int64_t *d_started_us, const int32_t *d_call_slot, int64_t n_rows, int64_t n_calls,
                           const uint64_t *h_call_qset, const int64_t *h_date_from, const int64_t *h_date_to, int nq,
                           crag_upload_slot *slot, uint8_t *d_out_mask, int64_t mask_stride, void *stream);

#define CRAG_ATTR_MAX_QUERIES 64
#define CRAG_ATTR_MAX_CLAUSES 8
#define CRAG_ATTR_MAX_KEYS    512
int crag_attr_masks_host(const int64_t *d_attr_ptr, const int32_t *d_attr_ids, int64_t n_rows, int64_t n_attrs,
                         const int32_t *h_keys, const uint64_t *h_key_sets, int n_keys,
                         const uint64_t *h_clause_sets, int nq,
                         const uint8_t *d_in_mask, int64_t in_stride,
                         crag_upload_slot *slot, uint8_t *d_out_mask, int64_t mask_stride, void *stream);

#define CRAG_FACET_MAX_QUERIES    64
#define CRAG_FACET_MAX_NAMESPACES 16
#define CRAG_FACET_MAX_TOP        64
int64_t crag_facet_workspace_bytes(int64_t n_rows, int nq, int64_t width, int has_masks);
int crag_facet_counts_host(const int64_t *d_post_ptr, const int32_t *d_post_rows, const int32_t *d_post_fid,
                           int64_t n_postings, int64_t n_rows, int64_t n_attrs,
                           const uint8_t *d_masks, int64_t mask_stride,
                           const int32_t *h_range_lo, const int32_t *h_range_hi, int n_ranges, int nq, int top,
                           void *d_workspace, int64_t workspace_bytes,
                           int32_t *d_out_ids, uint32_t *d_out_counts, int32_t *d_out_distinct, int64_t *d_out_rows,
                           void *stream);

int crag_index_profile_enable(crag_index *ix, int enabled);
int crag_index_profile_read(crag_index *ix, int64_t *n_launches, double *scan_ms_total,
                            double *merge_ms_total);
int crag_index_profile_read_ex(crag_index *ix, int64_t *n_launches, double *scan_ms_total,
                               double *merge_ms_total, double *event_pair_ms_total);

int crag_index_prefilter_stats(crag_index *ix, int64_t *searches, int64_t *candidates, int64_t *rescored_rows);

int crag_index_phase_trace(crag_index *ix, uint64_t *out128);

const char *crag_index_last_scan_kernel(const crag_index *ix);

const char *crag_index_scan_waits(const crag_index *ix);

int64_t crag_index_prefilter_row_bytes(const crag_index *ix);

int crag_index_scan_geometry(const crag_index *ix, int nq, int *workgroups, int *threads,
                             int *query_blocks, int64_t *algorithmic_bytes_per_launch);

#ifdef __cplusplus
}
#endif
#endif
```

Baseline: 1.371 million queries/sec.

## Add per-workgroup candidate slots and speculative rescoring tail to the prefilter finalize

```diff
diff --git a/cadence_rag_amd/_native.py b/cadence_rag_amd/_native.py
--- a/cadence_rag_amd/_native.py
+++ b/cadence_rag_amd/_native.py
@@ -81,6 +81,7 @@
                                               _c.POINTER(_c.c_double), _c.POINTER(_c.c_double)]),
     "crag_index_last_scan_kernel": (_c.c_char_p, [_P]),
     "crag_index_scan_waits": (_c.c_char_p, [_P]),
+    "crag_index_pf_tail": (_c.c_char_p, [_P]),
     "crag_index_prefilter_row_bytes": (_c.c_int64, [_P]),
     "crag_index_search_pipelined": (_c.c_int, [_P, _P, _c.c_int, _c.c_int, _P, _c.c_int64, _P, _P, _P, _P, _c.c_int]),
     "crag_index_join": (_c.c_int, [_P, _P]),
diff --git a/cadence_rag_amd/csrc/crag_api.hip b/cadence_rag_amd/csrc/crag_api.hip
--- a/cadence_rag_amd/csrc/crag_api.hip
+++ b/cadence_rag_amd/csrc/crag_api.hip
@@ -31,6 +31,12 @@
     if (const char *v = getenv("CRAG_PF_WAITS")) {
         if (!strcmp(v, "tile")) ix->sw.pf_waits = crag::PF_WAITS_TILE;
         else if (!strcmp(v, "fragment")) ix->sw.pf_waits = crag::PF_WAITS_FRAGMENT;
+    }
+    if (const char *v = getenv("CRAG_PF_TAIL")) {
+        if (!strcmp(v, "classic")) ix->sw.pf_tail = crag::PF_TAIL_CLASSIC;
+        else if (!strcmp(v, "slots")) ix->sw.pf_tail = crag::PF_TAIL_SLOTS;
+        else if (!strcmp(v, "spec")) ix->sw.pf_tail = crag::PF_TAIL_SPEC;
+        else if (!strcmp(v, "both")) ix->sw.pf_tail = crag::PF_TAIL_BOTH;
     }
     if (const char *v = getenv("CRAG_PF_LAGS")) {
         int d = 0, r = 0;
@@ -275,6 +281,7 @@
 
 const char *crag_index_last_scan_kernel(const crag_index *ix) { return ix ? ix->last_scan_kernel : ""; }
 const char *crag_index_scan_waits(const crag_index *ix) { return ix ? ix->last_scan_waits : ""; }
+const char *crag_index_pf_tail(const crag_index *ix) { return ix ? ix->last_pf_tail : ""; }
 
 int64_t crag_index_prefilter_row_bytes(const crag_index *ix) {
     if (!ix || ix->sw.no_prefilter) return 0;
diff --git a/cadence_rag_amd/csrc/crag_api_search.hip b/cadence_rag_amd/csrc/crag_api_search.hip
--- a/cadence_rag_amd/csrc/crag_api_search.hip
+++ b/cadence_rag_amd/csrc/crag_api_search.hip
@@ -42,7 +42,11 @@
     return CRAG_OK;
 }
 
-int reserve_workspace(const crag_index *ix, Workspace *ws, const SearchPlan &pl, int k, hipStream_t st) {
+int cand_stride(const SearchPlan &pl, int tail) {
+    return pl.cap + ((tail & crag::PF_TAIL_SLOTS) ? pl.G * crag::PF_SLOTS : 0);
+}
+
+int reserve_workspace(const crag_index *ix, Workspace *ws, const SearchPlan &pl, int k, int tail, hipStream_t st) {
     DevBuf *b = ws->buf;
     const size_t nq_pad = (size_t)pl.nq_pad;
     int rc;
@@ -53,7 +57,9 @@
     if (!pl.prefilter) return CRAG_OK;
     if ((rc = b[Workspace::A16].ensure(nq_pad * crag::DIM * 2))) return rc;
     if ((rc = b[Workspace::PF_GBOUND].ensure_zeroed((ix->n_cu + nq_pad) * crag::PF_BOUND_CELLS * sizeof(uint32_t), st))) return rc;
-    if ((rc = b[Workspace::PF_CAND].ensure(nq_pad * pl.cap * sizeof(uint2)))) return rc;
+    if ((rc = b[Workspace::PF_CAND].ensure(nq_pad * (size_t)cand_stride(pl, tail) * sizeof(uint2)))) return rc;
+    if ((tail & crag::PF_TAIL_SLOTS) &&
+        (rc = b[Workspace::PF_SLOTBUF].ensure(nq_pad * pl.G * crag::PF_SLOTS * sizeof(uint2)))) return rc;
     if (pl.rsplit > 1) {
         const size_t slots = nq_pad * 8;
         if ((rc = b[Workspace::PF_XKEYS].ensure(slots * CRAG_MAX_K * sizeof(uint64_t)))) return rc;
@@ -132,7 +138,7 @@
 }
 
 crag::PfParams pf_params(const crag_index *ix, const Workspace *ws, const SearchPlan &pl, const SearchArgs &a,
-                         int reverse) {
+                         int reverse, int tail) {
     crag::PfParams fp;
     fp.corpus = ix->corpus;
     fp.corpus16 = ix->corpus16;
@@ -155,6 +161,8 @@
     fp.sets = pl.sets;
     fp.pub0 = pl.pub0;
     fp.cap = pl.cap;
+    fp.cand_stride = cand_stride(pl, tail);
+    fp.slots = (tail & crag::PF_TAIL_SLOTS) ? ws->at<uint2>(Workspace::PF_SLOTBUF) : nullptr;
     fp.derive_lag = pl.derive_lag;
     fp.read_lag = pl.read_lag;
     fp.nt = pl.nt;
@@ -162,13 +170,17 @@
 }
 
 crag::FinParams fin_params(const crag_index *ix, const Workspace *ws, const SearchPlan &pl, const SearchArgs &a,
-                           const crag::PfParams &fp, crag::ScanParams sp, const crag::MergeParams &mp) {
+                           const crag::PfParams &fp, crag::ScanParams sp, const crag::MergeParams &mp, int tail) {
     crag::FinParams fin;
     fin.corpus = ix->corpus;
     fin.inv_norm = ix->inv_norm;
     fin.a32 = ws->at<const float>(Workspace::A32);
     fin.qinv = ws->at<const float>(Workspace::QINV);
-    fin.cand = ws->at<const uint2>(Workspace::PF_CAND);
+    fin.cand = ws->at<uint2>(Workspace::PF_CAND);
+    fin.cand_stride = fp.cand_stride;
+    fin.slots = fp.slots;
+    fin.tail = tail;
+    fin.G = pl.G;
     fin.count = ws->at<uint32_t>(Workspace::PF_COUNT);
     fin.gbound = fp.gbound;
     fin.flags = ws->at<const uint32_t>(Workspace::PF_FLAGS);
@@ -204,7 +216,9 @@
     int rc;
     Workspace *ws = nullptr;
     if ((rc = acquire_workspace(ix, st, &ws))) return rc;
-    if ((rc = reserve_workspace(ix, ws, pl, a.k, st))) return rc;
+    const int tail = pl.prefilter ? pf_tail_for(a.k, pl.sets, pl.rsplit, pl.G, ix->corpus16 ? ix->size * (int64_t)crag::DIM * 2 : 0,
+                                                   ix->sw.pf_tail) : crag::PF_TAIL_CLASSIC;
+    if ((rc = reserve_workspace(ix, ws, pl, a.k, tail, st))) return rc;
     if (pl.window_too_large)
         return fail(CRAG_EINVAL, "index too large for one device scan window (%lld rows)", (long long)ix->size);
     EvSet *ev = nullptr;
@@ -221,21 +235,24 @@
     }
     if (pl.prefilter) {
         if (++ws->seq == 0u) ws->seq = 1u;
-        const crag::PfParams fp = pf_params(ix, ws, pl, a, reverse);
+        const crag::PfParams fp = pf_params(ix, ws, pl, a, reverse, tail);
         const int nqb = pl.wide ? 2 : 1;
         ws->dirty = true;
         const int waits = pf_waits_for(ix->size * (int64_t)crag::DIM * 2, ix->corpus16 != nullptr, pl.nt, ix->sw.pf_waits);
         HIP_TRY(crag::launch_prefilter(fp, nqb, pl.nq_pad / (32 * nqb), waits == crag::PF_WAITS_FRAGMENT, st,
                                        &ix->last_scan_kernel));
         ix->last_scan_waits = waits == crag::PF_WAITS_FRAGMENT ? "fragment" : "tile";
+        static const char *const tail_names[4] = {"classic", "slots", "spec", "both"};
+        ix->last_pf_tail = tail_names[tail & 3];
         if (ix->env_fail_after_scan > 0 && ++ix->pf_searches == ix->env_fail_after_scan)
             return fail(CRAG_EHIP, "injected failure behind the scan launch (CRAG_TEST_FAIL_AFTER_SCAN)");
         if (ev) HIP_TRY(hipEventRecord(ev->e2, st));
-        HIP_TRY(crag::launch_finalize(fin_params(ix, ws, pl, a, fp, sp, mp), st));
+        HIP_TRY(crag::launch_finalize(fin_params(ix, ws, pl, a, fp, sp, mp, tail), st));
         ws->dirty = false;
     } else {
         HIP_TRY(crag::launch_scan(sp, pl.q_blocks, st, &ix->last_scan_kernel));
         ix->last_scan_waits = "tile";
+        ix->last_pf_tail = "classic";
         if (ev) HIP_TRY(hipEventRecord(ev->e2, st));
         HIP_TRY(crag::launch_merge_partials(mp, a.nq, st));
     }
@@ -278,6 +295,12 @@
 }
 
 int64_t crag_pf_frag_waits_max_bytes_(void) { return crag::PF_FRAG_WAITS_MAX_BYTES; }
+
+int crag_pf_tail_(int k, int sets, int rsplit, int G, int64_t mirror_bytes, int pf_tail_switch) {
+    return pf_tail_for(k, sets, rsplit, G, mirror_bytes, pf_tail_switch);
+}
+
+int64_t crag_pf_slots_max_bytes_(void) { return crag::PF_SLOTS_MAX_BYTES; }
 
 int crag_index_search_async(crag_index *ix, const float *d_queries, int nq, int k,
                             const uint8_t *d_row_mask, int64_t mask_stride, int64_t *d_out_ids,
diff --git a/cadence_rag_amd/csrc/crag_exact.h b/cadence_rag_amd/csrc/crag_exact.h
--- a/cadence_rag_amd/csrc/crag_exact.h
+++ b/cadence_rag_amd/csrc/crag_exact.h
@@ -105,6 +105,21 @@
     }
 }
 
+__device__ __forceinline__ float exact_slice_chain(const f32x4 *qslice , const f32x4 (&c0)[16],
+                                                   const f32x4 (&c1)[16]) {
+    float acc = 0.f;
+#pragma unroll
+    for (int s = 0; s < 16; ++s) {
+        const f32x4 q0 = qslice[2 * s], q1 = qslice[2 * s + 1];
+#pragma unroll
+        for (int cc = 0; cc < 4; ++cc) {
+            acc = __builtin_fmaf(q0[cc], c0[s][cc], acc);
+            acc = __builtin_fmaf(q1[cc], c1[s][cc], acc);
+        }
+    }
+    return acc;
+}
+
 __device__ __forceinline__ void slice_query_read(const f32x4 *qslice, int h, f32x4 (&q)[8]) {
 #pragma unroll
     for (int i = 0; i < 8; ++i) q[i] = qslice[8 * h + i];
diff --git a/cadence_rag_amd/csrc/crag_index.h b/cadence_rag_amd/csrc/crag_index.h
--- a/cadence_rag_amd/csrc/crag_index.h
+++ b/cadence_rag_amd/csrc/crag_index.h
@@ -18,7 +18,7 @@
 struct Workspace {
     enum Buf {
         PARTIAL, GBOUND,
-        A32, A16, QINV, PF_CAND, PF_XKEYS, PF_XIDS, PF_XCOUNT,
+        A32, A16, QINV, PF_CAND, PF_SLOTBUF, PF_XKEYS, PF_XIDS, PF_XCOUNT,
         PF_GBOUND, PF_COUNT, PF_FLAGS, PF_XTICKET,
         N_BUF,
         KEPT_ZERO_FIRST = PF_GBOUND, KEPT_ZERO_END = N_BUF
@@ -66,6 +66,7 @@
     unsigned long long *phase_trace = nullptr;
     const char *last_scan_kernel = "";
     const char *last_scan_waits = "";
+    const char *last_pf_tail = "";
     DevBuf stage_q, stage_rows, stage_ids, stage_mask, stage_out, scratch;
     int64_t edit_chunk_rows = 16384;
     DevBuf edit_bounce, edit_srcpos, edit_mask, edit_prefix, edit_newpos;
diff --git a/cadence_rag_amd/csrc/crag_kernels.h b/cadence_rag_amd/csrc/crag_kernels.h
--- a/cadence_rag_amd/csrc/crag_kernels.h
+++ b/cadence_rag_amd/csrc/crag_kernels.h
@@ -57,6 +57,10 @@
 constexpr int PF_MIN_ROWS_PER_GROUP = 128;
 enum PfWaits { PF_WAITS_TILE = 0, PF_WAITS_FRAGMENT = 1 };
 constexpr int64_t PF_FRAG_WAITS_MAX_BYTES = 256ll << 20;
+enum PfTail { PF_TAIL_CLASSIC = 0, PF_TAIL_SLOTS = 1, PF_TAIL_SPEC = 2, PF_TAIL_BOTH = 3 };
+constexpr int PF_SLOTS = 2;
+constexpr int64_t PF_SLOTS_MAX_BYTES = 256ll << 20;
+constexpr int PF_SLOTS_MAX_K = 10;
 
 struct PrepParams {
     const float *queries;
@@ -87,6 +91,8 @@
     int nt;
     int derive_lag, read_lag;
     int cap;
+    int cand_stride;
+    uint2 *slots;
 };
 
 struct FinParams {
@@ -94,7 +100,10 @@
     const float *inv_norm;
     const float *a32;
     const float *qinv;
-    const uint2 *cand;
+    uint2 *cand;
+    int cand_stride;
+    const uint2 *slots;
+    int tail;
     uint32_t *count;
     uint32_t *gbound;
     const uint32_t *flags;
@@ -105,6 +114,7 @@
     int32_t *out_counts;
     unsigned long long *stats;
     int k, cap;
+    int G;
     int nq;
     int rsplit;
     uint64_t *xkeys;
diff --git a/cadence_rag_amd/csrc/crag_search.hip b/cadence_rag_amd/csrc/crag_search.hip
--- a/cadence_rag_amd/csrc/crag_search.hip
+++ b/cadence_rag_amd/csrc/crag_search.hip
@@ -1385,6 +1385,8 @@
     uint32_t n_stage;
     uint32_t need[NQB];
     uint32_t want_flush[2][SCAN_WAVES];
+    uint32_t qslot[32 * NQB];
+    uint32_t spill;
 };
 
 template <int NQB>
@@ -1415,7 +1417,8 @@
     __syncthreads();
     const uint32_t n = L.n_stage < (uint32_t)PF_STAGE ? L.n_stage : (uint32_t)PF_STAGE;
     const int tid = threadIdx.x;
-    if (LAST && n == 0u) return;
+    const bool to_slots = LAST && p.slots != nullptr;
+    if (LAST && n == 0u && !to_slots) return;
     uint2 ent[PF_PER];
     bool keep[PF_PER];
 #pragma unroll
@@ -1427,6 +1430,30 @@
             keep[i] = ord2f(ent[i].x) >= L.qthr[ent[i].y & 63u];
         }
     }
+    if constexpr (LAST) {
+        if (to_slots) {
+            const size_t wg_slot0 = ((size_t)blockIdx.y * (32 * NQB) * p.G + blockIdx.x) * PF_SLOTS;
+#pragma unroll
+            for (int i = 0; i < PF_PER; ++i)
+                if (keep[i]) {
+                    const uint32_t ql = ent[i].y & 63u;
+                    const uint32_t pos = atomicAdd(&L.qslot[ql], 1u);
+                    if (pos < (uint32_t)PF_SLOTS) {
+                        p.slots[wg_slot0 + (size_t)ql * p.G * PF_SLOTS + pos] =
+                            make_uint2(ent[i].x, (uint32_t)(window_row0 + (int64_t)(ent[i].y >> 6)));
+                        keep[i] = false;
+                    } else {
+                        L.spill = 1u;
+                    }
+                }
+            __syncthreads();
+            if (tid < 32 * NQB * PF_SLOTS) {
+                const uint32_t ql = (uint32_t)tid / PF_SLOTS, sl = (uint32_t)tid % PF_SLOTS;
+                if (sl >= L.qslot[ql]) p.slots[wg_slot0 + (size_t)ql * p.G * PF_SLOTS + sl] = make_uint2(0u, 0u);
+            }
+            if (L.spill == 0u) return;
+        }
+    }
     if (tid < 32 * NQB) {
         L.qcount[tid] = 0u;
         L.qfill[tid] = 0u;
@@ -1459,7 +1486,7 @@
             const uint32_t pos = L.qbase[ql] + atomicAdd(&L.qfill[ql], 1u);
             const int qg = (int)blockIdx.y * (32 * NQB) + (int)ql;
             if (pos < (uint32_t)p.cap) {
-                p.cand[(size_t)qg * p.cap + pos] = make_uint2(ent[i].x, (uint32_t)(window_row0 + (int64_t)(ent[i].y >> 6)));
+                p.cand[(size_t)qg * p.cand_stride + pos] = make_uint2(ent[i].x, (uint32_t)(window_row0 + (int64_t)(ent[i].y >> 6)));
             } else {
                 p.flags[0] = p.seq;
             }
@@ -1559,6 +1586,8 @@
     if (threadIdx.x < 32 * NQB) L.qthr[threadIdx.x] = -__builtin_inff();
     if (threadIdx.x < NQB) L.need[threadIdx.x] = 0u;
     if (threadIdx.x == 0) L.n_stage = 0u;
+    if (threadIdx.x < 32 * NQB) L.qslot[threadIdx.x] = 0u;
+    if (threadIdx.x == 0) L.spill = 0u;
     constexpr int PF_STASH = MIRROR ? PF_STASH_MIRROR : PF_STASH_ROWS;
     float stash[PF_STASH][RPO];
 #pragma unroll
@@ -1887,13 +1916,14 @@
     unsigned long long hist[64];
     int s_nbest, s_nsurv, s_rescored;
     uint32_t s_kth;
+    int s_nslot;
 };
 union FinFbLds {
     FinLds f;
     float2 slab[2][SCAN_WAVES][8][64];
 };
 
-template <int S, int PS>
+template <int S, int PS, bool SLOTS = false, bool SPEC = false>
 __global__ __launch_bounds__(SCAN_THREADS) void finalize_fb_kernel(FinParams p) {
     __shared__ FinFbLds U;
     __shared__ int s_last;
@@ -1939,10 +1969,18 @@
     int &s_nbest = U.f.s_nbest, &s_nsurv = U.f.s_nsurv, &s_rescored = U.f.s_rescored;
     uint32_t &s_kth = U.f.s_kth;
     const int q = (int)blockIdx.x / R, rpart = (int)blockIdx.x % R, tid = threadIdx.x;
-    const uint2 *gcand = p.cand + (size_t)q * p.cap;
+    const uint2 *gcand = p.cand + (size_t)q * p.cand_stride;
+    if constexpr (SLOTS) {
+        if (tid == 0) U.f.s_nslot = 0;
+    }
     const bool overflow = p.flags[0] == p.seq;
     const uint32_t total = p.count[q];
-    const uint2 first = gcand[tid];
+    uint2 first = make_uint2(0u, 0u);
+    if constexpr (SLOTS) {
+        if (tid < p.G * PF_SLOTS) first = p.slots[(size_t)q * p.G * PF_SLOTS + tid];
+    } else {
+        first = gcand[tid];
+    }
     const float qinv = p.qinv[q];
     f32x4 qfrag = f32x4{0.f, 0.f, 0.f, 0.f};
     if (tid < 256)
@@ -1960,11 +1998,18 @@
         return;
     }
     const int k = p.k;
-    const int C = (int)(total < (uint32_t)p.cap ? total : (uint32_t)p.cap);
-    const bool in_lds = C <= FIN_ROUND;
-    if (tid < C) lcand[tid] = first;
-    if (in_lds)
-        for (int e = tid + NT; e < C; e += NT) lcand[e] = gcand[e];
+    int C = (int)(total < (uint32_t)p.cap ? total : (uint32_t)p.cap);
+    bool in_lds = C <= FIN_ROUND;
+    if constexpr (SLOTS) {
+        asm volatile("s_waitcnt lgkmcnt(0)" ::: "memory");
+        __builtin_amdgcn_s_barrier();
+        asm volatile("" ::: "memory");
+        if (first.x != 0u) lcand[atomicAdd(&U.f.s_nslot, 1)] = first;
+    } else {
+        if (tid < C) lcand[tid] = first;
+        if (in_lds)
+            for (int e = tid + NT; e < C; e += NT) lcand[e] = gcand[e];
+    }
     if (tid < 256) qs[tid >> 5][(tid >> 1) & 15][tid & 1] = qfrag;
     if (tid == 0) {
         s_nbest = 0;
@@ -1973,10 +2018,81 @@
     }
     __syncthreads();
     if (tid == 0 && R == 1) p.count[q] = 0u;
+    unsigned long long n_cand = (unsigned long long)total;
+    if constexpr (SLOTS) {
+        const int n_slot = U.f.s_nslot, n_list = C;
+        n_cand += (unsigned long long)n_slot;
+        C = n_slot + n_list;
+        in_lds = C <= FIN_ROUND;
+        if (n_list > 0) {
+            if (in_lds) {
+                for (int e = tid; e < n_list; e += NT) lcand[n_slot + e] = gcand[e];
+            } else if (tid < n_slot) {
+                p.cand[(size_t)q * p.cand_stride + n_list + tid] = lcand[tid];
+            }
+            __syncthreads();
+        }
+    }
     FIN_T(1);
 
+    const int grp = tid >> 3, sub = tid & 7;
+    const bool spec = SPEC && C <= 64;
+    if constexpr (SPEC) {
+        if (spec) {
+            const bool live = grp < C;
+            const uint2 ce = live ? lcand[grp] : make_uint2(0u, 0u);
+            const uint32_t row = ce.y;
+            float inv_row = 0.f;
+            int64_t rid = -1;
+            f32x4 c0[16], c1[16];
+            if (live) {
+                if (sub == 0) {
+                    inv_row = p.inv_norm[row];
+                    rid = p.ids ? p.ids[row] : (int64_t)row;
+                }
+                const f32x4 *ctile = reinterpret_cast<const f32x4 *>(p.corpus + (size_t)(row >> 5) * TILE_FLOATS) + (size_t)sub * 32 * 32;
+                exact_slice_fetch<PS>(ctile, (int)(row & 31u), c0, c1);
+            }
+            __builtin_amdgcn_sched_barrier(0);
+            uint32_t thr_spec = 0u;
+            if (C > k) {
+                const int ln = tid & 63;
+                const uint32_t mine = ln < C ? lcand[ln].x : 0u;
+                int rank = 0;
+                for (int i = 0; i < C; ++i) {
+                    const uint32_t o = lcand[i].x;
+                    rank += (o > mine || (o == mine && i < ln)) ? 1 : 0;
+                }
+                const unsigned long long at = __builtin_amdgcn_ballot_w64(ln < C && rank == k - 1);
+                const uint32_t kth = (uint32_t)__builtin_amdgcn_readlane((int)mine, (int)__builtin_ctzll(at)) &
+                                     ~((1u << FIN_SKIP_BITS) - 1u);
+                thr_spec = f2ord(ord2f(kth) - 2.f * PF_DELTA);
+            }
+            FIN_T(2);
+            float part = 0.f;
+            if (live) part = exact_slice_chain(&qs[sub][0][0], c0, c1);
+            float d = __shfl(part, (tid & 63 & ~7) | 0);
+#pragma unroll
+            for (int ww = 1; ww < 8; ++ww) d += __shfl(part, (tid & 63 & ~7) | ww);
+            if (live && sub == 0 && ce.x >= thr_spec) {
+                atomicAdd(&s_rescored, 1);
+                const float scale = inv_row * qinv;
+                float sc = d * scale;
+                sc = __builtin_amdgcn_fmed3f(sc, -1.f, 1.f);
+                if (scale > 0.f && sc == sc) {
+                    const uint32_t u = __float_as_uint(sc);
+                    const uint32_t ord = u ^ ((uint32_t)((int32_t)u >> 31) | 0x80000000u);
+                    const int slot = atomicAdd(&s_nbest, 1);
+                    best[slot] = mk64(ord, ~row);
+                    best_id[slot] = rid;
+                }
+            }
+            __syncthreads();
+        }
+    }
+
     uint32_t thr_ord = 0u;
-    if (C > k) {
+    if (!spec && C > k) {
         if (C <= 64) {
             if (tid < C) {
                 const uint32_t mine = lcand[tid].x;
@@ -2063,10 +2179,9 @@
         }
         thr_ord = f2ord(ord2f(s_kth) - 2.f * PF_DELTA);
     }
-    FIN_T(2);
-
-    const int grp = tid >> 3, sub = tid & 7;
-    for (int r0 = 0; r0 < C; r0 += FIN_ROUND) {
+    if (!spec) FIN_T(2);
+
+    for (int r0 = spec ? C : 0; r0 < C; r0 += FIN_ROUND) {
         const int rn = (C - r0) < FIN_ROUND ? (C - r0) : FIN_ROUND;
         if (tid == 0) s_nsurv = 0;
         __syncthreads();
@@ -2227,7 +2342,7 @@
     if (tid == 0) {
         p.out_counts[q] = count;
         if (stat) {
-            stat[0] = stat_old[0] + (unsigned long long)total;
+            stat[0] = stat_old[0] + n_cand;
             stat[1] = stat_old[1] + rescored_all;
             if (q == 0) stat[2] = stat_old[2] + 1ull;
         }
@@ -2332,6 +2447,21 @@
 hipError_t launch_finalize(const FinParams &p, hipStream_t st) {
     const dim3 grid(p.nq * p.rsplit + p.fb_blocks), block(SCAN_THREADS);
     const int ks = (p.k + 31) / 32;
+    if (p.tail != PF_TAIL_CLASSIC) {
+        const bool big = p.scan.piece_shift == PS_BIG;
+#define CRAG_TAIL(SLOTS_, SPEC_)                                                                              \
+    do {                                                                                                      \
+        if (big) hipLaunchKernelGGL((finalize_fb_kernel<1, PS_BIG, SLOTS_, SPEC_>), grid, block, 0, st, p);   \
+        else hipLaunchKernelGGL((finalize_fb_kernel<1, PS_SMALL, SLOTS_, SPEC_>), grid, block, 0, st, p);     \
+    } while (0)
+        if (ks != 1 || p.rsplit != 1 || ((p.tail & PF_TAIL_SLOTS) && (!p.slots || p.G * PF_SLOTS > FIN_THREADS)))
+            return hipErrorInvalidValue;
+        if (p.tail == PF_TAIL_SLOTS) CRAG_TAIL(true, false);
+        else if (p.tail == PF_TAIL_SPEC) CRAG_TAIL(false, true);
+        else CRAG_TAIL(true, true);
+#undef CRAG_TAIL
+        return hipGetLastError();
+    }
     if (p.scan.piece_shift == PS_BIG) {
         if (ks == 1) hipLaunchKernelGGL((finalize_fb_kernel<1, PS_BIG>), grid, block, 0, st, p);
         else if (ks == 2) hipLaunchKernelGGL((finalize_fb_kernel<2, PS_BIG>), grid, block, 0, st, p);
diff --git a/cadence_rag_amd/csrc/crag_search_plan.h b/cadence_rag_amd/csrc/crag_search_plan.h
--- a/cadence_rag_amd/csrc/crag_search_plan.h
+++ b/cadence_rag_amd/csrc/crag_search_plan.h
@@ -13,6 +13,7 @@
     int pf_nt = -1;
     int64_t nt_above_bytes = 1536ll << 20;
     int pf_waits = -1;
+    int pf_tail = -1;
 };
 
 struct SearchPlan {
@@ -62,3 +63,13 @@
     if (pf_waits_switch >= 0) return pf_waits_switch ? crag::PF_WAITS_FRAGMENT : crag::PF_WAITS_TILE;
     return mirror_bytes <= crag::PF_FRAG_WAITS_MAX_BYTES ? crag::PF_WAITS_FRAGMENT : crag::PF_WAITS_TILE;
 }
+
+inline int pf_tail_for(int k, int sets, int rsplit, int G, int64_t mirror_bytes, int pf_tail_switch) {
+    if (k > 24 || sets != 1 || rsplit != 1) return crag::PF_TAIL_CLASSIC;
+    const bool slots_fit = G * crag::PF_SLOTS <= crag::SCAN_THREADS;
+    if (pf_tail_switch < 0)
+        return slots_fit && k <= crag::PF_SLOTS_MAX_K && mirror_bytes > 0 && mirror_bytes <= crag::PF_SLOTS_MAX_BYTES
+                   ? crag::PF_TAIL_SLOTS
+                   : crag::PF_TAIL_CLASSIC;
+    return (pf_tail_switch & crag::PF_TAIL_BOTH) & (slots_fit ? crag::PF_TAIL_BOTH : crag::PF_TAIL_SPEC);
+}
diff --git a/cadence_rag_amd/dense_index.py b/cadence_rag_amd/dense_index.py
--- a/cadence_rag_amd/dense_index.py
+++ b/cadence_rag_amd/dense_index.py
@@ -422,6 +422,10 @@
         name = self._lib.crag_index_scan_waits(self._h)
         return name.decode() if name else ""
 
+    def pf_tail(self) -> str:
+        name = self._lib.crag_index_pf_tail(self._h)
+        return name.decode() if name else ""
+
     def scan_geometry(self, nq: int) -> dict:
         wg, th, qb = ctypes.c_int(0), ctypes.c_int(0), ctypes.c_int(0)
         ab = ctypes.c_int64(0)
diff --git a/include/crag_dense.h b/include/crag_dense.h
--- a/include/crag_dense.h
+++ b/include/crag_dense.h
@@ -154,6 +154,8 @@
 
 const char *crag_index_scan_waits(const crag_index *ix);
 
+const char *crag_index_pf_tail(const crag_index *ix);
+
 int64_t crag_index_prefilter_row_bytes(const crag_index *ix);
 
 int crag_index_scan_geometry(const crag_index *ix, int nq, int *workgroups, int *threads,
```

Result: no change. 1.384 million queries/sec, median of 6 (+0.9%).
